# shizukutanaka/Otedama

Hardware: AMD Instinct MI355X
Metric: hashes/sec (whole node) SHA-256d + scrypt at 1/2/4/8 MI355X; p50 share latency (higher is better)
Workload: dtype u32

## Files before the change

csrc/bindings.cpp:

```cpp
#include <pybind11/pybind11.h>
#include <pybind11/stl.h>

#include <array>
#include <atomic>
#include <cstring>
#include <stdexcept>
#include <thread>
#include <tuple>

#include "otedama/aead.h"
#include "otedama/job.h"
#include "otedama/runtime.h"
#include "otedama/trace.h"
#include "otedama/sha256.h"
#include "otedama/sv2_frame.h"
#include "otedama/clock_bounds.h"
#include "otedama/launch_plan.h"
#include "otedama/search_launch.h"
#include "otedama/work_queue.h"
#include "otedama/x11.h"

namespace py = pybind11;
using namespace otedama;

namespace {

std::string need(const py::bytes& b, size_t n, const char* what) {
  std::string s = b;
  if (s.size() != n) throw std::invalid_argument(std::string(what) + ": expected " + std::to_string(n) + " bytes");
  return s;
}

py::bytes to_bytes(const uint8_t* p, size_t n) { return py::bytes(reinterpret_cast<const char*>(p), n); }

std::shared_ptr<JobTemplate> make_job(const py::dict& d) {
  auto j = std::make_shared<JobTemplate>();
  auto get = [&](const char* k) -> py::object {
    if (d.contains(k)) return py::object(d[k]);
    return py::none();
  };
  std::string hdr = need(d["header"].cast<py::bytes>(), 80, "header");
  std::memcpy(j->header, hdr.data(), 80);
  std::string tgt = need(d["target"].cast<py::bytes>(), 32, "target");
  std::memcpy(j->target, tgt.data(), 32);
  if (!get("epoch").is_none()) j->epoch = d["epoch"].cast<uint64_t>();
  if (!get("job_id").is_none()) j->job_id = d["job_id"].cast<std::string>();
  if (!get("channel_id").is_none()) j->channel_id = d["channel_id"].cast<uint32_t>();
  if (!get("algo").is_none()) {
    auto a = d["algo"].cast<std::string>();
    if (a == "sha256d") j->algo = Algo::kSha256d;
    else if (a == "scrypt") j->algo = Algo::kScrypt;
    else if (a == "x11") j->algo = Algo::kX11;
    else throw std::invalid_argument("unsupported algo for the native miner: " + a);
  }
  if (!get("version_mask").is_none()) j->version_mask = d["version_mask"].cast<uint32_t>();
  if (!get("ntime_roll").is_none()) j->ntime_roll = d["ntime_roll"].cast<uint32_t>();
  if (!get("coinb1").is_none()) {
    j->has_coinbase = true;
    std::string c1 = d["coinb1"].cast<py::bytes>(), c2 = d["coinb2"].cast<py::bytes>();
    std::string e1 = d["extranonce1"].cast<py::bytes>();
    j->coinb1.assign(c1.begin(), c1.end());
    j->coinb2.assign(c2.begin(), c2.end());
    j->extranonce1.assign(e1.begin(), e1.end());
    j->extranonce2_size = d["extranonce2_size"].cast<uint32_t>();
    for (auto& br : d["merkle_branches"].cast<py::list>()) {
      std::string b = br.cast<py::bytes>();
      j->merkle_branches.emplace_back(b.begin(), b.end());
    }
  }
  if (!get("variant_start").is_none()) j->variant_start = d["variant_start"].cast<uint64_t>();
  if (!get("variant_stride").is_none()) j->variant_stride = d["variant_stride"].cast<uint64_t>();
  if (j->variant_stride == 0) j->variant_stride = 1;
  return j;
}

py::list shares_to_list(std::vector<ShareRecord>&& v) {
  py::list out;
  for (auto& s : v) {
    py::dict d;
    d["epoch"] = s.epoch;
    d["job_id"] = s.job_id;
    d["channel_id"] = s.channel_id;
    d["nonce"] = s.nonce;
    d["ntime"] = s.ntime;
    d["version"] = s.version;
    d["extranonce2"] = s.extranonce2;
    d["extranonce2_size"] = s.extranonce2_size;
    d["hash"] = to_bytes(s.hash, 32);
    d["device_id"] = s.device_id;
    d["found_at"] = s.found_at;
    d["device_found_at"] = s.device_found_at;
    out.append(d);
  }
  return out;
}

py::dict stats_to_dict(const MinerStats& s) {
  py::dict d;
  d["hashes"] = s.hashes;
  d["candidates"] = s.candidates;
  d["shares"] = s.shares;
  d["dropped"] = s.dropped;
  d["launches"] = s.launches;
  d["rejected_candidates"] = s.rejected_candidates;
  d["variant_launches"] = s.variant_launches;
  d["busy_seconds"] = s.busy_seconds;
  d["faulted"] = s.faulted;
  d["error"] = s.error;
  d["variant_next"] = s.variant_next;
  d["variant_epoch"] = s.variant_epoch;
  d["job_switches"] = s.job_switches;
  d["last_job_switch_ms"] = s.last_job_switch_ms;
  d["job_switch_ms"] = s.job_switch_ms;
  d["work_started"] = s.work_started;
  d["reserved_cus"] = s.reserved_cus;
  d["ring_overflow"] = s.ring_overflow;
  d["verify_dropped"] = s.verify_dropped;
  d["verify_queue_peak"] = s.verify_queue_peak;
  d["launch_hashes"] = s.launch_hashes;
  d["aborted_launches"] = s.aborted_launches;
  d["ring_hits"] = s.ring_hits;
  d["clock_calib_rtt_us"] = s.clock_calib_rtt_us;
  d["clock_samples"] = s.clock_samples;
  d["host_abort"] = s.host_abort;
  d["hashes_done_at_s"] = s.hashes_done_at_s;
  {
    py::dict ph;
    for (const auto& kv : s.startup_ms) ph[py::str(kv.first)] = kv.second;
    d["startup_ms"] = ph;
    py::dict rs;
    for (const auto& kv : s.startup_rss_mb) rs[py::str(kv.first)] = kv.second;
    d["startup_rss_mb"] = rs;
  }
  return d;
}

}

PYBIND11_MODULE(_native, m) {
  m.doc() = "Otedama MI355X native runtime (gfx950 HIP kernels + C++ host runtime)";

  m.def("cpu_has_sha_ni", &cpu_has_sha_ni);
  m.def("sha256", [](const py::bytes& b) {
    std::string s = b; uint8_t o[32];
    sha256(reinterpret_cast<const uint8_t*>(s.data()), s.size(), o);
    return to_bytes(o, 32);
  });
  m.def("sha256d", [](const py::bytes& b) {
    std::string s = b; uint8_t o[32];
    { py::gil_scoped_release r; sha256d(reinterpret_cast<const uint8_t*>(s.data()), s.size(), o); }
    return to_bytes(o, 32);
  });
  m.def("hmac_sha256", [](const py::bytes& k, const py::bytes& msg) {
    std::string ks = k, ms = msg; uint8_t o[32];
    hmac_sha256(reinterpret_cast<const uint8_t*>(ks.data()), ks.size(),
                reinterpret_cast<const uint8_t*>(ms.data()), ms.size(), o);
    return to_bytes(o, 32);
  });
  m.def("aead_seal", [](int kind, const py::bytes& key, const py::bytes& nonce, const py::bytes& plain,
                        const py::bytes& aad) {
    std::string out = aead_seal(static_cast<AeadKind>(kind), key, nonce, plain, aad);
    return py::bytes(out);
  }, py::arg("kind"), py::arg("key"), py::arg("nonce"), py::arg("plain"), py::arg("aad") = py::bytes());
  m.def("aead_open", [](int kind, const py::bytes& key, const py::bytes& nonce, const py::bytes& sealed,
                        const py::bytes& aad) -> py::object {
    std::string out;
    if (!aead_open(static_cast<AeadKind>(kind), key, nonce, sealed, aad, &out)) return py::none();
    return py::bytes(out);
  }, py::arg("kind"), py::arg("key"), py::arg("nonce"), py::arg("sealed"), py::arg("aad") = py::bytes());
  m.attr("SCRYPT_COOP") = kScryptCoop;
  m.attr("SCRYPT_LANE_W8") = kScryptLaneW8;
  m.attr("SCRYPT_COOP2") = kScryptCoop2;
  m.attr("SCRYPT_COOP_SPLIT") = kScryptCoopSplit;
  m.attr("AEAD_AES256GCM") = 0;
  m.attr("AEAD_CHACHA20POLY1305") = 1;
  m.def("scrypt_1024_1_1_batch", [](const std::vector<py::bytes>& hs) {
    std::vector<std::string> in;
    for (const auto& h : hs) in.push_back(need(h, 80, "header"));
    std::vector<std::array<uint8_t, 32>> out(in.size());
    std::vector<const uint8_t*> ip;
    std::vector<uint8_t*> op;
    for (size_t i = 0; i < in.size(); ++i) {
      ip.push_back(reinterpret_cast<const uint8_t*>(in[i].data()));
      op.push_back(out[i].data());
    }
    {
      py::gil_scoped_release r;
      scrypt_1024_1_1_batch(int(in.size()), ip.data(), op.data());
    }
    py::list res;
    for (const auto& o : out) res.append(to_bytes(o.data(), 32));
    return res;
  });
  m.def("scrypt_1024_1_1", [](const py::bytes& h) {
    std::string s = need(h, 80, "header"); uint8_t o[32];
    { py::gil_scoped_release r; scrypt_1024_1_1(reinterpret_cast<const uint8_t*>(s.data()), o); }
    return to_bytes(o, 32);
  });
  m.def("_clock_bounds", [](double window, const std::vector<std::pair<double, double>>& samples) {
    ClockBounds cb(window);
    std::vector<double> out;
    for (const auto& s : samples) out.push_back(cb.add(s.first, s.second));
    return out;
  });
  m.def("_launch_plan_rules", [](uint64_t batch_nonces, uint32_t target_hi, bool capped, int sha_variants, int run,
                                 const std::string& reserve_cus, int ncu) {
    const ShaLayout lay = pick_layout(sha_variants, run);
    const CuMask cm = parse_reserved_cus(reserve_cus.c_str(), ncu);
    py::dict d;
    d["batch"] = normalize_batch(batch_nonces);
    d["cap"] = launch_cap_hashes(target_hi, capped);
    d["layout"] = py::make_tuple(lay.nvar, lay.use_v);
    d["cu_mask"] = cm.words;
    d["reserved"] = cm.reserved;
    return d;
  }, py::arg("batch_nonces") = 0, py::arg("target_hi") = 0, py::arg("capped") = true, py::arg("sha_variants") = 1,
     py::arg("run") = 1, py::arg("reserve_cus") = "", py::arg("ncu") = 256);
  m.def("_launch_plan_walk", [](const std::string& kind, uint64_t batch, uint64_t cap, int nvar, uint64_t lanes,
                                uint64_t start, size_t max_launches, uint64_t variant_start, uint64_t variant_stride) {
    const LaunchKind lk = kind == "scrypt" ? LaunchKind::kScrypt : kind == "x11" ? LaunchKind::kX11
                        : kind == "v" ? LaunchKind::kVersionParallel : kind == "k" ? LaunchKind::kVariantK
                        : kind == "single" ? LaunchKind::kSingle
                        : throw std::invalid_argument("kind: scrypt, x11, v, k or single");
    if (start >= kNonceSpace) throw std::invalid_argument("start must be below 2^32");
    SearchCursor c;
    c.nonce_off = start;
    std::vector<std::tuple<uint64_t, uint64_t, uint64_t>> launches;
    while (c.k == 0 && launches.size() < max_launches) {
      const uint64_t base = c.nonce_off, count = launch_count(lk, batch, cap, nvar, lanes, c.nonce_off);
      c.advance(count, nvar);
      launches.emplace_back(base, count, c.variant_next(variant_start, variant_stride, nvar));
    }
    return py::make_tuple(launches, c.k);
  }, py::arg("kind"), py::arg("batch"), py::arg("cap"), py::arg("nvar") = 1, py::arg("lanes") = 0,
     py::arg("start") = 0, py::arg("max_launches") = size_t(1) << 20, py::arg("variant_start") = 0,
     py::arg("variant_stride") = 1);
  m.def("_work_queue_flood", [](size_t cap, size_t n, bool hash_each, size_t batch) {
    BoundedWorkQueue<std::array<uint8_t, 80>> q(cap);
    std::atomic<uint64_t> processed{0};
    uint64_t accepted = 0;
    {
      py::gil_scoped_release r;
      std::thread consumer([&] {
        if (batch > 1) {
          std::vector<std::array<uint8_t, 80>> items;
          std::vector<const uint8_t*> ip;
          std::vector<std::array<uint8_t, 32>> outs(batch);
          std::vector<uint8_t*> op;
          for (auto& o : outs) op.push_back(o.data());
          while (items.clear(), q.pop_many(&items, batch) > 0) {
            ip.clear();
            for (const auto& it : items) ip.push_back(it.data());
            if (hash_each) scrypt_1024_1_1_batch(int(items.size()), ip.data(), op.data());
            processed.fetch_add(items.size());
          }
          return;
        }
        std::array<uint8_t, 80> h;
        uint8_t out[32];
        while (q.pop(&h)) {
          if (hash_each) scrypt_1024_1_1(h.data(), out);
          processed.fetch_add(1);
        }
      });
      for (size_t i = 0; i < n; ++i) {
        std::array<uint8_t, 80> h{};
        std::memcpy(h.data() + 76, &i, 4);
        if (q.push(std::move(h))) ++accepted;
      }
      q.stop(~size_t(0));
      consumer.join();
    }
    py::dict d;
    d["accepted"] = accepted;
    d["refused"] = q.refused();
    d["peak"] = q.peak();
    d["processed"] = processed.load();
    return d;
  }, py::arg("cap"), py::arg("n"), py::arg("hash_each") = true, py::arg("batch") = 1);
  m.attr("X11_STAGES") = kX11StageCount;
  m.def("x11", [](const py::bytes& msg) {
    std::string s = msg; uint8_t o[32];
    { py::gil_scoped_release r; x11::x11(reinterpret_cast<const uint8_t*>(s.data()), s.size(), o, nullptr); }
    return to_bytes(o, 32);
  }, py::arg("msg"));
  m.def("x11_trace", [](const py::bytes& msg) {
    std::string s = msg; uint8_t o[32], t[64 * kX11StageCount];
    x11::x11(reinterpret_cast<const uint8_t*>(s.data()), s.size(), o, t);
    return to_bytes(t, sizeof t);
  }, py::arg("msg"), "The 11 intermediate 64-byte digests of the X11 chain, concatenated.");
  m.def("x11_stage", [](int i, const py::bytes& msg) {
    if (i < 0 || i >= kX11StageCount) throw std::invalid_argument("stage must be in [0, 11)");
    std::string s = msg; uint8_t o[64];
    x11::stage(i, reinterpret_cast<const uint8_t*>(s.data()), s.size(), o);
    return to_bytes(o, 64);
  }, py::arg("stage"), py::arg("msg"));
  m.def("x11_luffa_sbox_selfcheck", &x11::luffa_sbox_selfcheck);
  m.def(
      "sv2_scan",
      [](py::buffer b, uint32_t max_frame) {
        py::buffer_info info = b.request();
        if (info.itemsize != 1 || info.ndim != 1) throw std::invalid_argument("sv2_scan: need a contiguous byte buffer");
        const size_t n = (size_t)info.size;
        if (n > 0xFFFFFFFFull) throw std::invalid_argument("sv2_scan: buffer larger than 4 GiB");
        std::vector<Sv2FrameRec> recs(n / kSv2HeaderSize + 1);
        size_t consumed = 0, k = 0;
        int status = kSv2Ok;
        {
          py::gil_scoped_release nogil;
          k = sv2_scan(static_cast<const uint8_t*>(info.ptr), n, max_frame, recs.data(), recs.size(), &consumed,
                       &status);
        }
        py::list frames(k);
        for (size_t i = 0; i < k; ++i) {
          const Sv2FrameRec& r = recs[i];
          frames[i] = py::make_tuple(r.extension_type, r.msg_type, r.offset, r.length);
        }
        return py::make_tuple(frames, consumed, status);
      },
      py::arg("buf"), py::arg("max_frame"),
      "Split complete SV2 frames: ([(extension_type, msg_type, payload_offset, payload_length)], consumed, status)");
  m.def("cpu_scan_sha256d", [](const py::bytes& h, const py::bytes& t, uint32_t start, uint64_t count) {
    std::string hs = need(h, 80, "header"), ts = need(t, 32, "target");
    std::vector<uint32_t> hits;
    {
      py::gil_scoped_release r;
      hits = cpu_scan_sha256d(reinterpret_cast<const uint8_t*>(hs.data()), reinterpret_cast<const uint8_t*>(ts.data()),
                              start, count);
    }
    return hits;
  }, py::arg("header"), py::arg("target"), py::arg("start"), py::arg("count"));
  m.def("cpu_scan_method", &cpu_scan_method);
  m.def("_cpu_scan_lanes", [](int lanes, const py::bytes& h, const py::bytes& t, uint32_t start, uint64_t count) {
    std::string hs = need(h, 80, "header"), ts = need(t, 32, "target");
    std::vector<uint32_t> hits;
    {
      py::gil_scoped_release r;
      hits = cpu_scan_sha256d_lanes(lanes, reinterpret_cast<const uint8_t*>(hs.data()),
                                    reinterpret_cast<const uint8_t*>(ts.data()), start, count);
    }
    return hits;
  });
  m.def("merkle_root", [](const py::dict& job, uint64_t en2) {
    auto j = make_job(job); uint8_t root[32];
    merkle_root_from_coinbase(*j, en2, root);
    return to_bytes(root, 32);
  });
  m.def("variant_header", [](const py::dict& job, uint64_t v) {
    auto j = make_job(job);
    uint8_t hdr[80]; uint32_t ver, nt; uint64_t en2;
    j->variant_header(v, hdr, &ver, &nt, &en2);
    return py::make_tuple(to_bytes(hdr, 80), ver, nt, en2);
  });
  m.def("variant_space", [](const py::dict& job) { return make_job(job)->variant_space(); });

  m.def("sha256d_prepare", [](const py::bytes& h, const py::bytes& t) {
    std::string hs = need(h, 80, "header"), ts = need(t, 32, "target");
    Sha256dParams p;
    sha256d_prepare(reinterpret_cast<const uint8_t*>(hs.data()), reinterpret_cast<const uint8_t*>(ts.data()), &p);
    return py::bytes(reinterpret_cast<const char*>(&p), sizeof p);
  });
  m.attr("SHA256D_MAX_K") = kSha256dMaxK;
  {
    py::list ks;
    for (int k = 2; k <= kSha256dMaxK; ++k)
      if (sha256d_k_floor(k) == k) ks.append(k);
    m.attr("SHA256D_K_VALUES") = py::tuple(ks);
  }
  m.def("sha256d_prepare_k", [](const py::list& headers, const py::bytes& t) {
    std::string ts = need(t, 32, "target");
    std::vector<std::string> hs;
    for (auto& h : headers) hs.push_back(need(h.cast<py::bytes>(), 80, "header"));
    std::vector<const uint8_t*> ptrs;
    for (auto& h : hs) ptrs.push_back(reinterpret_cast<const uint8_t*>(h.data()));
    Sha256dParamsK p;
    if (!sha256d_prepare_k(ptrs.data(), (int)ptrs.size(), reinterpret_cast<const uint8_t*>(ts.data()), &p))
      throw std::invalid_argument("need K headers (K in SHA256D_K_VALUES) with identical bytes 64..75");
    return py::bytes(reinterpret_cast<const char*>(&p), sizeof p);
  }, py::arg("headers"), py::arg("target"));
  m.attr("SHA256D_V_GROUP") = kSha256dVGroup;
  m.attr("SHA256D_V2_GROUP") = kSha256dV2Group;
  m.def("sha256d_prepare_v", [](const py::list& headers, const py::bytes& t) {
    std::string ts = need(t, 32, "target");
    std::vector<std::string> hs;
    for (auto& h : headers) hs.push_back(need(h.cast<py::bytes>(), 80, "header"));
    std::vector<const uint8_t*> ptrs;
    for (auto& h : hs) ptrs.push_back(reinterpret_cast<const uint8_t*>(h.data()));
    Sha256dParamsV p;
    std::vector<Sha256dVariant> vars(hs.size());
    if (!sha256d_prepare_v(ptrs.data(), (int)ptrs.size(), reinterpret_cast<const uint8_t*>(ts.data()), &p, vars.data()))
      throw std::invalid_argument("need a positive multiple of 64 headers with identical bytes 64..75");
    return py::make_tuple(py::bytes(reinterpret_cast<const char*>(&p), sizeof p),
                          py::bytes(reinterpret_cast<const char*>(vars.data()), vars.size() * sizeof(Sha256dVariant)));
  }, py::arg("headers"), py::arg("target"));
  m.def("scrypt_prepare", [](const py::bytes& h, const py::bytes& t) {
    std::string hs = need(h, 80, "header"), ts = need(t, 32, "target");
    ScryptParams p;
    scrypt_prepare(reinterpret_cast<const uint8_t*>(hs.data()), reinterpret_cast<const uint8_t*>(ts.data()), &p);
    return py::bytes(reinterpret_cast<const char*>(&p), sizeof p);
  });

  m.def("x11_prepare", [](const py::bytes& h, const py::bytes& t) {
    std::string hs = need(h, 80, "header"), ts = need(t, 32, "target");
    X11Params p;
    x11_prepare(reinterpret_cast<const uint8_t*>(hs.data()), reinterpret_cast<const uint8_t*>(ts.data()), &p);
    return py::bytes(reinterpret_cast<const char*>(&p), sizeof p);
  });

  m.def("trace_push", [](const std::string& name) { trace_push(name.c_str()); });
  m.def("trace_pop", [] { trace_pop(); });
  m.def("trace_mark", [](const std::string& name) { trace_mark(name.c_str()); });
  m.def("gpu_device_count", &gpu_device_count);
  m.def("gpu_arch_name", &gpu_arch_name);
  m.def("gpu_cu_count", &gpu_cu_count);
  m.def("scrypt_scratch_bytes", &scrypt_scratch_bytes);
  m.def("maps_range_writable", [](const std::string& maps, uint64_t lo, uint64_t hi) {
    return maps_range_writable(maps, uintptr_t(lo), uintptr_t(hi));
  });
  m.def("launch_sha256d", [](const py::bytes& params, uint32_t base, uint64_t count, uintptr_t out, uint32_t cap,
                             int grid, uintptr_t stream) {
    std::string ps = need(params, sizeof(Sha256dParams), "params");
    Sha256dParams p; std::memcpy(&p, ps.data(), sizeof p);
    if (count == 0 || count > (1ull << 32)) throw std::invalid_argument("count must be in [1, 2^32]");
    if (grid <= 0 || out == 0) throw std::invalid_argument("bad grid / out");
    py_launch_sha256d(p, base, count, out, cap, grid, stream);
  }, py::arg("params"), py::arg("base"), py::arg("count"), py::arg("out"), py::arg("cap"), py::arg("grid"),
     py::arg("stream"));
  m.def("launch_sha256d_k", [](const py::bytes& params, uint32_t base, uint64_t count, uintptr_t out, uint32_t cap,
                               int grid, uintptr_t stream) {
    std::string ps = need(params, sizeof(Sha256dParamsK), "params");
    Sha256dParamsK p; std::memcpy(&p, ps.data(), sizeof p);
    if (p.k < 2 || p.k > kSha256dMaxK) throw std::invalid_argument("bad K");
    if (count == 0 || count > (1ull << 32)) throw std::invalid_argument("count must be in [1, 2^32]");
    if (grid <= 0 || out == 0) throw std::invalid_argument("bad grid / out");
    py_launch_sha256d_k(p, base, count, out, cap, grid, stream);
  }, py::arg("params"), py::arg("base"), py::arg("count"), py::arg("out"), py::arg("cap"), py::arg("grid"),
     py::arg("stream"));
  m.def("launch_sha256d_v", [](const py::bytes& params, uintptr_t vars, uint32_t base, uint64_t count, uintptr_t out,
                               uint32_t cap, int grid, uintptr_t stream, bool occupancy8, int block, int chains) {
    std::string ps = need(params, sizeof(Sha256dParamsV), "params");
    Sha256dParamsV p; std::memcpy(&p, ps.data(), sizeof p);
    p.occupancy8 = occupancy8 ? 1u : 0u;
    if (p.groups == 0 || count == 0 || count > (1ull << 32)) throw std::invalid_argument("bad groups / count");
    if (block != 64 && block != 256) throw std::invalid_argument("block must be 64 or 256 threads");
    if (chains < 1 || chains > 4) throw std::invalid_argument("chains must be 1..4");
    if (p.groups % uint32_t(chains) != 0)
      throw std::invalid_argument("chains variants per lane need a multiple of 64 * chains variants");
    if (grid <= 0 || (uint64_t(grid) * uint32_t(block / 64)) % (p.groups / uint32_t(chains)) != 0 || vars == 0 || out == 0)
      throw std::invalid_argument("the wave count must be a multiple of the variant groups; vars/out must be set");
    py_launch_sha256d_v(p, vars, base, count, out, cap, grid, stream, block, chains);
  }, py::arg("params"), py::arg("vars"), py::arg("base"), py::arg("count"), py::arg("out"), py::arg("cap"),
     py::arg("grid"), py::arg("stream"), py::arg("occupancy8") = false, py::arg("block") = 256, py::arg("chains") = 1);
  m.def("launch_scrypt", [](const py::bytes& params, uint32_t base, uint32_t count, uintptr_t xbuf, uintptr_t scratch,
                            int gap, uintptr_t out, uint32_t cap, int grid, uintptr_t stream) {
    std::string ps = need(params, sizeof(ScryptParams), "params");
    ScryptParams p; std::memcpy(&p, ps.data(), sizeof p);
    if (gap != 1 && gap != 2 && gap != 4 && gap != kScryptCoop && gap != kScryptLaneW8 && gap != kScryptCoop2 &&
        gap != kScryptCoopSplit)
      throw std::invalid_argument("gap must be 1, 2, 4, SCRYPT_COOP or SCRYPT_LANE_W8");
    if (grid <= 0 || out == 0 || xbuf == 0 || scratch == 0 || count == 0) throw std::invalid_argument("bad launch args");
    py_launch_scrypt(p, base, count, xbuf, scratch, gap, out, cap, grid, stream);
  }, py::arg("params"), py::arg("base"), py::arg("count"), py::arg("xbuf"), py::arg("scratch"), py::arg("gap"),
     py::arg("out"), py::arg("cap"), py::arg("grid"), py::arg("stream"));

  m.def("launch_x11_stage", [](const py::bytes& params, int stage, uint32_t base, uintptr_t H, uint32_t stride,
                               uint32_t n, uintptr_t out, uint32_t cap, uintptr_t stream) {
    std::string ps = need(params, sizeof(X11Params), "params");
    X11Params p; std::memcpy(&p, ps.data(), sizeof p);
    if (stage < 0 || stage >= kX11StageCount) throw std::invalid_argument("stage must be in [0, 11)");
    if (H == 0 || n == 0 || stride < n) throw std::invalid_argument("need H != 0, n > 0, stride >= n");
    py_launch_x11_stage(p, stage, base, H, stride, n, out, cap, stream);
  }, py::arg("params"), py::arg("stage"), py::arg("base"), py::arg("H"), py::arg("stride"), py::arg("n"),
     py::arg("out") = 0, py::arg("cap") = 0, py::arg("stream") = 0);
  m.def("launch_x11", [](const py::bytes& params, uint32_t base, uintptr_t H, uint32_t stride, uint32_t n,
                         uintptr_t out, uint32_t cap, uintptr_t stream) {
    std::string ps = need(params, sizeof(X11Params), "params");
    X11Params p; std::memcpy(&p, ps.data(), sizeof p);
    if (H == 0 || n == 0 || stride < n) throw std::invalid_argument("need H != 0, n > 0, stride >= n");
    py_launch_x11(p, base, H, stride, n, out, cap, stream);
  }, py::arg("params"), py::arg("base"), py::arg("H"), py::arg("stride"), py::arg("n"), py::arg("out") = 0,
     py::arg("cap") = 0, py::arg("stream") = 0);

  py::class_<MinerBase, std::shared_ptr<MinerBase>>(m, "Miner")
      .def("start", &MinerBase::start, py::call_guard<py::gil_scoped_release>())
      .def("stop", &MinerBase::stop, py::call_guard<py::gil_scoped_release>())
      .def("set_job", [](MinerBase& self, py::object job) {
        if (job.is_none()) { py::gil_scoped_release r; self.set_job(nullptr); return; }
        auto j = make_job(job.cast<py::dict>());
        py::gil_scoped_release r;
        self.set_job(j);
      })
      .def("poll", [](MinerBase& self, size_t max) {
        std::vector<ShareRecord> v;
        { py::gil_scoped_release r; v = self.poll(max); }
        return shares_to_list(std::move(v));
      }, py::arg("max") = 256)
      .def("stats", [](MinerBase& self) { return stats_to_dict(self.stats()); })
      .def("share_fd", &MinerBase::share_fd,
           "eventfd that becomes readable when shares are queued (read 8 bytes to reset, then poll())")
      .def_property_readonly("device_id", &MinerBase::device_id);

  py::class_<GpuMiner, MinerBase, std::shared_ptr<GpuMiner>>(m, "GpuMiner")
      .def(py::init<int, std::string, uint64_t, int, size_t, int>(), py::arg("device"), py::arg("device_id"),
           py::arg("batch_nonces") = (1ull << 32), py::arg("grid") = 2048, py::arg("queue_cap") = 1024,
           py::arg("sha_variants") = 128);
  py::class_<CpuMiner, MinerBase, std::shared_ptr<CpuMiner>>(m, "CpuMiner")
      .def(py::init<int, std::string, size_t>(), py::arg("threads"), py::arg("device_id") = "cpu-0",
           py::arg("queue_cap") = 1024);

  m.attr("SHA256D_PARAMS_SIZE") = sizeof(Sha256dParams);
  m.attr("SHA256D_V_PARAMS_SIZE") = sizeof(Sha256dParamsV);
  m.attr("SCRYPT_PARAMS_SIZE") = sizeof(ScryptParams);
}
```

csrc/include/otedama/hitsink.h:

```cpp
#pragma once
#include <cstdint>

namespace otedama {

struct HitRecord {
  uint32_t nonce;
  uint32_t variant;
  uint32_t stamp;
  uint32_t tag;
};
static_assert(sizeof(HitRecord) == 16, "HitRecord is one 16-byte record");

struct HitSink {
  uint32_t* out = nullptr;
  HitRecord* ring = nullptr;
  const uint32_t* abort = nullptr;
  uint32_t cap = 0;
  uint32_t tag = 0;
  uint32_t epoch = 0;
  uint32_t words = 1;
};

}
```

csrc/include/otedama/launch_plan.h:

```cpp
#pragma once
#include <algorithm>
#include <cstdint>
#include <cstdlib>
#include <vector>

#include "otedama/job.h"

namespace otedama {

constexpr uint32_t kHitCap = 4096;
constexpr uint64_t kMinLaunchHashes = 1ull << 22;
constexpr uint64_t kNoLaunchCap = 1ull << 40;
constexpr uint64_t kNonceSpace = 1ull << 32;

inline uint64_t normalize_batch(uint64_t batch_nonces) {
  if (batch_nonces == 0 || batch_nonces > kNonceSpace) batch_nonces = 1ull << 30;
  while (kNonceSpace % batch_nonces) --batch_nonces;
  return batch_nonces;
}

inline uint64_t launch_cap_hashes(uint32_t target_hi, bool capped) {
  if (!capped) return kNoLaunchCap;
  const double p = (double(target_hi) + 1.0) / 4294967296.0;
  const double lim = double(kHitCap / 8) / p;
  uint64_t cap = kNoLaunchCap;
  while (cap > kMinLaunchHashes && double(cap) > lim) cap >>= 1;
  return cap;
}

struct ShaLayout {
  int nvar = 1;
  bool use_v = false;
};

inline ShaLayout pick_layout(int sha_variants, int run) {
  const int sha_k = sha_variants < 1 ? 1 : sha_variants > kSha256dMaxK ? kSha256dMaxK : sha_variants;
  if (sha_variants >= kSha256dV2Group && run >= kSha256dV2Group) return {kSha256dV2Group, true};
  if (sha_variants >= kSha256dVGroup && run >= kSha256dVGroup) return {kSha256dVGroup, true};
  if (sha_k > 1) return {sha256d_k_floor(std::min(run, sha_k)), false};
  return {1, false};
}

enum class LaunchKind { kScrypt, kX11, kVersionParallel, kVariantK, kSingle };

inline uint64_t launch_count(LaunchKind kind, uint64_t batch, uint64_t cap, int nvar, uint64_t lanes,
                             uint64_t nonce_off) {
  const uint64_t remaining = kNonceSpace - nonce_off;
  const uint64_t launch = std::min(batch, cap);
  switch (kind) {
    case LaunchKind::kScrypt:
    case LaunchKind::kX11:
      return std::min({remaining, lanes, cap});
    case LaunchKind::kVersionParallel:
      return std::min(launch >= uint64_t(nvar) ? launch / uint64_t(nvar) : 1, remaining);
    case LaunchKind::kVariantK: {
      uint64_t div = 1;
      while (div * 2 <= uint64_t(nvar) && div * 2 <= launch) div *= 2;
      return std::min(launch / div, remaining);
    }
    case LaunchKind::kSingle:
      break;
  }
  return std::min(launch, remaining);
}

struct SearchCursor {
  uint64_t k = 0;
  uint64_t nonce_off = 0;

  void reset() { k = 0; nonce_off = 0; }
  void advance(uint64_t count, int nvar) {
    nonce_off += count;
    if (nonce_off >= kNonceSpace) { nonce_off = 0; k += uint64_t(nvar); }
  }
  uint64_t variant_next(uint64_t variant_start, uint64_t variant_stride, int nvar) const {
    return variant_start + (nonce_off == 0 ? k : k + uint64_t(nvar)) * variant_stride;
  }
};

struct CuMask {
  std::vector<uint32_t> words;
  int reserved = 0;
};
inline CuMask parse_reserved_cus(const char* spec, int ncu) {
  CuMask m;
  m.words.assign(size_t(ncu + 31) / 32, 0xFFFFFFFFu);
  if (ncu % 32) m.words.back() = (1u << (ncu % 32)) - 1u;
  for (const char* q = spec; *q;) {
    char* end = nullptr;
    const long cu = std::strtol(q, &end, 10);
    if (end == q) break;
    if (cu >= 0 && cu < ncu && (m.words[size_t(cu) / 32] >> (cu % 32) & 1u)) {
      m.words[size_t(cu) / 32] &= ~(1u << (cu % 32));
      ++m.reserved;
    }
    q = (*end == ',') ? end + 1 : end;
  }
  return m;
}

inline uint64_t aborted_launch_hashes(uint64_t full, double rate_hpms, double ms) {
  return rate_hpms > 0 ? std::min<uint64_t>(full, uint64_t(rate_hpms * ms)) : full;
}
inline double update_rate_hpms(double rate_hpms, uint64_t full, double ms) {
  return rate_hpms > 0 ? 0.8 * rate_hpms + 0.2 * (double(full) / ms) : double(full) / ms;
}
inline double update_scrypt_hash_s(double scrypt_hash_s, double ms) { return 0.7 * scrypt_hash_s + 0.3e-3 * ms; }

}
```

csrc/include/otedama/runtime.h:

```cpp
#pragma once
#include <atomic>
#include <condition_variable>
#include <cstdint>
#include <deque>
#include <memory>
#include <mutex>
#include <string>
#include <thread>
#include <vector>

namespace otedama {

enum class Algo : int { kSha256d = 0, kScrypt = 1, kX11 = 2 };

struct JobTemplate {
  uint64_t epoch = 0;
  std::string job_id;
  uint32_t channel_id = 0;
  Algo algo = Algo::kSha256d;
  uint8_t header[80] = {0};
  uint8_t target[32] = {0};
  uint32_t version_mask = 0;
  uint32_t ntime_roll = 0;
  bool has_coinbase = false;
  std::vector<uint8_t> coinb1, coinb2, extranonce1;
  uint32_t extranonce2_size = 0;
  std::vector<std::vector<uint8_t>> merkle_branches;
  uint64_t variant_start = 0;
  uint64_t variant_stride = 1;

  uint64_t variant_space() const;
  void variant_header(uint64_t v, uint8_t out[80], uint32_t* version, uint32_t* ntime,
                      uint64_t* extranonce2) const;
};

struct ShareRecord {
  uint64_t epoch;
  std::string job_id;
  uint32_t channel_id;
  uint32_t nonce;
  uint32_t ntime;
  uint32_t version;
  uint64_t extranonce2;
  uint32_t extranonce2_size;
  uint8_t hash[32];
  std::string device_id;
  double found_at = 0;
  double device_found_at = 0;
};

struct MinerStats {
  uint64_t hashes = 0;
  uint64_t candidates = 0;
  uint64_t shares = 0;
  uint64_t dropped = 0;
  uint64_t launches = 0;
  uint64_t rejected_candidates = 0;
  uint64_t variant_launches = 0;
  double busy_seconds = 0;
  bool faulted = false;
  std::string error;
  uint64_t variant_next = 0;
  uint64_t variant_epoch = 0;
  uint64_t job_switches = 0;
  double last_job_switch_ms = 0;
  std::vector<double> job_switch_ms;
  std::vector<std::pair<uint64_t, double>> work_started;
  uint64_t aborted_launches = 0;
  uint64_t ring_hits = 0;
  uint64_t ring_overflow = 0;
  uint64_t verify_dropped = 0;
  uint64_t verify_queue_peak = 0;
  uint64_t launch_hashes = 0;
  double clock_calib_rtt_us = 0;
  uint64_t clock_samples = 0;
  bool host_abort = false;
  uint64_t reserved_cus = 0;
  double hashes_done_at_s = 0;
  std::vector<std::pair<std::string, double>> startup_ms;
  std::vector<std::pair<std::string, double>> startup_rss_mb;
};

bool verify_share(Algo algo, const uint8_t header80[80], const uint8_t target[32], uint8_t hash_out[32]);
void scrypt_1024_1_1(const uint8_t header80[80], uint8_t out[32]);
void scrypt_1024_1_1_batch(int n, const uint8_t* const header80[], uint8_t* const out[]);
void merkle_root_from_coinbase(const JobTemplate& job, uint64_t extranonce2, uint8_t root_out[32]);

class ShareQueue {
 public:
  explicit ShareQueue(size_t cap);
  ~ShareQueue();
  ShareQueue(const ShareQueue&) = delete;
  ShareQueue& operator=(const ShareQueue&) = delete;
  bool push(ShareRecord&& s);
  std::vector<ShareRecord> drain(size_t max);
  size_t size();
  uint64_t dropped() const { return dropped_.load(); }
  int event_fd() const { return efd_; }
 private:
  int efd_ = -1;
  std::mutex mu_;
  std::deque<ShareRecord> q_;
  size_t cap_;
  std::atomic<uint64_t> dropped_{0};
};

class MinerBase {
 public:
  MinerBase(std::string device_id, size_t queue_cap) : device_id_(std::move(device_id)), queue_(queue_cap) {}
  virtual ~MinerBase() = default;
  virtual void start() = 0;
  virtual void stop() = 0;
  void set_job(std::shared_ptr<const JobTemplate> job);
  std::vector<ShareRecord> poll(size_t max) { return queue_.drain(max); }
  MinerStats stats();
  const std::string& device_id() const { return device_id_; }
  int share_fd() const { return queue_.event_fd(); }

 protected:
  std::shared_ptr<const JobTemplate> current_job(uint64_t* gen);
  std::shared_ptr<const JobTemplate> peek_job(uint64_t* gen, double* set_at);
  std::string device_id_;
  ShareQueue queue_;
  std::mutex job_mu_;
  std::condition_variable job_cv_;
  std::shared_ptr<const JobTemplate> job_;
  std::shared_ptr<const JobTemplate> last_work_;
  uint64_t job_gen_ = 0;
  double job_set_at_ = 0;
  std::atomic<bool> running_{false};
  std::mutex stats_mu_;
  MinerStats stats_;
};

class GpuMiner : public MinerBase {
 public:
  GpuMiner(int device, std::string device_id, uint64_t batch_nonces, int grid, size_t queue_cap,
           int sha_variants = 128);
  ~GpuMiner() override;
  void start() override;
  void stop() override;
 private:
  struct Run;
  void loop();
  int device_;
  uint64_t batch_;
  int grid_;
  int sha_variants_;
  std::thread th_;
};

class CpuMiner : public MinerBase {
 public:
  CpuMiner(int threads, std::string device_id, size_t queue_cap);
  ~CpuMiner() override;
  void start() override;
  void stop() override;
 private:
  void loop(int tid);
  int threads_;
  std::vector<std::thread> ths_;
  std::atomic<uint64_t> cursor_{0};
  std::atomic<uint64_t> cursor_gen_{0};
  std::mutex cursor_mu_;
};

std::vector<uint32_t> cpu_scan_sha256d(const uint8_t header80[80], const uint8_t target[32], uint32_t start,
                                       uint64_t count);
std::string cpu_scan_method();
std::vector<uint32_t> cpu_scan_sha256d_lanes(int lanes, const uint8_t header80[80], const uint8_t target[32],
                                             uint32_t start, uint64_t count);

double monotonic_seconds();

bool maps_range_writable(const std::string& maps, uintptr_t lo, uintptr_t hi);

}
```

csrc/include/otedama/search_launch.h:

```cpp
#pragma once
#include <cstdint>
#include <string>

#include "otedama/hitsink.h"
#include "otedama/job.h"

namespace otedama {

uint64_t scrypt_scratch_bytes(int grid, int gap);

int gpu_device_count();
std::string gpu_arch_name(int device);
int gpu_cu_count(int device);

void py_launch_sha256d(const Sha256dParams& p, uint32_t base, uint64_t count, uintptr_t out, uint32_t cap, int grid,
                       uintptr_t stream);
void py_launch_sha256d_k(const Sha256dParamsK& p, uint32_t base, uint64_t count, uintptr_t out, uint32_t cap, int grid,
                         uintptr_t stream);
void py_launch_sha256d_v(const Sha256dParamsV& p, uintptr_t vars, uint32_t base, uint64_t count, uintptr_t out,
                         uint32_t cap, int grid, uintptr_t stream, int block, int chains);
void py_launch_scrypt(const ScryptParams& p, uint32_t base, uint32_t count, uintptr_t xbuf, uintptr_t scratch, int gap,
                      uintptr_t out, uint32_t cap, int grid, uintptr_t stream);
void py_launch_x11_stage(const X11Params& p, int stage, uint32_t base, uintptr_t H, uint32_t stride, uint32_t n,
                         uintptr_t out, uint32_t cap, uintptr_t stream);
void py_launch_x11(const X11Params& p, uint32_t base, uintptr_t H, uint32_t stride, uint32_t n, uintptr_t out,
                   uint32_t cap, uintptr_t stream);

}

#ifdef __HIPCC__
#include <hip/hip_runtime.h>

namespace otedama {

hipError_t launch_sha256d_search(const Sha256dParams& p, uint32_t base, uint64_t count, const HitSink& sink, int grid,
                                 hipStream_t stream);
hipError_t launch_sha256d_search_k(const Sha256dParamsK& p, uint32_t base, uint64_t count, const HitSink& sink,
                                   int grid, hipStream_t stream);
hipError_t launch_sha256d_search_v(const Sha256dParamsV& p, const Sha256dVariant* vars, uint32_t base, uint64_t count,
                                   const HitSink& sink, int grid, hipStream_t stream, int block = 256, int chains = 1);

hipError_t launch_scrypt_search(const ScryptParams& p, uint32_t base, uint32_t count, void* xbuf, void* scratch,
                                int gap, const HitSink& sink, int grid, hipStream_t stream);

}
#endif
```

csrc/kernels/hitsink_dev.h:

```cpp
#pragma once
#include <hip/hip_runtime.h>

#include <cstdint>

#include "otedama/hitsink.h"

namespace otedama_dev {

__device__ __forceinline__ uint32_t abort_peek(const uint32_t* word, uint32_t epoch) {
  if (word == nullptr) return epoch;
  const uint32_t v = __hip_atomic_load(const_cast<uint32_t*>(word), __ATOMIC_RELAXED, __HIP_MEMORY_SCOPE_SYSTEM);
  return __builtin_amdgcn_readfirstlane(v);
}
__device__ __forceinline__ uint32_t abort_peek(const otedama::HitSink& s) { return abort_peek(s.abort, s.epoch); }

__device__ __forceinline__ uint32_t abort_issue(const otedama::HitSink& s) {
  if (s.abort == nullptr) return s.epoch;
  return __hip_atomic_load(const_cast<uint32_t*>(s.abort), __ATOMIC_RELAXED, __HIP_MEMORY_SCOPE_SYSTEM);
}

__device__ __forceinline__ uint32_t abort_peek_scalar(const otedama::HitSink& s) {
  if (s.abort == nullptr) return s.epoch;
  uint32_t v;
  asm volatile("s_load_dword %0, %1, 0x0 glc\n\ts_waitcnt lgkmcnt(0)" : "=s"(v) : "s"(s.abort));
  return v;
}

__device__ __forceinline__ bool abort_newer(uint32_t word, uint32_t epoch) {
  return static_cast<int32_t>(word - epoch) > 0;
}
__device__ __forceinline__ bool abort_seen(uint32_t raw, uint32_t epoch) {
  return abort_newer(__builtin_amdgcn_readfirstlane(raw), epoch);
}

__device__ __forceinline__ void hit_publish(const otedama::HitSink& s, uint32_t nonce, uint32_t variant) {
  const uint32_t slot = atomicAdd(s.out, 1u);
  if (slot >= s.cap) return;
  if (s.ring != nullptr) {
    otedama::HitRecord* r = s.ring + slot;
    r->nonce = nonce;
    r->variant = variant;
    r->stamp = static_cast<uint32_t>(__builtin_amdgcn_s_memrealtime());
    __threadfence_system();
    __hip_atomic_store(&r->tag, s.tag, __ATOMIC_RELAXED, __HIP_MEMORY_SCOPE_SYSTEM);
  } else if (s.words == 2) {
    s.out[1 + 2 * slot] = nonce;
    s.out[2 + 2 * slot] = variant;
  } else {
    s.out[1 + slot] = nonce;
  }
}

}
```

csrc/kernels/scrypt_search.hip:

```cpp
#include <hip/hip_runtime.h>

#include <cstdint>

#include "cdna_bitops.h"
#include "hitsink_dev.h"
#include <cstdlib>
#include <cstring>

#include "otedama/job.h"
#include "otedama/search_launch.h"

namespace {

using namespace otedama_dev;

__device__ __forceinline__ uint32_t bswap(uint32_t x) { return __builtin_bswap32(x); }

__device__ __forceinline__ void salsa20_8(uint32_t B[16]) {
  uint32_t x0 = B[0], x1 = B[1], x2 = B[2], x3 = B[3], x4 = B[4], x5 = B[5], x6 = B[6], x7 = B[7];
  uint32_t x8 = B[8], x9 = B[9], x10 = B[10], x11 = B[11], x12 = B[12], x13 = B[13], x14 = B[14], x15 = B[15];
#pragma unroll
  for (int i = 0; i < 8; i += 2) {
    x4 ^= rol(x0 + x12, 7);   x8 ^= rol(x4 + x0, 9);    x12 ^= rol(x8 + x4, 13);   x0 ^= rol(x12 + x8, 18);
    x9 ^= rol(x5 + x1, 7);    x13 ^= rol(x9 + x5, 9);   x1 ^= rol(x13 + x9, 13);   x5 ^= rol(x1 + x13, 18);
    x14 ^= rol(x10 + x6, 7);  x2 ^= rol(x14 + x10, 9);  x6 ^= rol(x2 + x14, 13);   x10 ^= rol(x6 + x2, 18);
    x3 ^= rol(x15 + x11, 7);  x7 ^= rol(x3 + x15, 9);   x11 ^= rol(x7 + x3, 13);   x15 ^= rol(x11 + x7, 18);
    x1 ^= rol(x0 + x3, 7);    x2 ^= rol(x1 + x0, 9);    x3 ^= rol(x2 + x1, 13);    x0 ^= rol(x3 + x2, 18);
    x6 ^= rol(x5 + x4, 7);    x7 ^= rol(x6 + x5, 9);    x4 ^= rol(x7 + x6, 13);    x5 ^= rol(x4 + x7, 18);
    x11 ^= rol(x10 + x9, 7);  x8 ^= rol(x11 + x10, 9);  x9 ^= rol(x8 + x11, 13);   x10 ^= rol(x9 + x8, 18);
    x12 ^= rol(x15 + x14, 7); x13 ^= rol(x12 + x15, 9); x14 ^= rol(x13 + x12, 13); x15 ^= rol(x14 + x13, 18);
  }
  B[0] += x0; B[1] += x1; B[2] += x2; B[3] += x3; B[4] += x4; B[5] += x5; B[6] += x6; B[7] += x7;
  B[8] += x8; B[9] += x9; B[10] += x10; B[11] += x11; B[12] += x12; B[13] += x13; B[14] += x14; B[15] += x15;
}

__device__ __forceinline__ void blockmix(uint32_t X[32]) {
#pragma unroll
  for (int k = 0; k < 16; ++k) X[k] ^= X[16 + k];
  salsa20_8(X);
#pragma unroll
  for (int k = 0; k < 16; ++k) X[16 + k] ^= X[k];
  salsa20_8(X + 16);
}

__device__ __forceinline__ void store_entry(uint4* __restrict__ dst, const uint32_t X[32]) {
#pragma unroll
  for (int q = 0; q < 8; ++q) dst[q] = make_uint4(X[4 * q], X[4 * q + 1], X[4 * q + 2], X[4 * q + 3]);
}
__device__ __forceinline__ void load_entry(const uint4* __restrict__ src, uint32_t T[32]) {
#pragma unroll
  for (int q = 0; q < 8; ++q) {
    const uint4 v = src[q];
    T[4 * q] = v.x; T[4 * q + 1] = v.y; T[4 * q + 2] = v.z; T[4 * q + 3] = v.w;
  }
}

__device__ __forceinline__ void hmac_states(const uint32_t key[8], uint32_t istate[8], uint32_t ostate[8]) {
  uint32_t blk[16];
#pragma unroll
  for (int i = 0; i < 8; ++i) blk[i] = key[i] ^ 0x36363636u;
#pragma unroll
  for (int i = 8; i < 16; ++i) blk[i] = 0x36363636u;
#pragma unroll
  for (int i = 0; i < 8; ++i) istate[i] = kSha256IVd[i];
  sha256_compress(istate, blk);
#pragma unroll
  for (int i = 0; i < 8; ++i) blk[i] = key[i] ^ 0x5c5c5c5cu;
#pragma unroll
  for (int i = 8; i < 16; ++i) blk[i] = 0x5c5c5c5cu;
#pragma unroll
  for (int i = 0; i < 8; ++i) ostate[i] = kSha256IVd[i];
  sha256_compress(ostate, blk);
}

__device__ __forceinline__ void hmac_outer(const uint32_t ostate[8], const uint32_t digest[8], uint32_t out[8]) {
  uint32_t blk[16];
#pragma unroll
  for (int i = 0; i < 8; ++i) blk[i] = digest[i];
  blk[8] = 0x80000000u;
#pragma unroll
  for (int i = 9; i < 15; ++i) blk[i] = 0u;
  blk[15] = 768u;
#pragma unroll
  for (int i = 0; i < 8; ++i) out[i] = ostate[i];
  sha256_compress(out, blk);
}

__device__ __forceinline__ void scrypt_pbkdf_in(const otedama::ScryptParams& p, uint32_t nonce, uint32_t X[32]) {
  uint32_t hdrbe[20];
#pragma unroll
  for (int i = 0; i < 19; ++i) hdrbe[i] = bswap(p.hdr[i]);
  hdrbe[19] = bswap(nonce);
  uint32_t key[8];
#pragma unroll
  for (int i = 0; i < 8; ++i) key[i] = p.hmid[i];
  {
    uint32_t blk[16] = {hdrbe[16], hdrbe[17], hdrbe[18], hdrbe[19], 0x80000000u, 0, 0, 0, 0, 0, 0, 0, 0, 0, 0, 640u};
    sha256_compress(key, blk);
  }
  uint32_t istate[8], ostate[8];
  hmac_states(key, istate, ostate);
  uint32_t ist2[8];
#pragma unroll
  for (int i = 0; i < 8; ++i) ist2[i] = istate[i];
  sha256_compress(ist2, hdrbe);
#pragma unroll
  for (int blkno = 1; blkno <= 4; ++blkno) {
    uint32_t st[8];
#pragma unroll
    for (int i = 0; i < 8; ++i) st[i] = ist2[i];
    uint32_t blk[16] = {hdrbe[16], hdrbe[17], hdrbe[18], hdrbe[19], uint32_t(blkno), 0x80000000u,
                        0, 0, 0, 0, 0, 0, 0, 0, 0, (64u + 84u) * 8u};
    sha256_compress(st, blk);
    uint32_t t[8];
    hmac_outer(ostate, st, t);
#pragma unroll
    for (int i = 0; i < 8; ++i) X[8 * (blkno - 1) + i] = bswap(t[i]);
  }
}

__device__ __forceinline__ uint32_t scrypt_pbkdf_out(const otedama::ScryptParams& p, uint32_t nonce,
                                                     const uint32_t X[32]) {
  uint32_t key[8];
#pragma unroll
  for (int i = 0; i < 8; ++i) key[i] = p.hmid[i];
  {
    uint32_t blk[16] = {bswap(p.hdr[16]), bswap(p.hdr[17]), bswap(p.hdr[18]), bswap(nonce), 0x80000000u,
                        0, 0, 0, 0, 0, 0, 0, 0, 0, 0, 640u};
    sha256_compress(key, blk);
  }
  uint32_t istate[8], ostate[8];
  hmac_states(key, istate, ostate);
  uint32_t st[8];
#pragma unroll
  for (int i = 0; i < 8; ++i) st[i] = istate[i];
  uint32_t blk[16];
#pragma unroll
  for (int i = 0; i < 16; ++i) blk[i] = bswap(X[i]);
  sha256_compress(st, blk);
#pragma unroll
  for (int i = 0; i < 16; ++i) blk[i] = bswap(X[16 + i]);
  sha256_compress(st, blk);
  uint32_t tail[16] = {1u, 0x80000000u, 0, 0, 0, 0, 0, 0, 0, 0, 0, 0, 0, 0, 0, (64u + 132u) * 8u};
  sha256_compress(st, tail);
  uint32_t out[8];
  hmac_outer(ostate, st, out);
  return out[7];
}

template <int GAP>
__device__ __forceinline__ void scrypt_romix(uint32_t X[32], uint4* __restrict__ Vw, uint32_t lane) {
  for (int i = 0; i < 1024; ++i) {
    if (i % GAP == 0) store_entry(Vw + ((uint64_t(i / GAP) * 64u + lane) << 3), X);
    blockmix(X);
  }
  for (int i = 0; i < 1024; ++i) {
    const uint32_t j = X[16] & 1023u;
    uint32_t T[32];
    load_entry(Vw + ((uint64_t(j / GAP) * 64u + lane) << 3), T);
    if constexpr (GAP > 1) {
      for (uint32_t r = 0; r < (j % GAP); ++r) blockmix(T);
    }
#pragma unroll
    for (int k = 0; k < 32; ++k) X[k] ^= T[k];
    blockmix(X);
  }
}

typedef __attribute__((address_space(3))) void glds_lptr_t;
typedef unsigned coop_v4u __attribute__((ext_vector_type(4)));

#ifndef OTD_SCRYPT_STORE_CPOL
#define OTD_SCRYPT_STORE_CPOL 2
#endif
constexpr int kStoreNT = OTD_SCRYPT_STORE_CPOL;

__device__ __forceinline__ uint32_t coop_swz(uint32_t s_local) {
  return ((s_local >> 1) & 3u) | (((s_local >> 3) & 1u) << 2);
}

__device__ __forceinline__ void coop_store_entry(const uint32_t X[32], __amdgpu_buffer_rsrc_t rs, uint4* __restrict__ tile,
                                                 uint32_t lane, uint32_t i) {
  char* tb = reinterpret_cast<char*>(tile);
  uint32_t ln = lane;
  asm volatile("" : "+v"(ln));
  const uint32_t slot = ln & 7u, octet = ln >> 3, own = ln & 31u;
  const uint32_t rd = (own << 7) ^ (coop_swz(own) << 4);
#pragma unroll
  for (int h = 0; h < 2; ++h) {
    asm volatile("s_waitcnt lgkmcnt(0)" ::: "memory");
    if ((ln >> 5) == uint32_t(h)) {
#pragma unroll
      for (int c = 0; c < 8; ++c)
        *reinterpret_cast<uint4*>(tb + (rd ^ (uint32_t(c) << 4))) =
            make_uint4(X[4 * c], X[4 * c + 1], X[4 * c + 2], X[4 * c + 3]);
    }
    __builtin_amdgcn_wave_barrier();
#pragma unroll
    for (int r = 0; r < 4; ++r) {
      const uint4 v = tile[64 * r + ln];
      const uint32_t owner = uint32_t(32 * h + 8 * r) + octet;
      const uint32_t chunk = slot ^ (((octet >> 1) & 3u) | (uint32_t(r & 1) << 2));
      const coop_v4u vv = {v.x, v.y, v.z, v.w};
      __builtin_amdgcn_raw_buffer_store_b128(vv, rs, (i << 13) | (owner << 7) | (chunk << 4), 0, kStoreNT);
    }
  }
}

template <int LCPOL>
__device__ __forceinline__ void coop_issue(const uint32_t X[32], __amdgpu_buffer_rsrc_t rs, uint4* __restrict__ tile,
                                           uint32_t lane, coop_v4u R[4]) {
  uint32_t ln = lane;
  asm volatile("" : "+v"(ln));
  const uint32_t slot = ln & 7u, octet = ln >> 3;
  const uint32_t j = X[16] & 1023u;
  asm volatile("s_waitcnt lgkmcnt(0)" ::: "memory");
#pragma unroll
  for (int r = 0; r < 4; ++r) {
    const uint32_t chunk = slot ^ (((octet >> 1) & 3u) | (uint32_t(r & 1) << 2));
    const uint32_t o0 = uint32_t(8 * r) + octet, o1 = o0 + 32u;
    const uint32_t j0 = uint32_t(__shfl(int(j), int(o0), 64));
    const uint32_t j1 = uint32_t(__shfl(int(j), int(o1), 64));
    __builtin_amdgcn_raw_ptr_buffer_load_lds(rs, (glds_lptr_t*)(tile + 64 * r), 16, (j0 << 13) | (o0 << 7) | (chunk << 4),
                                             0, 0, LCPOL);
    R[r] = __builtin_amdgcn_raw_buffer_load_b128(rs, (j1 << 13) | (o1 << 7) | (chunk << 4), 0, LCPOL);
  }
}

__device__ __forceinline__ void coop_consume(uint32_t X[32], uint4* __restrict__ tile, uint32_t lane,
                                             const coop_v4u R[4]) {
  const char* tb = reinterpret_cast<const char*>(tile);
  uint32_t ln = lane;
  asm volatile("" : "+v"(ln));
  const uint32_t own = ln & 31u;
  const uint32_t rd = (own << 7) ^ (coop_swz(own) << 4);
  asm volatile("s_waitcnt vmcnt(0)" ::: "memory");
  if (ln < 32u) {
#pragma unroll
    for (int c = 0; c < 8; ++c) {
      const uint4 t = *reinterpret_cast<const uint4*>(tb + (rd ^ (uint32_t(c) << 4)));
      X[4 * c] ^= t.x; X[4 * c + 1] ^= t.y; X[4 * c + 2] ^= t.z; X[4 * c + 3] ^= t.w;
    }
  }
  asm volatile("s_waitcnt lgkmcnt(0)" ::: "memory");
#pragma unroll
  for (int r = 0; r < 4; ++r) tile[64 * r + ln] = make_uint4(R[r].x, R[r].y, R[r].z, R[r].w);
  __builtin_amdgcn_wave_barrier();
  if (ln >= 32u) {
#pragma unroll
    for (int c = 0; c < 8; ++c) {
      const uint4 t = *reinterpret_cast<const uint4*>(tb + (rd ^ (uint32_t(c) << 4)));
      X[4 * c] ^= t.x; X[4 * c + 1] ^= t.y; X[4 * c + 2] ^= t.z; X[4 * c + 3] ^= t.w;
    }
  }
}

template <int LCPOL, int POLL>
__device__ __forceinline__ bool scrypt_romix_coop(uint32_t X[32], __amdgpu_buffer_rsrc_t rs, uint4* __restrict__ tile,
                                                  uint32_t lane, const otedama::HitSink& sink) {
  static_assert(POLL > 0 && 1024 % POLL == 0, "poll interval must divide the ROMix loop");
  if (abort_newer(abort_peek(sink), sink.epoch)) return false;
  for (uint32_t c = 0; c < 1024; c += POLL) {
    if (c && abort_newer(abort_peek_scalar(sink), sink.epoch)) return false;
    for (uint32_t i = c; i < c + POLL; ++i) {
      coop_store_entry(X, rs, tile, lane, i);
      blockmix(X);
    }
  }
  if (abort_newer(abort_peek(sink), sink.epoch)) return false;
  for (int i = 0; i < 1024; ++i) {
    coop_v4u R[4];
    coop_issue<LCPOL>(X, rs, tile, lane, R);
    coop_consume(X, tile, lane, R);
    blockmix(X);
  }
  return true;
}

template <int LCPOL, int PHASE>
__device__ __forceinline__ void scrypt_romix_coop_phase(uint32_t X[32], __amdgpu_buffer_rsrc_t rs,
                                                        uint4* __restrict__ tile, uint32_t lane) {
  if constexpr (PHASE == 1) {
    for (uint32_t i = 0; i < 1024; ++i) {
      coop_store_entry(X, rs, tile, lane, i);
      blockmix(X);
    }
  } else {
    for (int i = 0; i < 1024; ++i) {
      coop_v4u R[4];
      coop_issue<LCPOL>(X, rs, tile, lane, R);
      coop_consume(X, tile, lane, R);
      blockmix(X);
    }
  }
}

template <int LCPOL>
__device__ __forceinline__ void scrypt_romix_coop2(uint32_t XA[32], uint32_t XB[32], __amdgpu_buffer_rsrc_t rsA,
                                                   __amdgpu_buffer_rsrc_t rsB, uint4* __restrict__ tile, uint32_t lane) {
  for (uint32_t i = 0; i < 1024; ++i) {
    coop_store_entry(XA, rsA, tile, lane, i);
    blockmix(XA);
    coop_store_entry(XB, rsB, tile, lane, i);
    blockmix(XB);
  }
  coop_v4u R[4];
  coop_issue<LCPOL>(XA, rsA, tile, lane, R);
  for (int i = 0; i < 1024; ++i) {
    coop_consume(XA, tile, lane, R);
    coop_issue<LCPOL>(XB, rsB, tile, lane, R);
    blockmix(XA);
    coop_consume(XB, tile, lane, R);
    if (i < 1023) coop_issue<LCPOL>(XA, rsA, tile, lane, R);
    blockmix(XB);
  }
}

}

extern "C" __global__ __launch_bounds__(256) void otd_scrypt_pbkdf_in(const otedama::ScryptParams p, uint32_t base,
                                                                      uint32_t count, uint4* __restrict__ xbuf) {
  const uint32_t i = blockIdx.x * blockDim.x + threadIdx.x;
  if (i >= count) return;
  uint32_t X[32];
  scrypt_pbkdf_in(p, base + i, X);
  store_entry(xbuf + (uint64_t(i) << 3), X);
}

template <int GAP>
__global__ __launch_bounds__(256) void otd_scrypt_romix(uint32_t count, uint4* __restrict__ xbuf,
                                                        uint4* __restrict__ V) {
  const uint64_t slot = uint64_t(blockIdx.x) * blockDim.x + threadIdx.x;
  const uint64_t nslots = uint64_t(gridDim.x) * blockDim.x;
  uint4* Vw = V + (slot >> 6) * (uint64_t(1024 / GAP) * 64u * 8u);
  const uint32_t lane = uint32_t(slot & 63u);
  for (uint64_t i = slot; i < count; i += nslots) {
    uint32_t X[32];
    load_entry(xbuf + (i << 3), X);
    scrypt_romix<GAP>(X, Vw, lane);
    store_entry(xbuf + (i << 3), X);
  }
}

template <int LCPOL, int POLL>
__global__ __launch_bounds__(256) __attribute__((amdgpu_waves_per_eu(8, 8))) void otd_scrypt_romix_coop(uint32_t count, uint4* __restrict__ xbuf,
                                                             uint4* __restrict__ V, const otedama::HitSink sink) {
  __shared__ uint4 tiles[4 * 256];
  const uint64_t slot = uint64_t(blockIdx.x) * blockDim.x + threadIdx.x;
  const uint64_t nslots = uint64_t(gridDim.x) * blockDim.x;
  const uint32_t lane = uint32_t(slot & 63u);
  const uint64_t wave = (uint64_t(__builtin_amdgcn_readfirstlane(uint32_t(slot >> 32))) << 26) |
                        uint64_t(__builtin_amdgcn_readfirstlane(uint32_t(slot) >> 6));
  uint4* Vw = V + wave * (1024ull * 64u * 8u);
  const __amdgpu_buffer_rsrc_t rs = __builtin_amdgcn_make_buffer_rsrc(Vw, (short)0, 1024 * 64 * 128, 0x00020000);
  (void)Vw;
  uint4* tile = tiles + __builtin_amdgcn_readfirstlane(threadIdx.x >> 6) * 256;
  for (uint64_t i = slot; i < count; i += nslots) {
    uint32_t X[32];
    load_entry(xbuf + (i << 3), X);
    if (!scrypt_romix_coop<LCPOL, POLL>(X, rs, tile, lane, sink)) return;
    store_entry(xbuf + (i << 3), X);
  }
}

template <int LCPOL, int PHASE>
__global__ __launch_bounds__(256) __attribute__((amdgpu_waves_per_eu(8, 8))) void otd_scrypt_romix_coop_phase(
    uint32_t count, uint4* __restrict__ xbuf, uint4* __restrict__ V) {
  __shared__ uint4 tiles[4 * 256];
  const uint64_t slot = uint64_t(blockIdx.x) * blockDim.x + threadIdx.x;
  const uint32_t lane = uint32_t(slot & 63u);
  const uint64_t wave = (uint64_t(__builtin_amdgcn_readfirstlane(uint32_t(slot >> 32))) << 26) |
                        uint64_t(__builtin_amdgcn_readfirstlane(uint32_t(slot) >> 6));
  uint4* Vw = V + wave * (1024ull * 64u * 8u);
  const __amdgpu_buffer_rsrc_t rs = __builtin_amdgcn_make_buffer_rsrc(Vw, (short)0, 1024 * 64 * 128, 0x00020000);
  uint4* tile = tiles + __builtin_amdgcn_readfirstlane(threadIdx.x >> 6) * 256;
  if (slot < count) {
    uint32_t X[32];
    load_entry(xbuf + (slot << 3), X);
    scrypt_romix_coop_phase<LCPOL, PHASE>(X, rs, tile, lane);
    store_entry(xbuf + (slot << 3), X);
  }
}

template <int LCPOL>
__global__ __launch_bounds__(256) __attribute__((amdgpu_waves_per_eu(8, 8))) void otd_scrypt_romix_coop_seg(
    uint32_t count, uint4* __restrict__ xbuf, uint4* __restrict__ V, uint32_t it0, uint32_t it1,
    const otedama::HitSink sink) {
  __shared__ uint4 tiles[4 * 256];
  const uint64_t slot = uint64_t(blockIdx.x) * blockDim.x + threadIdx.x;
  const uint32_t lane = uint32_t(slot & 63u);
  uint4* tile = tiles + __builtin_amdgcn_readfirstlane(threadIdx.x >> 6) * 256;
  if (abort_newer(abort_peek(sink), sink.epoch)) return;
  const uint64_t nslots = uint64_t(gridDim.x) * blockDim.x;
  for (uint64_t h = slot; h < count; h += nslots) {
    const uint64_t hw = (uint64_t(__builtin_amdgcn_readfirstlane(uint32_t(h >> 32))) << 26) |
                        uint64_t(__builtin_amdgcn_readfirstlane(uint32_t(h) >> 6));
    const __amdgpu_buffer_rsrc_t rh =
        __builtin_amdgcn_make_buffer_rsrc(V + hw * (1024ull * 64u * 8u), (short)0, 1024 * 64 * 128, 0x00020000);
    uint32_t X[32];
    load_entry(xbuf + (h << 3), X);
    const uint32_t w1 = it1 < 1024u ? it1 : 1024u;
    for (uint32_t i = it0; i < w1; ++i) {
      coop_store_entry(X, rh, tile, lane, i);
      blockmix(X);
    }
    for (uint32_t i = it0 > 1024u ? it0 : 1024u; i < it1; ++i) {
      coop_v4u R[4];
      coop_issue<LCPOL>(X, rh, tile, lane, R);
      coop_consume(X, tile, lane, R);
      blockmix(X);
    }
    store_entry(xbuf + (h << 3), X);
  }
}

template <int LCPOL>
__global__ __launch_bounds__(256) __attribute__((amdgpu_waves_per_eu(4, 4))) void otd_scrypt_romix_coop2(
    uint32_t count, uint4* __restrict__ xbuf, uint4* __restrict__ V) {
  __shared__ uint4 tiles[4 * 256];
  const uint32_t lane = threadIdx.x & 63u;
  const uint64_t wave0 = (uint64_t(blockIdx.x) * blockDim.x + threadIdx.x) >> 6;
  const uint64_t nwaves = (uint64_t(gridDim.x) * blockDim.x) >> 6;
  const uint64_t wslot = (uint64_t(__builtin_amdgcn_readfirstlane(uint32_t(wave0 >> 32))) << 32) |
                         uint64_t(__builtin_amdgcn_readfirstlane(uint32_t(wave0)));
  uint4* VA = V + wslot * (2ull * 1024 * 64 * 8);
  uint4* VB = VA + 1024ull * 64 * 8;
  const __amdgpu_buffer_rsrc_t rsA = __builtin_amdgcn_make_buffer_rsrc(VA, (short)0, 1024 * 64 * 128, 0x00020000);
  const __amdgpu_buffer_rsrc_t rsB = __builtin_amdgcn_make_buffer_rsrc(VB, (short)0, 1024 * 64 * 128, 0x00020000);
  uint4* tile = tiles + __builtin_amdgcn_readfirstlane(threadIdx.x >> 6) * 256;
  for (uint64_t w = wslot; w * 128 < count; w += nwaves) {
    const uint64_t ia = w * 128 + lane, ib = ia + 64;
    uint32_t XA[32], XB[32];
    load_entry(xbuf + (ia << 3), XA);
    load_entry(xbuf + (ib << 3), XB);
    scrypt_romix_coop2<LCPOL>(XA, XB, rsA, rsB, tile, lane);
    store_entry(xbuf + (ia << 3), XA);
    store_entry(xbuf + (ib << 3), XB);
  }
}

__global__ __launch_bounds__(256) __attribute__((amdgpu_waves_per_eu(8, 8))) void otd_scrypt_romix_w8(
    uint32_t count, uint4* __restrict__ xbuf, uint4* __restrict__ V) {
  const uint64_t slot = uint64_t(blockIdx.x) * blockDim.x + threadIdx.x;
  const uint64_t nslots = uint64_t(gridDim.x) * blockDim.x;
  uint4* Vw = V + (slot >> 6) * (1024ull * 64u * 8u);
  const uint32_t lane = uint32_t(slot & 63u);
  for (uint64_t i = slot; i < count; i += nslots) {
    uint32_t X[32];
    load_entry(xbuf + (i << 3), X);
    scrypt_romix<1>(X, Vw, lane);
    store_entry(xbuf + (i << 3), X);
  }
}

extern "C" __global__ __launch_bounds__(256) void otd_scrypt_pbkdf_out(const otedama::ScryptParams p, uint32_t base,
                                                                       uint32_t count, const uint4* __restrict__ xbuf,
                                                                       const otedama::HitSink sink) {
  const uint32_t i = blockIdx.x * blockDim.x + threadIdx.x;
  if (i >= count) return;
  if (abort_newer(abort_peek(sink), sink.epoch)) return;
  uint32_t X[32];
  load_entry(xbuf + (uint64_t(i) << 3), X);
  const uint32_t h7 = scrypt_pbkdf_out(p, base + i, X);
  if (bswap(h7) <= p.target_hi) hit_publish(sink, base + i, 0u);
}

template __global__ void otd_scrypt_romix<1>(uint32_t, uint4*, uint4*);
template __global__ void otd_scrypt_romix<2>(uint32_t, uint4*, uint4*);
template __global__ void otd_scrypt_romix<4>(uint32_t, uint4*, uint4*);

namespace otedama {

uint64_t scrypt_scratch_bytes(int grid, int gap) {
  if (gap == kScryptCoop2) return uint64_t(grid) * 512ull * 1024ull * 128ull;
  if (gap == kScryptCoop || gap == kScryptLaneW8 || gap == kScryptCoopSplit) gap = 1;
  return uint64_t(grid) * 256ull * (1024ull / uint64_t(gap)) * 128ull;
}

static bool scrypt_write_polls() {
  static const bool on = [] {
    const char* v = std::getenv("OTEDAMA_SCRYPT_POLL");
    return !(v && v[0] == '0');
  }();
  return on;
}

static uint32_t scrypt_segments() {
  const char* v = std::getenv("OTEDAMA_SCRYPT_SEGMENTS");
  if (!v || !v[0]) return 0;
  const long x = std::strtol(v, nullptr, 10);
  return uint32_t(x < 1 ? 1 : (x > 64 ? 64 : x));
}

static int scrypt_seg_grid(int grid) {
  const char* v = std::getenv("OTEDAMA_SCRYPT_SEG_GRID");
  if (!v || !v[0]) return grid;
  int cap = 0;
  if (std::strcmp(v, "resident") == 0) {
    int dev = 0, cus = 0;
    if (hipGetDevice(&dev) != hipSuccess ||
        hipDeviceGetAttribute(&cus, hipDeviceAttributeMultiprocessorCount, dev) != hipSuccess || cus <= 0)
      return grid;
    cap = cus * 8;
  } else {
    cap = int(std::strtol(v, nullptr, 10));
  }
  return cap > 0 && cap < grid ? cap : grid;
}

hipError_t launch_scrypt_search(const ScryptParams& p, uint32_t base, uint32_t count, void* xbuf, void* scratch,
                                int gap, const HitSink& sink, int grid, hipStream_t stream) {
  uint4* X = static_cast<uint4*>(xbuf);
  uint4* V = static_cast<uint4*>(scratch);
  const int eg = int((count + 255) / 256);
  const uint32_t count64 = (count + 63u) & ~63u;
  if (gap == kScryptCoopSplit && uint64_t(count64) > uint64_t(grid) * 256u) return hipErrorInvalidValue;
  hipLaunchKernelGGL(otd_scrypt_pbkdf_in, dim3(eg), dim3(256), 0, stream, p, base, count, X);
  switch (gap) {
    case kScryptCoop:
      if (scrypt_segments() > 0 && uint64_t(count64) <= uint64_t(grid) * 256u) {
        const uint32_t S = scrypt_segments();
        const int sg = scrypt_seg_grid(grid);
        for (uint32_t k = 0; k < S; ++k)
          hipLaunchKernelGGL(otd_scrypt_romix_coop_seg<2>, dim3(sg), dim3(256), 0, stream, count64, X, V,
                             2048u * k / S, 2048u * (k + 1) / S, sink);
      } else if (scrypt_write_polls())
        hipLaunchKernelGGL((otd_scrypt_romix_coop<2, 64>), dim3(grid), dim3(256), 0, stream, count64, X, V, sink);
      else
        hipLaunchKernelGGL((otd_scrypt_romix_coop<2, 1024>), dim3(grid), dim3(256), 0, stream, count64, X, V, sink);
      break;
    case kScryptLaneW8:
      hipLaunchKernelGGL(otd_scrypt_romix_w8, dim3(grid), dim3(256), 0, stream, count, X, V);
      break;
    case kScryptCoopSplit:
      hipLaunchKernelGGL((otd_scrypt_romix_coop_phase<2, 1>), dim3(grid), dim3(256), 0, stream, count64, X, V);
      hipLaunchKernelGGL((otd_scrypt_romix_coop_phase<2, 2>), dim3(grid), dim3(256), 0, stream, count64, X, V);
      break;
    case kScryptCoop2:
      hipLaunchKernelGGL(otd_scrypt_romix_coop2<2>, dim3(grid), dim3(256), 0, stream, (count + 127u) & ~127u, X, V);
      break;
    case 1: hipLaunchKernelGGL(otd_scrypt_romix<1>, dim3(grid), dim3(256), 0, stream, count, X, V); break;
    case 2: hipLaunchKernelGGL(otd_scrypt_romix<2>, dim3(grid), dim3(256), 0, stream, count, X, V); break;
    case 4: hipLaunchKernelGGL(otd_scrypt_romix<4>, dim3(grid), dim3(256), 0, stream, count, X, V); break;
    default: return hipErrorInvalidValue;
  }
  hipLaunchKernelGGL(otd_scrypt_pbkdf_out, dim3(eg), dim3(256), 0, stream, p, base, count, X, sink);
  return hipGetLastError();
}

}
```

csrc/runtime/gpu_miner.hip:

```cpp
#include <hip/hip_runtime.h>
#include <hsa/hsa.h>
#include <hsa/hsa_ext_amd.h>
#include <immintrin.h>

#include <algorithm>
#include <atomic>
#include <chrono>
#include <cstdio>
#include <cstdlib>
#include <cstring>
#include <deque>
#include <memory>
#include <stdexcept>
#include <string>
#include <unistd.h>

#include "otedama/clock_bounds.h"
#include "otedama/hitsink.h"
#include "otedama/job.h"
#include "otedama/launch_plan.h"
#include "otedama/runtime.h"
#include "otedama/search_launch.h"
#include "otedama/sha256.h"
#include "otedama/trace.h"
#include "otedama/work_queue.h"
#include "otedama/x11_launch.h"

namespace otedama {

static double resident_mb() {
  FILE* f = std::fopen("/proc/self/statm", "r");
  if (!f) return 0;
  unsigned long size = 0, res = 0;
  const int n = std::fscanf(f, "%lu %lu", &size, &res);
  std::fclose(f);
  return n == 2 ? double(res) * double(sysconf(_SC_PAGESIZE)) / (1024.0 * 1024.0) : 0;
}

#define OTD_HIP(call)                                                                              \
  do {                                                                                             \
    hipError_t e_ = (call);                                                                        \
    if (e_ != hipSuccess)                                                                          \
      throw std::runtime_error(std::string("HIP error ") + hipGetErrorString(e_) + " at " #call); \
  } while (0)

}

__global__ void otd_rt_probe(uint64_t* out) {
  if (threadIdx.x == 0) *out = __builtin_amdgcn_s_memrealtime();
}

namespace otedama {

namespace {
constexpr size_t kVerifyCap = 8192;
constexpr int kInflight = 2;
constexpr double kRtHz = 100e6;
constexpr auto kIdlePoll = std::chrono::microseconds(100);
constexpr double kClockWindowS = 2.0;
constexpr int kScryptGap = kScryptCoop;
constexpr uint32_t kX11Batch = 1u << 23;

bool cpu_store_map(void* p, size_t n) {
  hsa_agent_t cpu{};
  auto pick = [](hsa_agent_t a, void* data) -> hsa_status_t {
    hsa_device_type_t t;
    if (hsa_agent_get_info(a, HSA_AGENT_INFO_DEVICE, &t) == HSA_STATUS_SUCCESS && t == HSA_DEVICE_TYPE_CPU) {
      *static_cast<hsa_agent_t*>(data) = a;
      return HSA_STATUS_INFO_BREAK;
    }
    return HSA_STATUS_SUCCESS;
  };
  if (hsa_iterate_agents(pick, &cpu) != HSA_STATUS_INFO_BREAK) return false;
  if (hsa_amd_agents_allow_access(1, &cpu, nullptr, p) != HSA_STATUS_SUCCESS) return false;
  FILE* f = std::fopen("/proc/self/maps", "r");
  if (!f) return false;
  std::string maps;
  char buf[4096];
  size_t got;
  while ((got = std::fread(buf, 1, sizeof buf, f)) > 0) maps.append(buf, got);
  std::fclose(f);
  const uintptr_t lo = reinterpret_cast<uintptr_t>(p);
  return maps_range_writable(maps, lo, lo + n);
}

template <class T, class Drop>
struct Owned {
  T h{};
  Owned() = default;
  Owned(const Owned&) = delete;
  Owned& operator=(const Owned&) = delete;
  ~Owned() { if (h) Drop()(h); }
  operator T() const { return h; }
};
struct FreeDevice { void operator()(void* p) const { (void)hipFree(p); } };
struct FreePinned { void operator()(void* p) const { (void)hipHostFree(p); } };
struct DestroyStream { void operator()(hipStream_t s) const { (void)hipStreamDestroy(s); } };
struct DestroyEvent { void operator()(hipEvent_t e) const { (void)hipEventDestroy(e); } };
template <class T> using DeviceMem = Owned<T*, FreeDevice>;
template <class T> using PinnedMem = Owned<T*, FreePinned>;
using Stream = Owned<hipStream_t, DestroyStream>;
using Event = Owned<hipEvent_t, DestroyEvent>;

struct Group {
  uint64_t gen = ~0ull, k = ~0ull;
  int nvar = 1;
  bool use_v = false;
  uint8_t header[kSha256dV2Group][80];
  uint32_t version[kSha256dV2Group] = {0}, ntime[kSha256dV2Group] = {0};
  uint64_t en2[kSha256dV2Group] = {0};
  Sha256dParamsV v_params{};
  Sha256dVariant v_table[kSha256dV2Group];
};

struct Candidate {
  std::shared_ptr<const JobTemplate> job;
  std::shared_ptr<const Group> group;
  uint64_t gen;
  uint32_t nonce, vi, stamp;
  double enq_host;
  uint32_t rt_enq;
  int nvar;
};

struct Batch {
  bool busy = false;
  std::shared_ptr<const JobTemplate> job;
  std::shared_ptr<const Group> group;
  uint64_t gen = 0;
  uint32_t epoch = 0, tag = 0;
  uint64_t count = 0;
  int nvar = 1;
  uint32_t consumed = 0;
  double enq_host = 0;
  uint32_t rt_enq = 0;
  bool started = false;
  hipStream_t stream = nullptr;
  Event start, done;
  DeviceMem<uint32_t> d_count;
  PinnedMem<uint32_t> h_count;
  PinnedMem<HitRecord> ring;
  HitRecord* ring_dev = nullptr;
  DeviceMem<Sha256dVariant> d_vars;
  PinnedMem<Sha256dVariant> h_vars;
  uint64_t* h_clk = nullptr;
  uint64_t* d_clk = nullptr;
  bool clk_pending = false;
  TraceId range = 0;
};

using JobPtr = std::shared_ptr<const JobTemplate>;
}

GpuMiner::GpuMiner(int device, std::string device_id, uint64_t batch_nonces, int grid, size_t queue_cap, int sha_variants)
    : MinerBase(std::move(device_id), queue_cap), device_(device), batch_(normalize_batch(batch_nonces)), grid_(grid),
      sha_variants_(sha_variants) {}

GpuMiner::~GpuMiner() { stop(); }

void GpuMiner::start() {
  if (running_.exchange(true)) return;
  th_ = std::thread([this] {
    try {
      loop();
    } catch (const std::exception& ex) {
      std::lock_guard<std::mutex> g(stats_mu_);
      stats_.faulted = true;
      stats_.error = ex.what();
    }
  });
}

void GpuMiner::stop() {
  if (!running_.exchange(false)) return;
  job_cv_.notify_all();
  if (th_.joinable()) th_.join();
}

struct GpuMiner::Run {
  explicit Run(GpuMiner& miner) : m(miner) {}

  GpuMiner& m;
  double t_phase = 0, t_loop = 0;

  Stream ctl;
  Stream search[kInflight];

  bool host_abort = false;
  DeviceMem<uint32_t> d_abort;
  Event ref_ev;
  PinnedMem<uint64_t> h_rt;
  uint64_t* d_rt = nullptr;
  DeviceMem<void> scratch;
  DeviceMem<void> xbuf;
  DeviceMem<uint64_t> x11_h;
  Batch slots[kInflight];

  int cus = 256;
  ShaLayout max_layout;
  int scrypt_grid = 0;
  uint32_t scrypt_batch = 0;
  bool scrypt_halves = true, x11_overlap = true;
  bool cap_launches = true;
  int grid_k = 0, grid_v = 0, grid_v2 = 0;

  double rt_offset = 0.0;
  double calib_rtt = 1e9;
  ClockBounds clk_bounds{kClockWindowS};

  std::shared_ptr<Group> group;
  uint64_t cur_gen = ~0ull;
  SearchCursor cursor;
  uint32_t epoch = 1, tag = 0;
  uint64_t epoch_gen = ~0ull;
  bool switch_pending = false, first_switch = true;
  double switch_t0 = 0;
  double rate_hpms = 0;
  double scrypt_hash_s = 0.064;
  std::deque<int> fifo;
  BoundedWorkQueue<Candidate> vq{kVerifyCap};
  std::thread verifier;

  ~Run() {
    vq.stop(m.running_.load() ? ~size_t(0) : 64);
    if (verifier.joinable()) verifier.join();
    for (auto& s : search)
      if (s) (void)hipStreamSynchronize(s);
    if (ctl) (void)hipStreamSynchronize(ctl);
  }

  void phase(const char* name) {
    const double now = monotonic_seconds();
    std::lock_guard<std::mutex> g(m.stats_mu_);
    m.stats_.startup_ms.emplace_back(name, (now - t_phase) * 1e3);
    m.stats_.startup_rss_mb.emplace_back(name, resident_mb());
    t_phase = now;
  }

  void setup_streams() {
    const int ncu = gpu_cu_count(m.device_);
    cus = ncu > 0 ? ncu : 256;
    const char* ss_env = std::getenv("OTEDAMA_SEARCH_STREAMS");
    const bool one_stream = ss_env && std::atoi(ss_env) == 1;
    CuMask mask;
    if (const char* rc_env = std::getenv("OTEDAMA_RESERVE_CUS")) mask = parse_reserved_cus(rc_env, cus);
    for (int i = 0; i < kInflight; ++i) {
      if (one_stream && i > 0) {
        slots[i].stream = search[0];
        continue;
      }
      if (mask.reserved > 0)
        OTD_HIP(hipExtStreamCreateWithCUMask(&search[i].h, uint32_t(mask.words.size()), mask.words.data()));
      else OTD_HIP(hipStreamCreateWithFlags(&search[i].h, hipStreamNonBlocking));
      slots[i].stream = search[i];
    }
    std::lock_guard<std::mutex> g(m.stats_mu_);
    m.stats_.reserved_cus = uint64_t(mask.reserved);
  }

  void setup_abort_word() {
    hipStream_t s0 = slots[0].stream;
    OTD_HIP(hipExtMallocWithFlags(reinterpret_cast<void**>(&d_abort.h), 256, hipDeviceMallocUncached));
    OTD_HIP(hipMemsetAsync(d_abort, 0, 256, s0));
    OTD_HIP(hipStreamSynchronize(s0));
    const char* ha_env = std::getenv("OTEDAMA_HOST_ABORT");
    host_abort = !(ha_env && ha_env[0] == '0') && cpu_store_map(d_abort, 256);
    if (host_abort) {
      for (uint32_t probe : {0xA5C3E10Fu, 0u}) {
        __atomic_store_n(d_abort.h, probe, __ATOMIC_RELEASE);
        _mm_sfence();
        uint32_t back = ~probe;
        OTD_HIP(hipMemcpyAsync(&back, d_abort, sizeof back, hipMemcpyDeviceToHost, s0));
        OTD_HIP(hipStreamSynchronize(s0));
        if (back != probe) { host_abort = false; break; }
      }
      if (!host_abort) {
        OTD_HIP(hipMemsetAsync(d_abort, 0, 256, s0));
        OTD_HIP(hipStreamSynchronize(s0));
      }
    }
    if (!host_abort) {
      int prio_lo = 0, prio_hi = 0;
      OTD_HIP(hipDeviceGetStreamPriorityRange(&prio_lo, &prio_hi));
      OTD_HIP(hipStreamCreateWithPriority(&ctl.h, hipStreamNonBlocking, prio_hi));
    }
    std::lock_guard<std::mutex> g(m.stats_mu_);
    m.stats_.host_abort = host_abort;
  }

  void setup_buffers() {
    OTD_HIP(hipHostMalloc(reinterpret_cast<void**>(&h_rt.h), 64 * (1 + kInflight),
                          hipHostMallocCoherent | hipHostMallocMapped));
    std::memset(h_rt, 0, 64 * (1 + kInflight));
    OTD_HIP(hipHostGetDevicePointer(reinterpret_cast<void**>(&d_rt), h_rt, 0));
    for (int i = 0; i < kInflight; ++i) {
      slots[i].h_clk = h_rt.h + 8 * (1 + i);
      slots[i].d_clk = d_rt + 8 * (1 + i);
    }
    phase("control_words");
    max_layout = pick_layout(m.sha_variants_, kSha256dV2Group);
    for (auto& s : slots) {
      OTD_HIP(hipMalloc(&s.d_count.h, 64));
      OTD_HIP(hipHostMalloc(reinterpret_cast<void**>(&s.h_count.h), 64, hipHostMallocDefault));
      OTD_HIP(hipHostMalloc(reinterpret_cast<void**>(&s.ring.h), kHitCap * sizeof(HitRecord),
                            hipHostMallocCoherent | hipHostMallocMapped));
      std::memset(s.ring, 0, kHitCap * sizeof(HitRecord));
      OTD_HIP(hipHostGetDevicePointer(reinterpret_cast<void**>(&s.ring_dev), s.ring, 0));
      OTD_HIP(hipEventCreate(&s.start.h));
      OTD_HIP(hipEventCreate(&s.done.h));
      if (max_layout.use_v) {
        OTD_HIP(hipMalloc(&s.d_vars.h, kSha256dV2Group * sizeof(Sha256dVariant)));
        OTD_HIP(hipHostMalloc(&s.h_vars.h, kSha256dV2Group * sizeof(Sha256dVariant), hipHostMallocDefault));
      }
    }
    phase("buffers");
    scrypt_grid = cus * 16;
    scrypt_batch = uint32_t(scrypt_grid) * 256u;
    const char* halves_env = std::getenv("OTEDAMA_SCRYPT_HALVES");
    scrypt_halves = !(halves_env && halves_env[0] == '0');
    const char* x11ov_env = std::getenv("OTEDAMA_X11_OVERLAP");
    x11_overlap = !(x11ov_env && x11ov_env[0] == '0');
    const char* cap_env = std::getenv("OTEDAMA_LAUNCH_CAP");
    cap_launches = !(cap_env && cap_env[0] == '0');
    grid_k = cus * 16;
    grid_v = cus * 64;
    grid_v2 = cus * 128;
  }

  void probe_clock(hipStream_t on) {
    __atomic_store_n(h_rt.h, 0ull, __ATOMIC_RELEASE);
    const double t0 = monotonic_seconds();
    hipLaunchKernelGGL(otd_rt_probe, dim3(1), dim3(64), 0, on, d_rt);
    OTD_HIP(hipGetLastError());
    OTD_HIP(hipStreamSynchronize(on));
    const double t1 = monotonic_seconds();
    const uint64_t rt = __atomic_load_n(h_rt.h, __ATOMIC_ACQUIRE);
    if (rt && (t1 - t0) < calib_rtt) {
      rt_offset = 0.5 * (t0 + t1) - double(rt) / kRtHz;
      calib_rtt = t1 - t0;
      std::lock_guard<std::mutex> g(m.stats_mu_);
      m.stats_.clock_calib_rtt_us = (t1 - t0) * 1e6;
    }
  }

  void clock_seen(Batch& b) {
    const uint64_t rt = __atomic_load_n(b.h_clk, __ATOMIC_ACQUIRE);
    if (!rt) return;
    const double now = monotonic_seconds();
    b.clk_pending = false;
    rt_offset = clk_bounds.add(now, now - double(rt) / kRtHz);
    std::lock_guard<std::mutex> g(m.stats_mu_);
    m.stats_.clock_samples += 1;
  }

  void write_abort(uint32_t e) {
    if (host_abort) {
      __atomic_store_n(d_abort.h, e, __ATOMIC_RELEASE);
      _mm_sfence();
    } else {
      OTD_HIP(hipStreamWriteValue32(ctl, d_abort, e, 0));
    }
  }

  JobPtr check_epoch(uint64_t* gen_out) {
    uint64_t gen = 0;
    double set_at = 0;
    auto job = m.peek_job(&gen, &set_at);
    const uint64_t want_gen = job ? gen : epoch_gen;
    if (want_gen != epoch_gen) {
      epoch_gen = want_gen;
      ++epoch;
      if (!fifo.empty()) write_abort(epoch);
      if (job) { switch_pending = true; switch_t0 = set_at; }
    }
    if (gen_out) *gen_out = gen;
    return job;
  }

  void verify_push(const Candidate& b, uint32_t nonce, uint32_t vi, uint32_t stamp, bool stamped, const JobPtr& cur,
                   uint64_t cur_g, uint64_t* good, uint64_t* bad, const uint8_t* pre_hash = nullptr) {
    if (vi >= (uint32_t)b.nvar) { ++*bad; return; }
    uint8_t hdr[80];
    std::memcpy(hdr, b.group->header[vi], 80);
    store_le32(hdr + 76, nonce);
    ShareRecord r{};
    const JobTemplate* tj = (cur && cur_g == b.gen) ? cur.get() : b.job.get();
    if (pre_hash) {
      std::memcpy(r.hash, pre_hash, 32);
      if (!le256_leq(r.hash, tj->target)) { ++*bad; return; }
    } else if (!verify_share(b.job->algo, hdr, tj->target, r.hash)) {
      ++*bad;
      return;
    }
    r.epoch = tj->epoch; r.job_id = tj->job_id; r.channel_id = tj->channel_id;
    r.nonce = nonce; r.ntime = b.group->ntime[vi]; r.version = b.group->version[vi]; r.extranonce2 = b.group->en2[vi];
    r.extranonce2_size = b.job->extranonce2_size; r.device_id = m.device_id_;
    r.found_at = monotonic_seconds();
    if (stamped) r.device_found_at = b.enq_host + double(int32_t(stamp - b.rt_enq)) / kRtHz;
    m.queue_.push(std::move(r));
    ++*good;
  }

  void verify_loop() {
    std::vector<Candidate> cs;
    cs.reserve(16);
    uint8_t hb[16][80], ho[16][32];
    const uint8_t* ip[16];
    uint8_t* op[16];
    for (int l = 0; l < 16; ++l) { ip[l] = hb[l]; op[l] = ho[l]; }
    while (cs.clear(), vq.pop_many(&cs, 16) > 0) {
      uint64_t good = 0, bad = 0, g = 0;
      auto cur = m.peek_job(&g, nullptr);
      int n = 0;
      for (const Candidate& c : cs) {
        if (c.job->algo != Algo::kScrypt || c.vi >= (uint32_t)c.nvar) continue;
        std::memcpy(hb[n], c.group->header[c.vi], 80);
        store_le32(hb[n] + 76, c.nonce);
        ++n;
      }
      if (n > 0) scrypt_1024_1_1_batch(n, ip, op);
      int l = 0;
      for (const Candidate& c : cs) {
        const bool batched = c.job->algo == Algo::kScrypt && c.vi < (uint32_t)c.nvar;
        verify_push(c, c.nonce, c.vi, c.stamp, true, cur, g, &good, &bad, batched ? ho[l] : nullptr);
        l += batched;
      }
      std::lock_guard<std::mutex> sg(m.stats_mu_);
      m.stats_.shares += good;
      m.stats_.rejected_candidates += bad;
    }
  }

  uint32_t drain_ring(Batch& b, uint32_t final_n, const JobPtr& cur, uint64_t cur_g) {
    const uint32_t limit = final_n == ~0u ? kHitCap : std::min(final_n, kHitCap);
    uint64_t good = 0, bad = 0, lost = 0, handled = 0;
    while (b.consumed < limit) {
      HitRecord* r = b.ring.h + b.consumed;
      const uint32_t tg = __atomic_load_n(&r->tag, __ATOMIC_ACQUIRE);
      if (tg != b.tag) {
        if (final_n == ~0u) break;
        ++lost;
        ++b.consumed;
        continue;
      }
      const uint32_t nonce = __atomic_load_n(&r->nonce, __ATOMIC_RELAXED);
      const uint32_t vi = __atomic_load_n(&r->variant, __ATOMIC_RELAXED);
      const uint32_t stamp = __atomic_load_n(&r->stamp, __ATOMIC_RELAXED);
      if (b.job->algo == Algo::kScrypt) {
        vq.push(Candidate{b.job, b.group, b.gen, nonce, vi, stamp, b.enq_host, b.rt_enq, b.nvar});
      } else {
        verify_push(Candidate{b.job, b.group, b.gen, 0, 0, 0, b.enq_host, b.rt_enq, b.nvar}, nonce, vi, stamp, true,
                    cur, cur_g, &good, &bad);
      }
      ++b.consumed;
      ++handled;
    }
    if (handled || lost) {
      const uint64_t refused = vq.refused(), peak = vq.peak();
      std::lock_guard<std::mutex> g(m.stats_mu_);
      m.stats_.shares += good;
      m.stats_.rejected_candidates += bad + lost;
      if (final_n == ~0u) m.stats_.ring_hits += handled;
      m.stats_.verify_dropped = refused;
      m.stats_.verify_queue_peak = peak;
    }
    return uint32_t(handled);
  }

  void finish(Batch& b, const JobPtr& cur, uint64_t cur_g) {
    trace_stop(b.range);
    const uint32_t n = *b.h_count.h;
    drain_ring(b, n, cur, cur_g);
    float ms = 0;
    (void)hipEventElapsedTime(&ms, b.start, b.done);
    float done_ms = 0;
    const bool have_done = hipEventElapsedTime(&done_ms, ref_ev, b.done) == hipSuccess;
    const uint64_t full = b.count * uint64_t(b.nvar);
    const bool aborted = int32_t(epoch - b.epoch) > 0;
    const uint64_t done_hashes = aborted ? aborted_launch_hashes(full, rate_hpms, ms) : full;
    if (!aborted && ms > 0) rate_hpms = update_rate_hpms(rate_hpms, full, ms);
    if (!aborted && ms > 0 && b.job && b.job->algo == Algo::kScrypt)
      scrypt_hash_s = update_scrypt_hash_s(scrypt_hash_s, ms);
    std::lock_guard<std::mutex> g(m.stats_mu_);
    if (n > kHitCap) {
      if (m.stats_.ring_overflow == 0)
        std::fprintf(stderr, "otedama: %s: launch found %u candidates, hit ring holds %u: %u lost (counted in "
                     "ring_overflow)\n", m.device_id_.c_str(), n, kHitCap, n - kHitCap);
      m.stats_.ring_overflow += n - kHitCap;
    }
    m.stats_.hashes += done_hashes;
    if (have_done) m.stats_.hashes_done_at_s = std::max(m.stats_.hashes_done_at_s, double(done_ms) * 1e-3);
    m.stats_.candidates += n;
    m.stats_.busy_seconds += ms * 1e-3;
    m.stats_.launches += 1;
    if (aborted) m.stats_.aborted_launches += 1;
    if (b.nvar > 1) m.stats_.variant_launches += 1;
    b.busy = false;
    b.job.reset();
    b.group.reset();
  }

  std::shared_ptr<Group> build_group(const JobPtr& job, uint64_t gen) {
    auto gp = std::make_shared<Group>();
    const uint64_t k = cursor.k;
    gp->gen = gen;
    gp->k = k;
    gp->nvar = 1;
    const uint64_t v = job->variant_start + k * job->variant_stride;
    job->variant_header(v, gp->header[0], &gp->version[0], &gp->ntime[0], &gp->en2[0]);
    if (job->algo != Algo::kSha256d || max_layout.nvar <= 1) return gp;
    int kv = 1;
    while (kv < max_layout.nvar) {
      const uint64_t vk = job->variant_start + (k + kv) * job->variant_stride;
      if (vk >= job->variant_space()) break;
      job->variant_header(vk, gp->header[kv], &gp->version[kv], &gp->ntime[kv], &gp->en2[kv]);
      if (std::memcmp(gp->header[kv] + 64, gp->header[0] + 64, 12) != 0) break;
      ++kv;
    }
    const ShaLayout lay = pick_layout(m.sha_variants_, kv);
    gp->nvar = lay.nvar;
    gp->use_v = lay.use_v;
    if (gp->use_v) {
      const uint8_t* hs[kSha256dV2Group];
      for (int j = 0; j < gp->nvar; ++j) hs[j] = gp->header[j];
      if (!sha256d_prepare_v(hs, gp->nvar, job->target, &gp->v_params, gp->v_table))
        throw std::runtime_error("sha256d_prepare_v");
      gp->v_params.occupancy8 = gp->nvar == kSha256dV2Group ? 0 : 1;
    }
    return gp;
  }

  uint64_t launch_cap(const JobTemplate& job) const {
    return launch_cap_hashes(load_le32(job.target + 28), cap_launches);
  }

  uint64_t launch_scrypt(Batch& s, const JobTemplate& job, const HitSink& sink) {
    if (!scratch) {
      OTD_HIP(hipMalloc(&scratch.h, scrypt_scratch_bytes(scrypt_grid, kScryptGap)));
      OTD_HIP(hipMalloc(&xbuf.h, uint64_t(scrypt_batch) * 128));
    }
    ScryptParams p;
    scrypt_prepare(group->header[0], job.target, &p);
    const int slot_i = int(&s - slots);
    const int grid = scrypt_halves ? scrypt_grid / 2 : scrypt_grid;
    const uint32_t lanes = scrypt_halves ? scrypt_batch / 2 : scrypt_batch;
    char* pad = static_cast<char*>(scratch.h) +
                (scrypt_halves ? uint64_t(slot_i) * scrypt_scratch_bytes(grid, kScryptGap) : 0);
    char* xb = static_cast<char*>(xbuf.h) + (scrypt_halves ? uint64_t(slot_i) * lanes * 128ull : 0);
    const uint64_t count = launch_count(LaunchKind::kScrypt, m.batch_, launch_cap(job), 1, lanes, cursor.nonce_off);
    OTD_HIP(launch_scrypt_search(p, uint32_t(cursor.nonce_off), uint32_t(count), xb, pad, kScryptGap, sink, grid,
                                 s.stream));
    return count;
  }

  uint64_t launch_x11(Batch& s, const JobTemplate& job, const HitSink& sink) {
    if (!x11_h) OTD_HIP(hipMalloc(&x11_h.h, uint64_t(kX11Batch) * 64 * (x11_overlap ? kInflight : 1)));
    X11Params p;
    x11_prepare(group->header[0], job.target, &p);
    const int slot_i = int(&s - slots);
    const uint64_t count = launch_count(LaunchKind::kX11, m.batch_, launch_cap(job), 1, kX11Batch, cursor.nonce_off);
    uint64_t* H = x11_h.h + (x11_overlap ? uint64_t(slot_i) * kX11Batch * 8 : 0);
    OTD_HIP(x11_launch_chain(p, uint32_t(cursor.nonce_off), H, kX11Batch, uint32_t(count), &sink, s.stream));
    return count;
  }

  uint64_t launch_sha_v(Batch& s, const JobTemplate& job, const HitSink& sink) {
    const bool two = group->nvar == kSha256dV2Group;
    Sha256dParamsV vp = group->v_params;
    vp.target_hi = load_le32(job.target + 28);
    const size_t table_bytes = size_t(group->nvar) * sizeof(Sha256dVariant);
    std::memcpy(s.h_vars, group->v_table, table_bytes);
    OTD_HIP(hipMemcpyAsync(s.d_vars, s.h_vars, table_bytes, hipMemcpyHostToDevice, s.stream));
    const uint64_t count =
        launch_count(LaunchKind::kVersionParallel, m.batch_, launch_cap(job), group->nvar, 0, cursor.nonce_off);
    OTD_HIP(launch_sha256d_search_v(vp, s.d_vars, uint32_t(cursor.nonce_off), count, sink, two ? grid_v2 : grid_v,
                                    s.stream, 256, two ? 2 : 1));
    return count;
  }

  uint64_t launch_sha_k(Batch& s, const JobTemplate& job, const HitSink& sink) {
    Sha256dParamsK p;
    const uint8_t* hs[kSha256dMaxK];
    for (int j = 0; j < group->nvar; ++j) hs[j] = group->header[j];
    if (!sha256d_prepare_k(hs, group->nvar, job.target, &p)) throw std::runtime_error("sha256d_prepare_k");
    const uint64_t count =
        launch_count(LaunchKind::kVariantK, m.batch_, launch_cap(job), group->nvar, 0, cursor.nonce_off);
    OTD_HIP(launch_sha256d_search_k(p, uint32_t(cursor.nonce_off), count, sink, grid_k, s.stream));
    return count;
  }

  uint64_t launch_sha_single(Batch& s, const JobTemplate& job, const HitSink& sink) {
    Sha256dParams p;
    sha256d_prepare(group->header[0], job.target, &p);
    const uint64_t count = launch_count(LaunchKind::kSingle, m.batch_, launch_cap(job), 1, 0, cursor.nonce_off);
    OTD_HIP(launch_sha256d_search(p, uint32_t(cursor.nonce_off), count, sink, m.grid_, s.stream));
    return count;
  }

  void enqueue(Batch& s, const JobPtr& job, uint64_t gen, const Batch* prev) {
    hipStream_t stream = s.stream;
    if (!group || group->gen != gen || group->k != cursor.k) group = build_group(job, gen);
    s.job = job;
    s.group = group;
    s.gen = gen;
    s.nvar = group->nvar;
    s.epoch = epoch;
    s.tag = ++tag == 0 ? ++tag : tag;
    s.consumed = 0;
    s.started = false;
    s.range = trace_start(job->algo == Algo::kScrypt ? "otd.scrypt.batch"
                          : job->algo == Algo::kX11  ? "otd.x11.batch"
                                                     : "otd.sha256d.batch");
    HitSink sink;
    sink.out = s.d_count;
    sink.ring = s.ring_dev;
    sink.abort = d_abort;
    sink.cap = kHitCap;
    sink.tag = s.tag;
    sink.epoch = s.epoch;
    sink.words = 2;
    const bool shared_buf = (job->algo == Algo::kScrypt && !scrypt_halves) || (job->algo == Algo::kX11 && !x11_overlap);
    if (prev && prev->busy && shared_buf) OTD_HIP(hipStreamWaitEvent(stream, prev->done, 0));
    OTD_HIP(hipMemsetAsync(s.d_count, 0, 64, stream));
    OTD_HIP(hipEventRecord(s.start, stream));
    __atomic_store_n(s.h_clk, 0ull, __ATOMIC_RELEASE);
    hipLaunchKernelGGL(otd_rt_probe, dim3(1), dim3(64), 0, stream, s.d_clk);
    OTD_HIP(hipGetLastError());
    s.clk_pending = true;
    s.enq_host = monotonic_seconds();
    s.rt_enq = uint32_t(uint64_t((s.enq_host - rt_offset) * kRtHz));
    s.count = job->algo == Algo::kScrypt ? launch_scrypt(s, *job, sink)
              : job->algo == Algo::kX11  ? launch_x11(s, *job, sink)
              : group->use_v             ? launch_sha_v(s, *job, sink)
              : group->nvar > 1          ? launch_sha_k(s, *job, sink)
                                         : launch_sha_single(s, *job, sink);
    OTD_HIP(hipMemcpyAsync(s.h_count, s.d_count, sizeof(uint32_t), hipMemcpyDeviceToHost, stream));
    OTD_HIP(hipEventRecord(s.done, stream));
    s.busy = true;
    cursor.advance(s.count, group->nvar);
    std::lock_guard<std::mutex> g(m.stats_mu_);
    m.stats_.variant_epoch = job->epoch;
    m.stats_.launch_hashes = s.count * uint64_t(s.nvar);
    m.stats_.variant_next = cursor.variant_next(job->variant_start, job->variant_stride, group->nvar);
  }

  bool retire_completed(const JobPtr& job, uint64_t gen) {
    bool progressed = false;
    for (auto it = fifo.begin(); it != fifo.end();) {
      Batch& b = slots[*it];
      const hipError_t q = hipEventQuery(b.done);
      if (q == hipErrorNotReady) { ++it; continue; }
      OTD_HIP(q);
      if (!b.started) b.started = true;
      finish(b, job, gen);
      it = fifo.erase(it);
      progressed = true;
    }
    return progressed;
  }

  void record_switch(const JobPtr& job) {
    for (int i : fifo) {
      Batch& b = slots[i];
      if (b.epoch != epoch) continue;
      const hipError_t q = hipEventQuery(b.start);
      if (q == hipErrorNotReady) break;
      OTD_HIP(q);
      b.started = true;
      const double ms = (monotonic_seconds() - switch_t0) * 1e3;
      switch_pending = false;
      std::lock_guard<std::mutex> g(m.stats_mu_);
      MinerStats& st = m.stats_;
      if (first_switch) {
        first_switch = false;
        double before = 0;
        for (const auto& kv : st.startup_ms) before += kv.second;
        st.startup_ms.emplace_back("wait_first_job", std::max(0.0, (switch_t0 - t_loop) * 1e3 - before));
        st.startup_ms.emplace_back("first_batch", ms);
      }
      st.job_switches += 1;
      st.last_job_switch_ms = ms;
      st.job_switch_ms.push_back(ms);
      if (st.job_switch_ms.size() > 64) st.job_switch_ms.erase(st.job_switch_ms.begin());
      st.work_started.emplace_back(job ? job->epoch : 0, switch_t0 + ms * 1e-3);
      if (st.work_started.size() > 64) st.work_started.erase(st.work_started.begin());
      break;
    }
  }

  bool fill(const JobPtr& job, uint64_t gen) {
    bool progressed = false;
    while (job && (int)fifo.size() < kInflight) {
      const uint64_t v = job->variant_start + cursor.k * job->variant_stride;
      if (v >= job->variant_space()) break;
      if (job->algo == Algo::kScrypt && scrypt_halves && fifo.size() == 1) {
        const Batch& only = slots[fifo.front()];
        if (only.epoch == epoch && monotonic_seconds() - only.enq_host < 0.5 * scrypt_hash_s) break;
      }
      int free_slot = -1;
      for (int i = 0; i < kInflight; ++i)
        if (!slots[i].busy) { free_slot = i; break; }
      if (free_slot < 0) break;
      enqueue(slots[free_slot], job, gen, fifo.empty() ? nullptr : &slots[fifo.back()]);
      fifo.push_back(free_slot);
      progressed = true;
    }
    return progressed;
  }

  void drain_inflight() {
    if (!fifo.empty()) {
      ++epoch;
      try {
        write_abort(epoch);
      } catch (const std::exception&) {
      }
    }
    uint64_t gen = 0;
    auto job = m.peek_job(&gen, nullptr);
    while (!fifo.empty()) {
      Batch& b = slots[fifo.front()];
      OTD_HIP(hipEventSynchronize(b.done));
      finish(b, job, gen);
      fifo.pop_front();
    }
  }

  void run() {
    trace_name_thread(("otedama-" + m.device_id_).c_str());
    t_phase = t_loop = monotonic_seconds();
    OTD_HIP(hipSetDevice(m.device_));
    OTD_HIP(hipFree(nullptr));
    phase("hip_set_device");
    setup_streams();
    setup_abort_word();
    phase("streams");
    setup_buffers();
    for (int t = 0; t < 8; ++t) probe_clock(slots[0].stream);
    phase("clock_calibration");
    OTD_HIP(hipEventCreate(&ref_ev.h));
    OTD_HIP(hipEventRecord(ref_ev, slots[0].stream));
    verifier = std::thread([this] { verify_loop(); });

    while (m.running_.load()) {
      uint64_t gen = 0;
      auto job = check_epoch(&gen);
      if (job && gen != cur_gen) { cur_gen = gen; cursor.reset(); }
      bool progressed = false;
      for (int i : fifo)
        if (slots[i].clk_pending) clock_seen(slots[i]);
      for (int i : fifo) progressed |= drain_ring(slots[i], ~0u, job, gen) > 0;
      progressed |= retire_completed(job, gen);
      if (switch_pending) record_switch(job);
      progressed |= fill(job, gen);
      if (!progressed) {
        if (!job && fifo.empty()) {
          uint64_t g2 = 0;
          (void)m.current_job(&g2);
        } else {
          std::this_thread::sleep_for(kIdlePoll);
        }
      }
    }
    drain_inflight();
  }
};

void GpuMiner::loop() { Run(*this).run(); }


static HitSink ops_sink(uintptr_t out, uint32_t cap, uint32_t words) {
  HitSink s;
  s.out = reinterpret_cast<uint32_t*>(out);
  s.cap = cap;
  s.words = words;
  return s;
}

void py_launch_sha256d(const Sha256dParams& p, uint32_t base, uint64_t count, uintptr_t out, uint32_t cap, int grid,
                       uintptr_t stream) {
  OTD_HIP(launch_sha256d_search(p, base, count, ops_sink(out, cap, 1), grid, reinterpret_cast<hipStream_t>(stream)));
}

void py_launch_sha256d_k(const Sha256dParamsK& p, uint32_t base, uint64_t count, uintptr_t out, uint32_t cap, int grid,
                         uintptr_t stream) {
  OTD_HIP(launch_sha256d_search_k(p, base, count, ops_sink(out, cap, 2), grid, reinterpret_cast<hipStream_t>(stream)));
}

void py_launch_sha256d_v(const Sha256dParamsV& p, uintptr_t vars, uint32_t base, uint64_t count, uintptr_t out,
                         uint32_t cap, int grid, uintptr_t stream, int block, int chains) {
  OTD_HIP(launch_sha256d_search_v(p, reinterpret_cast<const Sha256dVariant*>(vars), base, count,
                                  ops_sink(out, cap, 2), grid, reinterpret_cast<hipStream_t>(stream), block, chains));
}

void py_launch_scrypt(const ScryptParams& p, uint32_t base, uint32_t count, uintptr_t xbuf, uintptr_t scratch, int gap,
                      uintptr_t out, uint32_t cap, int grid, uintptr_t stream) {
  OTD_HIP(launch_scrypt_search(p, base, count, reinterpret_cast<void*>(xbuf), reinterpret_cast<void*>(scratch), gap,
                               ops_sink(out, cap, 1), grid, reinterpret_cast<hipStream_t>(stream)));
}

void py_launch_x11_stage(const X11Params& p, int stage, uint32_t base, uintptr_t H, uint32_t stride, uint32_t n,
                         uintptr_t out, uint32_t cap, uintptr_t stream) {
  const HitSink s = ops_sink(out, cap, 1);
  OTD_HIP(x11_launch_stage(stage, p, base, reinterpret_cast<uint64_t*>(H), stride, n, out ? &s : nullptr,
                           reinterpret_cast<hipStream_t>(stream)));
}

void py_launch_x11(const X11Params& p, uint32_t base, uintptr_t H, uint32_t stride, uint32_t n, uintptr_t out,
                   uint32_t cap, uintptr_t stream) {
  const HitSink s = ops_sink(out, cap, 1);
  OTD_HIP(x11_launch_chain(p, base, reinterpret_cast<uint64_t*>(H), stride, n, out ? &s : nullptr,
                           reinterpret_cast<hipStream_t>(stream)));
}

int gpu_device_count() {
  int n = 0;
  if (hipGetDeviceCount(&n) != hipSuccess) return 0;
  return n;
}

std::string gpu_arch_name(int device) {
  hipDeviceProp_t prop;
  if (hipGetDeviceProperties(&prop, device) != hipSuccess) return "";
  return prop.gcnArchName;
}

int gpu_cu_count(int device) {
  hipDeviceProp_t prop;
  if (hipGetDeviceProperties(&prop, device) != hipSuccess) return 0;
  return prop.multiProcessorCount;
}

}
```

otedama_amd/engine/devproc.py:

```python
from __future__ import annotations

import collections
import os
import select
import signal
import socket
import struct
import subprocess
import sys
import threading
import time

import msgpack

ROOT = os.path.dirname(os.path.dirname(os.path.dirname(os.path.abspath(__file__))))
STATS_PERIOD = 0.5
_HDR = struct.Struct("<I")
MAX_FRAME = 64 << 20

_CUMULATIVE = ("hashes", "candidates", "shares", "dropped", "launches", "rejected_candidates", "variant_launches",
               "busy_seconds", "job_switches", "aborted_launches", "ring_hits", "ring_overflow", "verify_dropped")


def _send(sock: socket.socket, obj, lock: threading.Lock | None = None) -> None:
    data = msgpack.packb(obj, use_bin_type=True)
    frame = _HDR.pack(len(data)) + data
    if lock is None:
        sock.sendall(frame)
    else:
        with lock:
            sock.sendall(frame)


class _Framer:
    def __init__(self):
        self.buf = bytearray()

    def feed(self, data: bytes) -> list:
        self.buf += data
        out = []
        while len(self.buf) >= 4:
            (n,) = _HDR.unpack_from(self.buf)
            if n > MAX_FRAME:
                raise ValueError(f"frame of {n} bytes exceeds {MAX_FRAME}")
            if len(self.buf) < 4 + n:
                break
            out.append(msgpack.unpackb(bytes(self.buf[4 : 4 + n]), raw=False))
            del self.buf[: 4 + n]
        return out


DEVICE_HW_QUEUES = ""


class DeviceProcess:

    def __init__(self, device_index: int, device_id: str, batch_nonces: int = 1 << 32, grid: int = 1536,
                 queue_cap: int = 4096, sha_variants: int = 128, cpu_threads: int = 0, log=None,
                 on_exit=None, on_ready=None, env: dict | None = None):
        self.device_index = device_index
        self.device_id = device_id
        self.args = {"batch": batch_nonces, "grid": grid, "queue_cap": queue_cap, "sha_variants": sha_variants,
                     "cpu_threads": cpu_threads}
        self.log = log or (lambda level, msg: None)
        self.on_exit = on_exit
        self.on_ready = on_ready
        self.env = env
        self._lock = threading.Lock()
        self._send_lock = threading.Lock()
        self._shares: collections.deque = collections.deque()
        self._efd = os.eventfd(0, os.EFD_NONBLOCK | os.EFD_CLOEXEC)
        self._job: dict | None = None
        self._proc: subprocess.Popen | None = None
        self._sock: socket.socket | None = None
        self._reader: threading.Thread | None = None
        self._child: dict = {}
        self._base = {k: 0 for k in _CUMULATIVE}
        self._stopping = False
        self.exit_code: int | None = None
        self.error = ""
        self.restarts = 0
        self.ready_at = 0.0
        self.spawned_at = 0.0
        self.startup_seconds = 0.0
        self.first_hash_wall = 0.0
        self.child_timing: dict = {}
        self.native_startup_ms: dict = {}

    def start(self) -> None:
        self._spawn()

    def _spawn(self) -> None:
        parent, child = socket.socketpair(socket.AF_UNIX, socket.SOCK_STREAM)
        env = dict(os.environ if self.env is None else self.env)
        env["OTEDAMA_NO_TORCH"] = "1"
        env["PYTHONPATH"] = ROOT + (os.pathsep + env["PYTHONPATH"] if env.get("PYTHONPATH") else "")
        hwq = env.get("OTEDAMA_DEVICE_HW_QUEUES", DEVICE_HW_QUEUES)
        if hwq and "GPU_MAX_HW_QUEUES" not in env:
            env["GPU_MAX_HW_QUEUES"] = str(hwq)
        a = self.args
        cmd = [sys.executable, "-m", "otedama_amd.engine.devproc", "--fd", str(child.fileno()),
               "--device", str(self.device_index), "--id", self.device_id, "--batch", str(a["batch"]),
               "--grid", str(a["grid"]), "--queue-cap", str(a["queue_cap"]), "--sha-variants", str(a["sha_variants"]),
               "--cpu-threads", str(a["cpu_threads"])]
        self.spawned_at = time.monotonic()
        self._proc = subprocess.Popen(cmd, pass_fds=(child.fileno(),), env=env, cwd=ROOT)
        child.close()
        self._sock = parent
        self.exit_code = None
        self.error = ""
        self._stopping = False
        self._child = {}
        self._reader = threading.Thread(target=self._read_loop, args=(parent, self._proc),
                                        name=f"otedama-devproc-{self.device_id}", daemon=True)
        self._reader.start()
        if self._job is not None:
            self._post({"op": "job", "t": self._job})

    def stop(self) -> None:
        self._stopping = True
        self._post({"op": "stop"})
        p = self._proc
        if p is not None:
            try:
                p.wait(timeout=10)
            except subprocess.TimeoutExpired:
                p.kill()
                p.wait()
        if self._reader is not None:
            self._reader.join(timeout=5)
        if self._sock is not None:
            try:
                self._sock.close()
            except OSError:
                pass

    def restart(self, replay_job: bool = True) -> bool:
        if self.alive:
            return False
        if not replay_job:
            self._job = None
        with self._lock:
            for k in _CUMULATIVE:
                self._base[k] += self._child.get(k, 0)
            self._child = {}
        self.restarts += 1
        self._spawn()
        return True

    def kill(self, sig: int = signal.SIGKILL) -> None:
        if self._proc is not None and self._proc.poll() is None:
            self._proc.send_signal(sig)

    @property
    def alive(self) -> bool:
        return self._proc is not None and self._proc.poll() is None and self.exit_code is None

    @property
    def pid(self) -> int:
        return self._proc.pid if self._proc is not None else 0

    def set_job(self, template: dict | None) -> None:
        self._job = dict(template) if template is not None else None
        self._post({"op": "job", "t": self._job, "sent": time.monotonic()})

    def poll(self, max_items: int = 256) -> list[dict]:
        out = []
        with self._lock:
            while self._shares and len(out) < max_items:
                out.append(self._shares.popleft())
        return out

    def share_fd(self) -> int:
        return self._efd

    def stats(self) -> dict:
        with self._lock:
            st = dict(self._child)
            for k in _CUMULATIVE:
                st[k] = self._base[k] + st.get(k, 0)
        st.setdefault("error", "")
        st.setdefault("faulted", False)
        if self.exit_code is not None:
            st["faulted"] = True
            st["error"] = self.error
        st["process_restarts"] = self.restarts
        st["pid"] = self.pid
        st["startup_seconds"] = self.startup_seconds
        st["first_hash_wall"] = self.first_hash_wall
        st["child_timing"] = dict(self.child_timing)
        st["native_startup_ms"] = dict(self.native_startup_ms)
        return st

    def _post(self, obj) -> None:
        s = self._sock
        if s is None:
            return
        try:
            _send(s, obj, self._send_lock)
        except OSError:
            pass

    def _read_loop(self, sock: socket.socket, proc: subprocess.Popen) -> None:
        fr = _Framer()
        while True:
            try:
                data = sock.recv(1 << 20)
            except OSError:
                data = b""
            if not data:
                break
            try:
                msgs = fr.feed(data)
            except ValueError as exc:
                self.log("error", f"devproc {self.device_id}: bad frame: {exc}")
                break
            for m in msgs:
                op = m.get("op")
                if op == "shares":
                    with self._lock:
                        self._shares.extend(m["s"])
                    os.eventfd_write(self._efd, 1)
                elif op == "stats":
                    with self._lock:
                        self._child = m["st"]
                elif op == "first_hash":
                    self.first_hash_wall = float(m.get("wall", 0.0))
                    self.child_timing = {"main": m.get("t_main", 0.0), "native_loaded": m.get("t_native", 0.0),
                                         "miner_started": m.get("t_started", 0.0), "first_job": m.get("t_job", 0.0),
                                         "first_hash": self.first_hash_wall}
                    self.native_startup_ms = dict(m.get("native_ms") or {})
                elif op == "ready":
                    self.ready_at = time.monotonic()
                    self.startup_seconds = self.ready_at - self.spawned_at
                    if self.on_ready is not None:
                        self.on_ready(self)
        try:
            sock.close()
        except OSError:
            pass
        try:
            rc = proc.wait(timeout=10)
        except subprocess.TimeoutExpired:
            proc.kill()
            rc = proc.wait()
        if proc is not self._proc:
            return
        last_err = self._child.get("error", "")
        self.exit_code = rc
        self.error = (f"device process exited with code {rc}" if rc >= 0 else
                      f"device process killed by signal {-rc}") + (f": {last_err}" if last_err else "")
        if not self._stopping:
            self.log("error", f"devproc {self.device_id}: {self.error}")
            if self.on_exit is not None:
                self.on_exit(self)


def _child(argv: list[str]) -> int:
    import argparse

    ap = argparse.ArgumentParser(prog="otedama_amd.engine.devproc")
    ap.add_argument("--fd", type=int, required=True)
    ap.add_argument("--device", type=int, required=True)
    ap.add_argument("--id", required=True)
    ap.add_argument("--batch", type=int, default=1 << 32)
    ap.add_argument("--grid", type=int, default=1536)
    ap.add_argument("--queue-cap", type=int, default=4096)
    ap.add_argument("--sha-variants", type=int, default=128)
    ap.add_argument("--cpu-threads", type=int, default=0, help="> 0: a native CpuMiner instead of a GPU (tests)")
    a = ap.parse_args(argv)
    t_main = time.time()
    os.environ["OTEDAMA_NO_TORCH"] = "1"
    sock = socket.socket(fileno=a.fd)
    from otedama_amd.ops.native import require_native

    N = require_native()
    t_native = time.time()
    if a.cpu_threads > 0:
        m = N.CpuMiner(a.cpu_threads, a.id, a.queue_cap)
    else:
        m = N.GpuMiner(a.device, a.id, batch_nonces=a.batch, grid=a.grid, queue_cap=a.queue_cap,
                       sha_variants=a.sha_variants)
    m.start()
    t_started = time.time()
    t_job = 0.0
    _send(sock, {"op": "ready", "pid": os.getpid()})
    efd = m.share_fd()
    poller = select.poll()
    poller.register(sock.fileno(), select.POLLIN)
    poller.register(efd, select.POLLIN)
    fr = _Framer()
    hops: collections.deque = collections.deque(maxlen=64)
    next_stats = 0.0
    first_hash = False
    rc = 0
    try:
        while True:
            timeout = max(0.0, next_stats - time.monotonic())
            if not first_hash:
                timeout = min(timeout, 0.005)
            for fd, _ev in poller.poll(timeout * 1e3):
                if fd == efd:
                    try:
                        os.read(efd, 8)
                    except BlockingIOError:
                        pass
                    shares = m.poll(4096)
                    if shares:
                        _send(sock, {"op": "shares", "s": shares})
                    continue
                data = sock.recv(1 << 20)
                if not data:
                    return 0
                for msg in fr.feed(data):
                    if msg.get("op") == "job":
                        m.set_job(msg.get("t"))
                        if msg.get("sent"):
                            hops.append((time.monotonic() - float(msg["sent"])) * 1e3)
                        t_job = t_job or time.time()
                    elif msg.get("op") == "stop":
                        return 0
            if not first_hash and (m.stats()["job_switches"] > 0 or m.stats()["hashes"] > 0):
                first_hash = True
                _send(sock, {"op": "first_hash", "wall": time.time(), "t_main": t_main, "t_native": t_native,
                             "t_started": t_started, "t_job": t_job,
                             "native_ms": dict(m.stats().get("startup_ms", {}))})
                next_stats = 0.0
            if time.monotonic() >= next_stats:
                st = m.stats()
                st["job_hop_ms"] = list(hops)
                _send(sock, {"op": "stats", "st": st})
                next_stats = time.monotonic() + STATS_PERIOD
                if st.get("faulted"):
                    rc = 3
                    return rc
    except (BrokenPipeError, ConnectionResetError):
        return 0
    finally:
        m.stop()
        shares = m.poll(1 << 16)
        if shares:
            try:
                _send(sock, {"op": "shares", "s": shares})
            except OSError:
                pass
        try:
            st = m.stats()
            st["job_hop_ms"] = list(hops)
            _send(sock, {"op": "stats", "st": st})
        except OSError:
            pass


if __name__ == "__main__":
    sys.exit(_child(sys.argv[1:]))
```

otedama_amd/parallel/comm_probe.py:

```python
from __future__ import annotations

import contextlib
import statistics
import sys
import time


def _say(msg: str) -> None:
    print(f"[comm_probe] {msg}", file=sys.stderr, flush=True)


def _q(xs: list[float]) -> dict:
    xs = sorted(xs)
    n = len(xs)

    def at(p):
        return xs[min(max(int(p * n + 0.5) - 1, 0), n - 1)] if n else None

    return {"p50_ms": at(0.5), "p99_ms": at(0.99), "max_ms": xs[-1] if n else None, "samples": n}


def _miner_rate(dp, t0: tuple[int, float], t1: tuple[int, float]) -> float | None:
    (h0, d0), (h1, d1) = t0, t1
    return (h1 - h0) / (d1 - d0) if d1 > d0 > 0 and h1 > h0 else None


def _counter(dp) -> tuple[int, float]:
    st = dp.stats()
    return int(st.get("hashes", 0)), float(st.get("hashes_done_at_s", 0.0) or 0.0)


def run_ops(comm, seconds: float, cadence_hz: float = 50.0, probe_kernel: bool = True) -> dict:
    import torch

    lat: dict[str, list[float]] = {"R1_job": [], "R2_gather": [], "R3_counters": [], "kernel": []}
    job = {"job_id": "probe", "header": bytes(80), "coinb1": bytes(2000), "coinb2": bytes(2000),
           "merkle_branches": [bytes(32)] * 12, "epoch": 1}
    shares = [{"epoch": 1, "nonce": i, "ntime": 1, "version": 2, "extranonce2": 3, "found_at": time.monotonic()}
              for i in range(4)]
    x = torch.zeros(1 << 12, dtype=torch.float32, device=comm.dev) if comm.stream is not None else None
    period = 1.0 / cadence_hz
    end = time.monotonic() + seconds
    k = 0
    nxt = time.monotonic()
    while time.monotonic() < end:
        k += 1
        t = time.perf_counter()
        if k % 10 == 0:
            comm.broadcast_job(job)
            lat["R1_job"].append((time.perf_counter() - t) * 1e3)
        elif k % 25 == 0:
            comm.gather_counters([1, 2, 3, 4])
            lat["R3_counters"].append((time.perf_counter() - t) * 1e3)
        else:
            comm.gather_shares(shares)
            lat["R2_gather"].append((time.perf_counter() - t) * 1e3)
        if probe_kernel and x is not None and k % 5 == 0:
            t = time.perf_counter()
            with torch.cuda.stream(comm.stream):
                x.add_(1.0)
            comm.stream.synchronize()
            lat["kernel"].append((time.perf_counter() - t) * 1e3)
        nxt += period
        time.sleep(max(0.0, nxt - time.monotonic()))
    return {k: _q(v) for k, v in lat.items() if v}


CONFIGS = {"legacy": {"pg_high": False, "staging": "legacy", "stream_priority": None},
           "node": {"pg_high": True, "staging": "stream", "stream_priority": "high"},
           "native": {"native": True}}


def _one_rank_group(device, high: bool) -> None:
    import torch.distributed as dist

    opts = None
    if high:
        opts = dist.ProcessGroupNCCL.Options()
        opts.is_high_priority_stream = True
    dist.init_process_group("nccl", store=dist.HashStore(), rank=0, world_size=1, device_id=device,
                            pg_options=opts)


def _with_config(dev, device_index: int, name: str, fn):
    import torch.distributed as dist

    from otedama_amd.parallel.comm import DistInfo, NodeComm

    cfg = CONFIGS[name]
    if cfg.get("native"):
        return _with_native(device_index, fn)
    _one_rank_group(dev, cfg["pg_high"])
    try:
        comm = NodeComm(DistInfo(0, 1, device_index, "nccl", dev), bounded=True, deadline=10.0, force=True,
                        stream_priority=cfg["stream_priority"], staging=cfg["staging"])
        run_ops(comm, 0.3)
        return fn(comm)
    finally:
        dist.destroy_process_group()


_NATIVE_GEN = [0]


def _with_native(device_index: int, fn):
    from otedama_amd.parallel.commbase import Device, DistInfo
    from otedama_amd.parallel.kvclient import StoreClient
    from otedama_amd.parallel.kvstore import StoreServer
    from otedama_amd.parallel.rcclcomm import NativeNodeComm

    with StoreServer() as srv:
        info = DistInfo(0, 1, device_index, "rccl", Device("cuda", device_index),
                        store=StoreClient("127.0.0.1", srv.port, timeout=30))
        comm = NativeNodeComm(info, bounded=True, deadline=10.0, force=True)
        _NATIVE_GEN[0] += 1
        comm.reform([0], _NATIVE_GEN[0])
        try:
            run_ops(comm, 0.3)
            return fn(comm)
        finally:
            comm.close()


def measure_comm_under_load(device_index: int = 0, algorithms=("sha256d", "scrypt"), seconds: float = 4.0,
                            cadence_hz: float = 50.0, windows: int = 2, reserves=("",), variants=()) -> dict:
    import torch
    import torch.distributed as dist

    from otedama_amd import hal
    from otedama_amd.engine.latency_probe import _switch_job
    from otedama_amd.engine.miners import MinerSet

    if dist.is_initialized():
        raise RuntimeError("the comm probe needs the default process group to itself")
    dev = torch.device(f"cuda:{device_index}")
    torch.cuda.set_device(dev)
    _say("idle phase")
    out: dict = {"idle": {c: _with_config(dev, device_index, c, lambda comm: run_ops(comm, seconds, cadence_hz))
                          for c in CONFIGS},
                 "configs": CONFIGS, "rccl_world": 1, "cadence_hz": cadence_hz,
                 "definition": ("rank-process call -> result on the host for R1 (64 KiB job blob), R2 (share slots "
                                "all_gather) and R3 (counters all_gather) of a forced one-rank RCCL group; 'kernel' = "
                                "a 16 KiB elementwise kernel on the comm stream, enqueue -> done")}
    devs = [d for d in hal.KFDDriver().enumerate() if d.index == device_index]
    if not devs:
        raise RuntimeError(f"no KFD GPU node for device {device_index}")
    import os

    runs = [(algo, f"reserve:{spec}" if spec else "", {"OTEDAMA_RESERVE_CUS": spec} if spec else {})
            for spec in reserves for algo in algorithms]
    runs += [(algo, v, dict(kv.split("=", 1) for kv in v.split("&"))) for v in variants for algo in algorithms]
    for algo, tag, env in runs:
        key = algo if not tag else f"{algo}@{tag}"
        configs = list(CONFIGS) if not tag else ["native"]
        _say(f"{key}: miner up, alternating windows")
        saved = {k: os.environ.get(k) for k in env}
        os.environ.update(env)
        ms = MinerSet(devs, algo, 1 << 32, 0, isolation="process")
        dp = ms.miners[0].native
        ms.start()
        try:
            end = time.monotonic() + 60
            while not dp.ready_at and dp.alive and time.monotonic() < end:
                time.sleep(0.01)
            ms.set_job(_switch_job(0, algo))
            time.sleep(3.0 if algo == "scrypt" else 1.5)
            res: dict = {"loaded": {}, "rate_alone": [], "rate_with_ops": {c: [] for c in configs}}
            for w in range(windows):
                a = _counter(dp)
                time.sleep(seconds)
                res["rate_alone"].append(_miner_rate(dp, a, _counter(dp)))
                for c in configs:
                    def window(comm, c=c, w=w):
                        a = _counter(dp)
                        r = run_ops(comm, seconds, cadence_hz)
                        res["rate_with_ops"][c].append(_miner_rate(dp, a, _counter(dp)))
                        if w == 0:
                            res["loaded"][c] = r

                    _with_config(dev, device_index, c, window)
            st = dp.stats()
            if st.get("faulted"):
                raise RuntimeError(st.get("error"))
            res["reserved_cus"] = st.get("reserved_cus", 0)
        finally:
            ms.stop()
            for k, v in saved.items():
                if v is None:
                    os.environ.pop(k, None)
                else:
                    os.environ[k] = v
        alone = [r for r in res["rate_alone"] if r]
        base = statistics.fmean(alone) if alone else None
        res["rate_alone_hps"] = base
        res["rate_loss_pct"] = {c: (100.0 * (1.0 - statistics.fmean([r for r in v if r]) / base)
                                    if base and any(v) else None) for c, v in res["rate_with_ops"].items()}
        out[key] = res
    return out


NODE_COMM_DEFINITION = (
    "every rank in lockstep on the run's data plane (bench.py preflight.data_plane): R1 = the node's 64 KiB job-blob "
    "broadcast, R2 = its share-slot all_gather (64 x 10 int64 per rank), R3 = its counter all_reduce, each host call -> "
    "result on the host; R2_dev = bench.py's device-resident hit-slot gather, enqueue -> stream done. Ops interleaved "
    "R1,R2,R3,R2_dev at `cadence_hz` from a common barrier. Phases: idle, then with every rank's device process mining "
    "the named algorithm (the production miner, one per GPU). miner_rate_change_pct = node-wide miner rate with the ops "
    "against an equal window without them. busbw: one all_gather of `busbw_bytes` in total (device buffers), "
    "busbw = bytes/time x (N-1)/N as nccl-tests defines it")


def _lockstep_ops(comm, ops: int, cadence_hz: float, dev) -> dict:
    import torch

    from otedama_amd.parallel.commbase import SHARE_SLOTS

    job = {"job_id": "comm", "header": bytes(80), "coinb1": bytes(2000), "coinb2": bytes(2000),
           "merkle_branches": [bytes(32)] * 12, "epoch": 1}
    shares = [{"epoch": 1, "nonce": i, "ntime": 1, "version": 2, "extranonce2": 3, "found_at": time.monotonic()}
              for i in range(4)]
    world = comm.info.world_size
    slot = torch.zeros(1 + 2 * SHARE_SLOTS, dtype=torch.int32, device=dev)
    gathered = torch.zeros(world, slot.numel(), dtype=torch.int32, device=dev)
    cuda = dev.type == "cuda"
    lat: dict[str, list[float]] = {"R1": [], "R2": [], "R3": [], "R2_dev": []}
    names = list(lat)
    comm.barrier()
    t0 = time.monotonic()
    period = 1.0 / cadence_hz
    for k in range(4 * ops):
        time.sleep(max(0.0, t0 + k * period - time.monotonic()))
        op = names[k % 4]
        t = time.perf_counter()
        if op == "R1":
            comm.broadcast_job(job)
        elif op == "R2":
            comm.gather_shares(shares)
        elif op == "R3":
            comm.allreduce_counters(1, 2, 3, 4)
        else:
            stream = comm.stream if cuda else None
            with torch.cuda.stream(stream) if stream is not None else contextlib.nullcontext():
                comm.gather_tensor(gathered, slot)
            if stream is not None:
                stream.synchronize()
            elif cuda:
                torch.cuda.synchronize(dev)
        lat[op].append((time.perf_counter() - t) * 1e3)
    return {k: _q(v) for k, v in lat.items()}


def _busbw(comm, dev, total_bytes: int, iters: int = 5) -> dict:
    import torch

    world, rank = comm.info.world_size, comm.info.rank
    per = max(4096, (total_bytes // world) // 4096 * 4096)
    send = torch.full((per,), (rank + 1) & 0xFF, dtype=torch.uint8, device=dev)
    recv = torch.zeros(world, per, dtype=torch.uint8, device=dev)

    def sync():
        if dev.type == "cuda":
            torch.cuda.synchronize(dev)

    comm.gather_tensor(recv, send)
    sync()
    ok = all(int(recv[r, 0]) == (r + 1) & 0xFF and int(recv[r, -1]) == (r + 1) & 0xFF for r in range(world))
    comm.barrier()
    sync()
    t0 = time.perf_counter()
    for _ in range(iters):
        comm.gather_tensor(recv, send)
    sync()
    t = comm.allreduce_max((time.perf_counter() - t0) / iters)
    ok = comm.allreduce_counters(int(ok))[0] == world
    algbw = per * world / t / 1e9
    return {"bytes": per * world, "iters": iters, "ms": t * 1e3, "algbw_gbps": algbw,
            "busbw_gbps": algbw * (world - 1) / world, "blocks_ok": ok, "device": dev.type}


def _start_miner(device_index: int, algo: str):
    from otedama_amd import hal
    from otedama_amd.engine.latency_probe import _switch_job
    from otedama_amd.engine.miners import MinerSet

    devs = [d for d in hal.KFDDriver().enumerate() if d.index == device_index]
    if not devs:
        raise RuntimeError(f"no KFD GPU node for device {device_index}")
    ms = MinerSet(devs, algo, 1 << 32, 0, isolation="process")
    dp = ms.miners[0].native
    ms.start()
    end = time.monotonic() + 60
    while not dp.ready_at and dp.alive and time.monotonic() < end:
        time.sleep(0.01)
    if not dp.ready_at:
        ms.stop()
        raise RuntimeError(f"{algo} device process not ready")
    ms.set_job(_switch_job(0, algo))
    return ms, dp


def measure_node_comm(comm, dev, phases=("idle", "sha256d", "scrypt"), ops: int = 200, cadence_hz: float = 100.0,
                      busbw_bytes: int = 256 << 20, rate_window_s: float = 3.0, warm_s: dict | None = None,
                      say=None) -> dict:
    say = say or (lambda m: None)
    world = comm.info.world_size
    warm_s = warm_s or {"sha256d": 1.5, "scrypt": 3.0}
    out: dict = {"world": world, "ops_per_type": ops, "cadence_hz": cadence_hz, "definition": NODE_COMM_DEFINITION}
    rates: dict = {}
    for ph in phases:
        if ph == "idle":
            say("comm: idle ops")
            out["idle"] = _lockstep_ops(comm, ops, cadence_hz, dev)
            continue
        say(f"comm: {ph} miner up")
        ms = dp = None
        err = ""
        try:
            ms, dp = _start_miner(dev.index or 0, ph)
            time.sleep(warm_s.get(ph, 2.0))
        except Exception as exc:
            err = f"{type(exc).__name__}: {exc}"[:200]
        try:
            if comm.allreduce_counters(int(ms is not None))[0] != world:
                out[ph] = {"skipped": err or "a peer's miner did not start"}
                continue
            comm.barrier()
            a = _counter(dp)
            time.sleep(rate_window_s)
            alone = _miner_rate(dp, a, _counter(dp)) or 0.0
            a = _counter(dp)
            res = _lockstep_ops(comm, ops, cadence_hz, dev)
            with_ops = _miner_rate(dp, a, _counter(dp)) or 0.0
            st = dp.stats()
            res["miner_rate_alone_hps"], res["miner_rate_with_ops_hps"] = alone, with_ops
            res["miner_faulted"] = bool(st.get("faulted"))
            out[ph] = res
            rates[ph] = (alone, with_ops)
        finally:
            if ms is not None:
                ms.stop()
    if rates:
        change = {}
        for ph, (alone, with_ops) in rates.items():
            tot_alone, tot_with, _, _ = comm.allreduce_counters(int(alone), int(with_ops))
            change[ph] = round(100.0 * (tot_with / tot_alone - 1.0), 2) if tot_alone > 0 else None
        out["miner_rate_change_pct"] = change
    if busbw_bytes > 0:
        say("comm: bus bandwidth")
        out["busbw"] = _busbw(comm, dev, busbw_bytes)
    return out


def main(argv=None) -> int:
    import argparse
    import json

    ap = argparse.ArgumentParser(prog="otedama_amd.parallel.comm_probe")
    ap.add_argument("--device", type=int, default=0)
    ap.add_argument("--algorithms", default="sha256d,scrypt")
    ap.add_argument("--seconds", type=float, default=4.0)
    ap.add_argument("--cadence", type=float, default=50.0)
    ap.add_argument("--windows", type=int, default=2)
    ap.add_argument("--reserves", default="", help="';'-separated OTEDAMA_RESERVE_CUS specs besides none, e.g. '0;0,32'")
    ap.add_argument("--variants", default="",
                    help="';'-separated miner environments, e.g. 'OTEDAMA_SCRYPT_SEGMENTS=8;OTEDAMA_SCRYPT_SEGMENTS=16'")
    a = ap.parse_args(argv)
    reserves = [""] + [x for x in a.reserves.split(";") if x]
    r = measure_comm_under_load(a.device, [x for x in a.algorithms.split(",") if x], a.seconds, a.cadence, a.windows,
                                reserves, [x for x in a.variants.split(";") if x])
    print(json.dumps(r))
    return 0


if __name__ == "__main__":
    raise SystemExit(main())
```

otedama_amd/parallel/node.py:

```python
from __future__ import annotations

import collections
import json
import os
import random
import select
import socket
import threading
import time

from otedama_amd.engine.miners import GROUP, RESPLIT_GROUPS, MinerSet
from otedama_amd.parallel.commbase import SHARE_SLOTS, SHARE_WORDS, pack_shares, unpack_shares
from otedama_amd.utils.trace import span

DEFAULT_TICK = 0.005
HB_INTERVAL = 0.5
HB_TIMEOUT = 2.0
LIVENESS_EVERY = 0.25
STATS_INTERVAL = 10.0
BELL_FALLBACK = 0.05
PREVIEW_GRACE = 0.02
PENDING_CAP = 8192
OP_RETAIN = 4096
EPOCH_SHIFT = 40
PREFIX = "otd/"
PREVIEW_MAX = 60000
SEEN_MAX = 65536
SEEN_TTL = 120.0


def share_preview_msgs(shares: list[dict], orig_rank: int) -> list[bytes]:
    out = []
    for i in range(0, len(shares), SHARE_SLOTS):
        part = shares[i:i + SHARE_SLOTS]
        rows = pack_shares(part, orig_rank)[: len(part)]
        out.append(b"p" + orig_rank.to_bytes(2, "little") + rows.tobytes())
    return out


def parse_share_preview(msg: bytes) -> list[dict]:
    body = msg[3:]
    if msg[:1] != b"p" or not body or len(body) % (8 * SHARE_WORDS):
        return []
    import numpy as np

    orig = int.from_bytes(msg[1:3], "little")
    rows = np.frombuffer(body, dtype=np.int64).reshape(1, -1, SHARE_WORDS)
    return unpack_shares(rows, [orig])


def share_key(s: dict) -> int:
    return hash((s["orig_rank"], s["epoch"], s["nonce"], s.get("ntime", 0), s.get("version", 0),
                 s.get("extranonce2", 0)))


def op_retain() -> int:
    try:
        return max(16, int(os.environ.get("OTEDAMA_NODE_OP_RETAIN", OP_RETAIN)))
    except ValueError:
        return OP_RETAIN


def _k(*parts) -> str:
    return PREFIX + "/".join(str(p) for p in parts)


def _store_get(store, key: str, timeout: float | None = None):
    try:
        if not store.check([key]):
            return None
        if timeout is None or not hasattr(store, "set_timeout"):
            return store.get(key)
        import datetime

        prev = getattr(store, "timeout", None)
        store.set_timeout(datetime.timedelta(seconds=timeout))
        try:
            return store.get(key)
        finally:
            if prev is not None:
                store.set_timeout(prev)
    except Exception:
        return None


def _clone(store):
    return store.clone() if hasattr(store, "clone") else store


class _Bell:

    PORT_TTL = 2.0
    DROP = float(os.environ.get("OTEDAMA_FAULT_BELL_DROP", "0") or 0)

    def __init__(self, store, orig_rank: int):
        self.sock = socket.socket(socket.AF_INET, socket.SOCK_DGRAM)
        self.sock.bind(("127.0.0.1", 0))
        self.sock.setblocking(False)
        self.port = self.sock.getsockname()[1]
        self.orig = orig_rank
        self.store = _clone(store) if store is not None else None
        self._lock = threading.Lock()
        self._ports: dict = {}
        self.rings = 0
        self.dropped = 0
        if self.store is not None:
            self.store.set(_k("bell", orig_rank), str(self.port))

    def _port_of(self, orig: int) -> int | None:
        if orig == self.orig:
            return self.port
        now = time.monotonic()
        with self._lock:
            hit = self._ports.get(orig)
            if hit is not None and now - hit[1] < self.PORT_TTL:
                return hit[0]
            raw = _store_get(self.store, _k("bell", orig)) if self.store is not None else None
            if raw is None:
                return hit[0] if hit else None
            port = int(raw)
            self._ports[orig] = (port, now)
            return port

    def port_at(self, key: str) -> int | None:
        now = time.monotonic()
        with self._lock:
            hit = self._ports.get(key)
            if hit is not None and now - hit[1] < self.PORT_TTL:
                return hit[0]
            raw = _store_get(self.store, key) if self.store is not None else None
            if raw is None:
                return hit[0] if hit else None
            port = int(raw)
            self._ports[key] = (port, now)
            return port

    def ring(self, orig: int, kind: bytes = b"o") -> None:
        port = self._port_of(orig)
        if port is None:
            return
        if self.DROP and random.random() < self.DROP:
            self.dropped += 1
            return
        try:
            self.sock.sendto(kind, ("127.0.0.1", port))
            self.rings += 1
        except OSError:
            pass

    def send_port(self, port: int, msg: bytes) -> bool:
        if self.DROP and random.random() < self.DROP:
            self.dropped += 1
            return False
        try:
            self.sock.sendto(msg, ("127.0.0.1", port))
            return True
        except OSError:
            return False

    def wait(self, timeout: float) -> list[bytes]:
        got: list[bytes] = []
        try:
            ready, _, _ = select.select([self.sock], [], [], max(timeout, 0.0))
        except (OSError, ValueError):
            return got
        if ready:
            while True:
                try:
                    got.append(self.sock.recv(65536))
                except (BlockingIOError, OSError):
                    break
        return got

    def close(self) -> None:
        try:
            self.sock.close()
        except OSError:
            pass


def op_msg(k: int, raw: str) -> bytes:
    return b"o" + k.to_bytes(8, "little") + raw.encode()


def parse_op_msg(msg: bytes) -> tuple[int, dict] | None:
    if len(msg) <= 9 or msg[:1] != b"o":
        return None
    try:
        return int.from_bytes(msg[1:9], "little"), json.loads(msg[9:])
    except ValueError:
        return None


class _Heartbeat:

    def __init__(self, store, orig_rank: int, local: MinerSet, comm: NodeComm | None = None):
        self._origin = store
        self.store = _clone(store)
        self.failures = 0
        self.orig = orig_rank
        self.local = local
        self.comm = comm
        self.extra: dict = {}
        self.stop = threading.Event()
        self.th = threading.Thread(target=self._loop, name=f"otedama-hb-{orig_rank}", daemon=True)

    def start(self):
        self.th.start()

    def payload(self) -> dict:
        st = list(self.local.device_stats().values())
        return {"t": time.time(), "hw": self.local.high_water(), "ep": self.local.epoch,
                "hashes": sum(s["hashes"] for s in st), "shares": sum(s["shares"] for s in st),
                "dropped": sum(s["dropped"] for s in st), "faulted": sum(1 for s in st if s["faulted"]),
                "done": st[0].get("hashes_done_at_s", 0.0) if len(st) == 1 else 0.0,
                "coll": self.comm.collectives if self.comm is not None else 0,
                "ws": sorted(tuple(x) for s in st for x in (s.get("work_started") or []))[-8:],
                "gen": self.comm.info.generation if self.comm is not None else 0,
                "pid": os.getpid(), **self.extra}

    def _loop(self):
        while not self.stop.is_set():
            try:
                self.store.set(_k("hb", self.orig), json.dumps(self.payload()))
            except Exception:
                self.failures += 1
                try:
                    self.store = _clone(self._origin)
                except Exception:
                    pass
            self.stop.wait(HB_INTERVAL)


class _Link:

    def __init__(self, local: MinerSet, comm: NodeComm, log):
        self.local = local
        self.comm = comm
        self.log = log
        self.store = comm.info.store
        self.rows: list[list[int]] = [[0, 0, 0, 0] for _ in range(comm.info.world_size)]
        self.error: BaseException | None = None
        self.tick_seconds: collections.deque = collections.deque(maxlen=1024)
        self.ops_run = 0
        self.reforms = 0

    @property
    def rank(self) -> int:
        return self.comm.info.rank

    @property
    def world(self) -> int:
        return self.comm.info.world_size

    @property
    def tick(self) -> float:
        return DEFAULT_TICK

    def local_counters(self) -> list[int]:
        st = self.local.device_stats().values()
        return [sum(s["hashes"] for s in st), sum(s["shares"] for s in st), sum(s["dropped"] for s in st),
                sum(1 for s in st if s["faulted"])]

    def run_op(self, op: dict, blob, outgoing: list[dict]):
        t0 = time.perf_counter()
        kind = op["op"]
        job, shares = None, None
        try:
            with span(f"otd.node.{kind}"):
                if kind == "job":
                    job = self.comm.broadcast_job(blob)
                elif kind == "gather":
                    shares = self.comm.gather_shares(outgoing)
                elif kind == "stats":
                    self.rows = self.comm.gather_counters(self.local_counters())
                elif kind == "reform":
                    self.comm.reform(list(op["members"]), int(op["gen"]))
                    self.local.set_rank(self.comm.info.rank, self.comm.info.world_size)
                    self.rows = [[0, 0, 0, 0] for _ in range(self.comm.info.world_size)]
                    self.reforms += 1
        finally:
            self.tick_seconds.append(time.perf_counter() - t0)
            self.ops_run += 1
        return job, shares

    def tick_quantile(self, q: float) -> float:
        xs = sorted(self.tick_seconds)
        if not xs:
            return 0.0
        return xs[min(len(xs) - 1, int(q * len(xs)))]


class NodeMinerSet:

    def __init__(self, local: MinerSet, comm: NodeComm, tick: float = DEFAULT_TICK, log=None,
                 stats_interval: float = STATS_INTERVAL, hb_timeout: float = HB_TIMEOUT):
        comm.bounded = True
        self.local = local
        self.comm = comm
        self.log = log or (lambda level, msg: None)
        self.link = _Link(local, comm, self.log)
        self.tick = tick
        self.stats_interval = stats_interval
        self.hb_timeout = hb_timeout
        self.algorithm = local.algorithm
        self.store = comm.info.store
        self._lock = threading.Lock()
        self._bell = _Bell(self.store, comm.info.orig_rank) if self.store is not None else None
        self._wake = threading.Event()
        self._gather_wanted = False
        self._seq = 0
        self._sent_seq = 0
        self._stop = False
        self._blob: dict | None = None
        self._template: dict | None = None
        self._epoch = 0
        self._variant_base = 0
        self._paused: set[str] = set()
        self._jobs: dict[int, dict] = {}
        self._remote = collections.deque(maxlen=65536)
        self._remote_efd = os.eventfd(0, os.EFD_NONBLOCK | os.EFD_CLOEXEC)
        self._seen: collections.OrderedDict = collections.OrderedDict()
        self._take_lock = threading.Lock()
        self.share_previews = 0
        self.share_gathered_first = 0
        self.previews_refused = 0
        self._spv: socket.socket | None = None
        self._spv_thread: threading.Thread | None = None
        self._thread: threading.Thread | None = None
        self._op_k = 0
        self._retain = op_retain()
        self._gen = comm.info.generation
        self._gen_started = time.monotonic()
        self.capacity = max(comm.info.capacity, comm.info.world_size, 1)
        self.takeover = comm.info.generation < 0
        self.incarnation = int(self.store.add(_k("leader_inc"), 1)) if self.store is not None else 1
        self._epoch = (self.incarnation - 1) << EPOCH_SHIFT
        self._seq = (self.incarnation - 1) << EPOCH_SHIFT
        local._epoch = max(local._epoch, self._epoch)
        self.remote_stale = 0
        self._rows_by_orig: dict[int, list[int]] = {}
        self.row_times: dict[int, float] = {}
        self.row_done_at: dict[int, float] = {}
        self._prev_rows: dict[int, list[int]] = {}
        self._hb_pairs: dict[int, tuple[int, float]] = {}
        self._prev_pairs: dict[int, tuple[int, float]] = {}
        self._exact: dict[int, bool] = {}
        self._rates: dict[str, float] = {}
        self._t_last = time.monotonic()
        self._remote_faults: dict[int, int] = {}
        self._remote_idle: dict[int, int] = {}
        self.lost_ranks: list[int] = []
        self._fail_at = 0.0
        self._hb = _Heartbeat(self.store, comm.info.orig_rank, local, comm) if self.store is not None else None
        self.job_set_at: collections.deque = collections.deque(maxlen=64)
        self.job_bcast_at: collections.deque = collections.deque(maxlen=64)

    @property
    def remote_ids(self) -> list[str]:
        return [f"rank{r}" for r in range(1, self.capacity)]

    def __len__(self) -> int:
        return len(self.local) * max(self.comm.info.world_size, 1)

    @property
    def miners(self):
        return self.local.miners

    @property
    def epoch(self) -> int:
        return self._epoch

    def start(self) -> None:
        self.local.start()
        if self._hb is not None:
            self._hb.start()
        if self.store is not None and not self.takeover:
            self.store.set(_k("next"), "0")
            self.store.set(_k("gen"), str(self._gen))
        if self.store is not None and self.capacity > 1:
            self._spv = socket.socket(socket.AF_INET, socket.SOCK_DGRAM)
            self._spv.bind(("127.0.0.1", 0))
            self._spv.setsockopt(socket.SOL_SOCKET, socket.SO_RCVBUF, 4 << 20)
            self._spv.setblocking(False)
            self.store.set(_k("spv"), str(self._spv.getsockname()[1]))
            self._spv_thread = threading.Thread(target=self._spv_loop, name="otedama-node-spv", daemon=True)
            self._spv_thread.start()
        self._thread = threading.Thread(target=self._loop, name="otedama-node-r0", daemon=True)
        self._thread.start()

    def stop(self) -> None:
        with self._lock:
            self._stop = True
        self._poke()
        if self._thread is not None:
            self._thread.join(timeout=30)
            self._thread = None
        if self._hb is not None:
            self._hb.stop.set()
        if self._spv_thread is not None:
            self._spv_thread.join(timeout=2)
            self._spv_thread = None
        if self._spv is not None:
            self._spv.close()
            self._spv = None
        self.local.stop()
        if self._bell is not None:
            self._bell.close()

    def _poke(self) -> None:
        self._wake.set()
        if self._bell is not None:
            self._bell.ring(self._bell.orig, b"w")

    def set_job(self, template: dict | None) -> int:
        with self._lock:
            self._template = dict(template) if template is not None else None
            if template is not None and self._variant_base:
                from otedama_amd.engine.miners import _work_key

                if _work_key(template) != getattr(self, "_work_key", None):
                    self._variant_base = 0
            if template is not None:
                from otedama_amd.engine.miners import _work_key

                self._work_key = _work_key(template)
            ep = self.local.set_job(self._with_base(self._template))
            self._epoch = ep
            self.job_set_at.append((ep, time.monotonic()))
            if template is not None:
                self._jobs[ep] = {"job_id": template.get("job_id", ""), "channel_id": template.get("channel_id", 0),
                                  "extranonce2_size": int(template.get("extranonce2_size", 0) or 0)}
                for old in [e for e in self._jobs if e < ep - 64]:
                    del self._jobs[old]
            self._publish()
            preview = self._blob if template is not None else None
        self._poke()
        if preview is not None:
            self._preview(preview)
        return ep

    def _preview(self, blob: dict) -> None:
        if self._bell is None or self.comm.info.world_size <= 1:
            return
        from otedama_amd.parallel.commbase import _encode

        msg = b"j" + json.dumps({"gen": self._gen, "blob": _encode(blob)}).encode()
        if len(msg) > PREVIEW_MAX:
            return
        for r in list(self.comm.info.members):
            if r != self.comm.info.orig_rank:
                self._bell.ring(r, msg)

    def _with_base(self, template: dict | None) -> dict | None:
        if template is None or not self._variant_base:
            return template
        return dict(template, variant_base=self._variant_base)

    def _publish(self) -> None:
        blob = None
        if self._template is not None:
            blob = {k: v for k, v in self._template.items() if k not in ("variant_start", "variant_stride")}
            blob["epoch"] = self._epoch
            if self._variant_base:
                blob["variant_base"] = self._variant_base
        self._seq += 1
        self._blob = {"job": blob, "paused": sorted(self._paused), "seq": self._seq}

    def pause_device(self, device_id: str, paused: bool = True) -> bool:
        if self.local.pause_device(device_id, paused):
            return True
        if device_id in self.remote_ids:
            with self._lock:
                if paused:
                    self._paused.add(device_id)
                else:
                    self._paused.discard(device_id)
                self._publish()
            self._poke()
            return True
        return False

    def pause_all(self) -> None:
        self.set_job(None)

    def poll(self, max_per_device: int = 256) -> list[dict]:
        out = self.local.poll(max_per_device)
        n = max_per_device * max(self.capacity - 1, 1)
        while self._remote and n > 0:
            out.append(self._remote.popleft())
            n -= 1
        return out

    def share_fds(self) -> list[int]:
        return list(self.local.share_fds()) + [self._remote_efd]

    def device_stats(self) -> dict[str, dict]:
        d = dict(self.local.device_stats())
        for r in range(1, self.capacity):
            row = self._rows_by_orig.get(r, [0, 0, 0, 0])
            lost = r in self.lost_ranks
            d[f"rank{r}"] = {"hashes": row[0], "shares": row[1], "dropped": row[2], "faulted": bool(row[3]) or lost,
                             "error": "rank lost" if lost else ("remote device fault" if row[3] else ""),
                             "candidates": 0, "launches": 0, "counted_at": self.row_times.get(r, 0.0),
                             "hashes_done_at_s": self.row_done_at.get(r, 0.0)}
        return d

    def total_hashes(self) -> int:
        return self.local.total_hashes() + sum(r[0] for o, r in self._rows_by_orig.items() if o != 0)

    def total_dropped(self) -> int:
        return self.local.total_dropped() + sum(r[2] for o, r in self._rows_by_orig.items() if o != 0)

    def faulted(self) -> list[tuple[str, str]]:
        out = self.local.faulted()
        for r in range(1, self.capacity):
            if r in self.lost_ranks:
                out.append((f"rank{r}", "rank lost"))
            elif self._rows_by_orig.get(r, [0, 0, 0, 0])[3]:
                out.append((f"rank{r}", "remote device fault"))
        return out

    def retire_faulted(self) -> list[tuple[str, str]]:
        out = self.local.retire_faulted()
        for r in range(1, self.capacity):
            n = self._rows_by_orig.get(r, [0, 0, 0, 0])[3]
            if n > self._remote_faults.get(r, 0):
                out.append((f"rank{r}", f"{n - self._remote_faults.get(r, 0)} device(s) faulted on rank{r}"))
                self._remote_faults[r] = n
        return out

    def stalled(self) -> list[str]:
        stall = self.local.stall_samples
        return self.local.stalled() + [f"rank{r}" for r, n in self._remote_idle.items() if n >= stall]

    def live(self):
        return self.local.live()

    def update_hashrates(self) -> dict[str, float]:
        rates = self.local.update_hashrates()
        now = time.monotonic()
        dt = max(now - self._t_last, 1e-6)
# ... 550 lines not shown
```

otedama_amd/parallel/rcclcomm.py:

```python
from __future__ import annotations

import importlib
import os
import time

import numpy as np

from otedama_amd.parallel.commbase import (COUNTER_WORDS, JOB_BLOB_BYTES, PG_TIMEOUT_S, SHARE_SLOTS, SHARE_WORDS,
                                           CollectiveTimeout, Device, DistInfo, job_from_payload, job_payload,
                                           pack_shares, unpack_shares)

COMM_KEY = "otd/comm"
FAILED_ID = b"!"
_HOSTED_SERVER = None


class NativeNodeComm:

    def __init__(self, info: DistInfo, bounded: bool = True, deadline: float = 3.0, force: bool = False,
                 device_stream: bool = False):
        self._rccl = rccl_module()
        self.info = info
        self.bounded = bounded
        self.deadline = deadline
        self.force = force
        self.collectives = 0
        self.stream = None
        self.dev = info.device
        if device_stream and getattr(info.device, "type", "cpu") == "cuda":
            import torch

            if not isinstance(info.device, torch.device):
                info.device = torch.device(info.device.type, info.device.index)
            self.dev = info.device
            lo, hi = torch.cuda.Stream.priority_range()
            self.stream = torch.cuda.Stream(self.dev, priority=min(lo, hi))
        self._rc = None
        self._job_h = np.zeros(JOB_BLOB_BYTES, dtype=np.uint8)

    @property
    def multi(self) -> bool:
        return self.info.world_size > 1 or self.force

    def bind_thread(self) -> None:
        """Nothing to do: every native op selects the comm's device itself."""

    def close(self) -> None:
        self.abort()

    def abort(self) -> None:
        rc, self._rc = self._rc, None
        if rc is not None:
            try:
                rc.abort()
            except Exception:
                pass

    def reform(self, members: list[int], generation: int, timeout: float | None = None) -> None:
        info = self.info
        if info.orig_rank not in members:
            raise ValueError(f"rank {info.orig_rank} is not a member of generation {generation}")
        self.abort()
        timeout = PG_TIMEOUT_S if timeout is None else timeout
        rank, world = members.index(info.orig_rank), len(members)
        if world > 1 or self.force:
            key = f"otd-g{generation}/rcclid"
            if rank == 0:
                try:
                    uid = self._rccl.unique_id()
                except Exception:
                    if info.store is not None:
                        info.store.set(key, FAILED_ID)
                    raise
                if info.store is not None:
                    info.store.set(key, uid)
            else:
                uid = _wait_get(info.store, key, timeout)
                if uid == FAILED_ID:
                    raise RuntimeError(f"generation {generation}: the group's rank 0 could not create an RCCL id")
            self._rc = self._rccl.RcclComm(int(info.device.index or 0), world, rank, uid, timeout)
        info.rank, info.world_size, info.generation, info.members = rank, world, generation, list(members)

    def _timeout(self) -> float:
        return self.deadline if self.bounded else PG_TIMEOUT_S

    def _call(self, fn, *args):
        if self._rc is None:
            raise RuntimeError("rccl: no communicator for this generation")
        self.collectives += 1
        try:
            return fn(*args, self._timeout())
        except TimeoutError as exc:
            raise CollectiveTimeout(str(exc)) from None

    def broadcast_job(self, job: dict | None) -> dict | None:
        if self.info.is_primary:
            buf = job_payload(job)
        else:
            buf = b""
        if self.multi:
            buf = self._call(self._rc.broadcast, buf, JOB_BLOB_BYTES, 0)
        return job_from_payload(buf)

    def gather_shares(self, shares: list[dict], device_index: int = 0) -> list[dict]:
        rows = pack_shares(shares, self.info.rank, device_index)
        if self.multi:
            raw = self._call(self._rc.all_gather, rows.tobytes())
            g = np.frombuffer(raw, dtype=np.int64).reshape(-1, SHARE_SLOTS, SHARE_WORDS)
        else:
            g = rows[None]
        return unpack_shares(g, self.info.members)

    def allreduce_counters(self, hashes: int, shares: int = 0, dropped: int = 0, faults: int = 0) -> tuple:
        v = np.array([hashes, shares, dropped, faults], dtype=np.int64)
        if self.multi:
            v = np.frombuffer(self._call(self._rc.all_reduce, v.tobytes(), "i64", "sum"), dtype=np.int64)
        return tuple(int(x) for x in v)

    def gather_counters(self, values: list[int]) -> list[list[int]]:
        v = np.array(list(values)[:COUNTER_WORDS] + [0] * (COUNTER_WORDS - len(values)), dtype=np.int64)
        if self.multi:
            raw = self._call(self._rc.all_gather, v.tobytes())
            return np.frombuffer(raw, dtype=np.int64).reshape(-1, COUNTER_WORDS).tolist()
        return [v.tolist()]

    def broadcast_control(self, words: list[int]) -> list[int]:
        v = np.array(list(words)[:4] + [0] * (4 - len(words)), dtype=np.int64)
        if self.multi:
            raw = self._call(self._rc.broadcast, v.tobytes() if self.info.is_primary else b"", 32, 0)
            v = np.frombuffer(raw, dtype=np.int64)
        return v.tolist()

    def allreduce_max(self, value: float) -> float:
        v = np.array([value], dtype=np.float64)
        if self.multi:
            v = np.frombuffer(self._call(self._rc.all_reduce, v.tobytes(), "f64", "max"), dtype=np.float64)
        return float(v[0])

    def barrier(self) -> None:
        if self.multi:
            self.allreduce_counters(0)

    def _cur_stream(self) -> int:
        if getattr(self.dev, "type", "cpu") != "cuda":
            return 0
        import torch

        return torch.cuda.current_stream(self.dev).cuda_stream

    def gather_tensor(self, out, inp) -> None:
        if not self.multi or (self.info.world_size == 1 and os.environ.get("OTEDAMA_RCCL_LOCAL_R2") == "1"):
            out[0].copy_(inp)
            return
        if self._rc is None:
            raise RuntimeError("rccl: no communicator for this generation")
        self.collectives += 1
        self._rc.all_gather_dev(inp.data_ptr(), out.data_ptr(), inp.numel() * inp.element_size(), self._cur_stream(),
                                self._timeout())

    def broadcast_tensor(self, t, src: int = 0) -> None:
        if not self.multi:
            return
        if self._rc is None:
            raise RuntimeError("rccl: no communicator for this generation")
        self.collectives += 1
        self._rc.broadcast_dev(t.data_ptr(), t.numel() * t.element_size(), src, self._cur_stream(), self._timeout())

    def run_async(self, fn):
        if self.stream is None:
            fn()
            return None
        import torch

        cur = torch.cuda.current_stream(self.dev)
        self.stream.wait_stream(cur)
        with torch.cuda.stream(self.stream):
            fn()
        ev = torch.cuda.Event()
        ev.record(self.stream)
        return ev


def rccl_module():
    name = os.environ.get("OTEDAMA_RCCL_MODULE")
    if name:
        return importlib.import_module(name)
    from otedama_amd import _rccl

    return _rccl


def cpu_standin() -> bool:
    return bool(os.environ.get("OTEDAMA_RCCL_MODULE")) and getattr(rccl_module(), "DEVICE_TYPE", "cuda") == "cpu"


def _rank_device(local: int) -> Device:
    return Device("cpu", None) if cpu_standin() else Device("cuda", local)


def _wait_get(store, key: str, timeout: float) -> bytes:
    end = time.monotonic() + timeout
    while not store.check([key]):
        if time.monotonic() > end:
            raise TimeoutError(f"{key} not published within {timeout:.0f} s")
        time.sleep(0.01)
    return store.get(key)


def native_wanted() -> bool:
    mode = os.environ.get("OTEDAMA_NODE_COMM", "").lower()
    if mode == "torch":
        return False
    if mode == "native":
        return True
    if os.environ.get("OTEDAMA_DIST_BACKEND", "") == "gloo":
        return False
    for var in ("HIP_VISIBLE_DEVICES", "CUDA_VISIBLE_DEVICES", "ROCR_VISIBLE_DEVICES"):
        if os.environ.get(var) == "":
            return False
    from otedama_amd.parallel.launch import visible_gpus_kfd

    return visible_gpus_kfd() > 0


def _store_client(rank: int, world: int):
    global _HOSTED_SERVER
    from otedama_amd.parallel.kvclient import StoreClient

    addr = os.environ.setdefault("MASTER_ADDR", "127.0.0.1")
    port = int(os.environ.get("MASTER_PORT", "29500"))
    hosted = os.environ.get("OTEDAMA_STORE_HOSTED") == "1" or os.environ.get("TORCHELASTIC_USE_AGENT_STORE") == "True"
    if rank == 0 and not hosted and _HOSTED_SERVER is None:
        from otedama_amd.parallel.kvstore import StoreServer

        _HOSTED_SERVER = StoreServer(addr, port)
        os.environ["OTEDAMA_STORE_HOSTED"] = "1"
    return StoreClient(addr, port, timeout=max(PG_TIMEOUT_S, 60.0))


def open_node_comm(joining: bool, host_buffers: bool = False, log=None):
    log = log or (lambda msg: None)
    if not native_wanted():
        return _torch_comm(joining, host_buffers)
    world = int(os.environ.get("WORLD_SIZE", "1"))
    rank = int(os.environ.get("RANK", "0"))
    local = int(os.environ.get("LOCAL_RANK", str(rank)))
    store = _store_client(rank, world)
    if joining:
        mode = _wait_get(store, COMM_KEY, PG_TIMEOUT_S).decode()
        if mode != "rccl":
            store.close()
            return _torch_comm(joining, host_buffers)
        info = DistInfo(-1, 0, local, "rccl", _rank_device(local), orig_rank=rank, generation=-1, members=[],
                        store=store, capacity=world)
        return info, NativeNodeComm(info)
    info = DistInfo(rank, world, local, "rccl", _rank_device(local), store=store, capacity=world)
    comm = None
    err = ""
    try:
        comm = NativeNodeComm(info)
        comm.reform(list(range(world)), 0)
        ok = True
    except Exception as exc:
        ok, err = False, f"{type(exc).__name__}: {exc}"
    store.set(f"otd/g0native/{rank}", "1" if ok else "0")
    flags = [_wait_get(store, f"otd/g0native/{r}", PG_TIMEOUT_S + 10.0) for r in range(world)]
    if all(f == b"1" for f in flags):
        if rank == 0:
            store.set(COMM_KEY, "rccl")
        return info, comm
    log(f"node: native RCCL unavailable on rank(s) {[r for r, f in enumerate(flags) if f != b'1']}"
        + (f" ({err})" if err else "") + "; using torch.distributed")
    if comm is not None:
        comm.abort()
    if rank == 0:
        store.set(COMM_KEY, "torch")
    store.close()
    return _torch_comm(joining, host_buffers)


def _torch_comm(joining: bool, host_buffers: bool):
    from otedama_amd.parallel.comm import NodeComm, init_from_env, join_from_env

    info = join_from_env() if joining else init_from_env()
    if not joining and info.store is not None and info.rank == 0:
        try:
            info.store.set(COMM_KEY, "torch")
        except Exception:
            pass
    return info, NodeComm(info, host_buffers=host_buffers)
```

Measured before the change: 19.29 billion.

## Add preemptible scrypt ROMix kernel that yields wave slots during RCCL collectives

Adds a resumable scrypt ROMix kernel that records per-wave progress and polls a yield word every few iterations, so in-flight batches can give their wave slots back and resume later. The RCCL comm wrapper raises a yield flag on all local miners around each collective and releases it after a stream event completes, so collectives are not starved by long scrypt kernels. It also adds a ds_bpermute variant of the coop shuffle. The aim is to reduce collective and share latency under mining load, at the cost of extra polling, relaunches and progress bookkeeping that can lower raw hash throughput.

```diff
diff --git a/csrc/bindings.cpp b/csrc/bindings.cpp
--- a/csrc/bindings.cpp
+++ b/csrc/bindings.cpp
@@ -119,6 +119,9 @@
   d["verify_queue_peak"] = s.verify_queue_peak;
   d["launch_hashes"] = s.launch_hashes;
   d["aborted_launches"] = s.aborted_launches;
+  d["yields"] = s.yields;
+  d["yield_expired"] = s.yield_expired;
+  d["resumed_launches"] = s.resumed_launches;
   d["ring_hits"] = s.ring_hits;
   d["clock_calib_rtt_us"] = s.clock_calib_rtt_us;
   d["clock_samples"] = s.clock_samples;
@@ -235,6 +238,25 @@
   }, py::arg("kind"), py::arg("batch"), py::arg("cap"), py::arg("nvar") = 1, py::arg("lanes") = 0,
      py::arg("start") = 0, py::arg("max_launches") = size_t(1) << 20, py::arg("variant_start") = 0,
      py::arg("variant_stride") = 1);
+  m.def("_romix_trips", &romix_trips, py::arg("count64"), py::arg("launch_grid"), py::arg("slot_base"));
+  m.def("_romix_progress_words", &romix_progress_words, py::arg("launch_grid"));
+  m.def("_romix_active_waves", &romix_active_waves, py::arg("count64"), py::arg("launch_grid"));
+  m.def("_romix_resume", [](uint32_t progress, uint32_t trips) {
+    const RomixResume r = romix_resume(progress, trips);
+    return py::make_tuple(r.trip, r.it, r.done);
+  }, py::arg("progress"), py::arg("trips"));
+  m.def("_romix_launch_stop", &romix_launch_stop, py::arg("progress"), py::arg("trips"),
+        py::arg("limit") = kRomixIters, py::arg("raised_at") = ~0u);
+  m.def("_romix_batch_complete", &romix_batch_complete, py::arg("finished_waves"), py::arg("count64"),
+        py::arg("launch_grid"));
+  m.def("_yield_step", [](bool aborted, bool complete, bool raised, uint64_t full, double rate_hpms, double ms) {
+    const YieldStep st = yield_step(aborted, complete, raised);
+    const char* name = st == YieldStep::kRetireAborted ? "retire_aborted" : st == YieldStep::kRetireComplete
+                       ? "retire_complete" : st == YieldStep::kResume ? "resume" : "wait";
+    return py::make_tuple(std::string(name), yielded_batch_hashes(st, full, rate_hpms, ms));
+  }, py::arg("aborted"), py::arg("complete"), py::arg("raised"), py::arg("full") = 0, py::arg("rate_hpms") = 0.0,
+     py::arg("ms") = 0.0);
+  m.def("_yield_wanted", &yield_wanted, py::arg("until"), py::arg("now"));
   m.def("_work_queue_flood", [](size_t cap, size_t n, bool hash_each, size_t batch) {
     BoundedWorkQueue<std::array<uint8_t, 80>> q(cap);
     std::atomic<uint64_t> processed{0};
@@ -463,6 +485,22 @@
   }, py::arg("params"), py::arg("base"), py::arg("count"), py::arg("xbuf"), py::arg("scratch"), py::arg("gap"),
      py::arg("out"), py::arg("cap"), py::arg("grid"), py::arg("stream"));
 
+  m.def("launch_scrypt_yield", [](const py::bytes& params, uint32_t base, uint32_t count, uintptr_t xbuf,
+                                  uintptr_t scratch, uintptr_t progress, uint32_t it_end, int stages, uintptr_t abort,
+                                  uintptr_t yield, uint32_t epoch, uintptr_t out, uint32_t cap, int grid,
+                                  int launch_grid, uintptr_t stream) {
+    std::string ps = need(params, sizeof(ScryptParams), "params");
+    ScryptParams p; std::memcpy(&p, ps.data(), sizeof p);
+    if (grid <= 0 || launch_grid <= 0 || launch_grid > grid || out == 0 || xbuf == 0 || scratch == 0 ||
+        progress == 0 || count == 0 || uint64_t(count) > uint64_t(grid) * 256u || (stages & ~7) || stages == 0)
+      throw std::invalid_argument("bad launch args");
+    py_launch_scrypt_yield(p, base, count, xbuf, scratch, progress, it_end, stages, abort, yield, epoch, out, cap,
+                           grid, launch_grid, stream);
+  }, py::arg("params"), py::arg("base"), py::arg("count"), py::arg("xbuf"), py::arg("scratch"), py::arg("progress"),
+     py::arg("it_end") = kRomixIters, py::arg("stages") = 7, py::arg("abort") = 0, py::arg("yield_word") = 0,
+     py::arg("epoch") = 0, py::arg("out") = 0, py::arg("cap") = 0, py::arg("grid") = 0, py::arg("launch_grid") = 0,
+     py::arg("stream") = 0);
+
   m.def("launch_x11_stage", [](const py::bytes& params, int stage, uint32_t base, uintptr_t H, uint32_t stride,
                                uint32_t n, uintptr_t out, uint32_t cap, uintptr_t stream) {
     std::string ps = need(params, sizeof(X11Params), "params");
@@ -503,7 +541,10 @@
   py::class_<GpuMiner, MinerBase, std::shared_ptr<GpuMiner>>(m, "GpuMiner")
       .def(py::init<int, std::string, uint64_t, int, size_t, int>(), py::arg("device"), py::arg("device_id"),
            py::arg("batch_nonces") = (1ull << 32), py::arg("grid") = 2048, py::arg("queue_cap") = 1024,
-           py::arg("sha_variants") = 128);
+           py::arg("sha_variants") = 128)
+      .def("request_yield", &GpuMiner::request_yield, py::arg("timeout_s") = 0.05,
+           "ask the scrypt batches in flight to give their wave slots back (held until release_yield or the timeout)")
+      .def("release_yield", &GpuMiner::release_yield);
   py::class_<CpuMiner, MinerBase, std::shared_ptr<CpuMiner>>(m, "CpuMiner")
       .def(py::init<int, std::string, size_t>(), py::arg("threads"), py::arg("device_id") = "cpu-0",
            py::arg("queue_cap") = 1024);
@@ -511,4 +552,9 @@
   m.attr("SHA256D_PARAMS_SIZE") = sizeof(Sha256dParams);
   m.attr("SHA256D_V_PARAMS_SIZE") = sizeof(Sha256dParamsV);
   m.attr("SCRYPT_PARAMS_SIZE") = sizeof(ScryptParams);
+  m.attr("SCRYPT_STAGE_IN") = kScryptStageIn;
+  m.attr("SCRYPT_STAGE_ROMIX") = kScryptStageRomix;
+  m.attr("SCRYPT_STAGE_OUT") = kScryptStageOut;
+  m.attr("ROMIX_ITERS") = kRomixIters;
+  m.attr("ROMIX_POLL") = kRomixPoll;
 }
diff --git a/csrc/include/otedama/hitsink.h b/csrc/include/otedama/hitsink.h
--- a/csrc/include/otedama/hitsink.h
+++ b/csrc/include/otedama/hitsink.h
@@ -15,6 +15,7 @@
   uint32_t* out = nullptr;
   HitRecord* ring = nullptr;
   const uint32_t* abort = nullptr;
+  const uint32_t* yield = nullptr;
   uint32_t cap = 0;
   uint32_t tag = 0;
   uint32_t epoch = 0;
diff --git a/csrc/include/otedama/launch_plan.h b/csrc/include/otedama/launch_plan.h
--- a/csrc/include/otedama/launch_plan.h
+++ b/csrc/include/otedama/launch_plan.h
@@ -107,4 +107,74 @@
 }
 inline double update_scrypt_hash_s(double scrypt_hash_s, double ms) { return 0.7 * scrypt_hash_s + 0.3e-3 * ms; }
 
+constexpr uint32_t kRomixIters = 2048;
+constexpr uint32_t kRomixWrite = 1024;
+constexpr uint32_t kRomixPoll = 64;
+
+inline uint32_t romix_trips(uint32_t count64, uint32_t launch_grid, uint32_t slot_base) {
+  const uint64_t nslots = uint64_t(launch_grid) * 256u;
+  if (nslots == 0 || slot_base >= count64) return 0;
+  return uint32_t((uint64_t(count64) - slot_base + nslots - 1) / nslots);
 }
+inline uint32_t romix_waves(uint32_t launch_grid) { return launch_grid * 4u; }
+inline uint32_t romix_progress_words(uint32_t launch_grid) { return romix_waves(launch_grid) + 1u; }
+
+struct RomixResume {
+  uint32_t trip = 0, it = 0;
+  bool done = false;
+};
+inline RomixResume romix_resume(uint32_t progress, uint32_t trips) {
+  RomixResume r;
+  r.done = uint64_t(progress) >= uint64_t(trips) * kRomixIters;
+  r.trip = r.done ? trips : progress / kRomixIters;
+  r.it = r.done ? 0 : progress % kRomixIters;
+  return r;
+}
+
+inline uint32_t romix_next_poll(uint32_t it) {
+  const uint32_t phase_end = it < kRomixWrite ? kRomixWrite : kRomixIters;
+  return std::min(it + kRomixPoll, phase_end);
+}
+
+inline uint32_t romix_launch_stop(uint32_t progress, uint32_t trips, uint32_t limit, uint32_t raised_at) {
+  const uint64_t end = uint64_t(trips) * kRomixIters;
+  uint64_t g = progress;
+  while (g < end) {
+    const uint32_t trip = uint32_t(g / kRomixIters), it = uint32_t(g % kRomixIters);
+    if (it >= limit) return uint32_t(g);
+    const uint32_t poll = std::min(romix_next_poll(it), limit);
+    g = uint64_t(trip) * kRomixIters + poll;
+    if (g >= raised_at) return uint32_t(g);
+    if (poll == limit && limit < kRomixIters) return uint32_t(g);
+  }
+  return uint32_t(end);
+}
+
+inline uint32_t romix_active_waves(uint32_t count64, uint32_t launch_grid) {
+  uint32_t n = 0;
+  for (uint32_t w = 0; w < romix_waves(launch_grid); ++w) n += romix_trips(count64, launch_grid, w * 64u) > 0;
+  return n;
+}
+inline bool romix_batch_complete(uint32_t finished_waves, uint32_t count64, uint32_t launch_grid) {
+  return finished_waves >= romix_active_waves(count64, launch_grid);
+}
+
+enum class YieldStep { kRetireAborted, kRetireComplete, kResume, kWait };
+inline YieldStep yield_step(bool aborted, bool complete, bool yield_raised) {
+  if (aborted) return YieldStep::kRetireAborted;
+  if (complete) return YieldStep::kRetireComplete;
+  return yield_raised ? YieldStep::kWait : YieldStep::kResume;
+}
+inline uint64_t yielded_batch_hashes(YieldStep step, uint64_t full, double rate_hpms, double ms) {
+  switch (step) {
+    case YieldStep::kRetireAborted: return aborted_launch_hashes(full, rate_hpms, ms);
+    case YieldStep::kRetireComplete: return full;
+    case YieldStep::kResume:
+    case YieldStep::kWait: break;
+  }
+  return 0;
+}
+
+inline bool yield_wanted(double until, double now) { return until > 0 && now < until; }
+
+}
diff --git a/csrc/include/otedama/runtime.h b/csrc/include/otedama/runtime.h
--- a/csrc/include/otedama/runtime.h
+++ b/csrc/include/otedama/runtime.h
@@ -76,6 +76,9 @@
   uint64_t clock_samples = 0;
   bool host_abort = false;
   uint64_t reserved_cus = 0;
+  uint64_t yields = 0;
+  uint64_t yield_expired = 0;
+  uint64_t resumed_launches = 0;
   double hashes_done_at_s = 0;
   std::vector<std::pair<std::string, double>> startup_ms;
   std::vector<std::pair<std::string, double>> startup_rss_mb;
@@ -140,8 +143,11 @@
   ~GpuMiner() override;
   void start() override;
   void stop() override;
+  void request_yield(double timeout_s);
+  void release_yield();
  private:
   struct Run;
+  std::atomic<double> yield_until_{0.0};
   void loop();
   int device_;
   uint64_t batch_;
diff --git a/csrc/include/otedama/search_launch.h b/csrc/include/otedama/search_launch.h
--- a/csrc/include/otedama/search_launch.h
+++ b/csrc/include/otedama/search_launch.h
@@ -13,6 +13,8 @@
 std::string gpu_arch_name(int device);
 int gpu_cu_count(int device);
 
+constexpr int kScryptStageIn = 1, kScryptStageRomix = 2, kScryptStageOut = 4;
+
 void py_launch_sha256d(const Sha256dParams& p, uint32_t base, uint64_t count, uintptr_t out, uint32_t cap, int grid,
                        uintptr_t stream);
 void py_launch_sha256d_k(const Sha256dParamsK& p, uint32_t base, uint64_t count, uintptr_t out, uint32_t cap, int grid,
@@ -21,6 +23,9 @@
                          uint32_t cap, int grid, uintptr_t stream, int block, int chains);
 void py_launch_scrypt(const ScryptParams& p, uint32_t base, uint32_t count, uintptr_t xbuf, uintptr_t scratch, int gap,
                       uintptr_t out, uint32_t cap, int grid, uintptr_t stream);
+void py_launch_scrypt_yield(const ScryptParams& p, uint32_t base, uint32_t count, uintptr_t xbuf, uintptr_t scratch,
+                            uintptr_t progress, uint32_t it_end, int stages, uintptr_t abort, uintptr_t yield,
+                            uint32_t epoch, uintptr_t out, uint32_t cap, int grid, int launch_grid, uintptr_t stream);
 void py_launch_x11_stage(const X11Params& p, int stage, uint32_t base, uintptr_t H, uint32_t stride, uint32_t n,
                          uintptr_t out, uint32_t cap, uintptr_t stream);
 void py_launch_x11(const X11Params& p, uint32_t base, uintptr_t H, uint32_t stride, uint32_t n, uintptr_t out,
@@ -43,5 +48,9 @@
 hipError_t launch_scrypt_search(const ScryptParams& p, uint32_t base, uint32_t count, void* xbuf, void* scratch,
                                 int gap, const HitSink& sink, int grid, hipStream_t stream);
 
+hipError_t launch_scrypt_yield(const ScryptParams& p, uint32_t base, uint32_t count, void* xbuf, void* scratch,
+                               uint32_t* progress, uint32_t it_end, int stages, const HitSink& sink, int grid,
+                               int launch_grid, hipStream_t stream);
+
 }
 #endif
diff --git a/csrc/kernels/hitsink_dev.h b/csrc/kernels/hitsink_dev.h
--- a/csrc/kernels/hitsink_dev.h
+++ b/csrc/kernels/hitsink_dev.h
@@ -19,11 +19,18 @@
   return __hip_atomic_load(const_cast<uint32_t*>(s.abort), __ATOMIC_RELAXED, __HIP_MEMORY_SCOPE_SYSTEM);
 }
 
+__device__ __forceinline__ uint32_t word_peek_scalar(const uint32_t* word) {
+  uint32_t v;
+  asm volatile("s_load_dword %0, %1, 0x0 glc\n\ts_waitcnt lgkmcnt(0)" : "=s"(v) : "s"(word));
+  return v;
+}
 __device__ __forceinline__ uint32_t abort_peek_scalar(const otedama::HitSink& s) {
   if (s.abort == nullptr) return s.epoch;
-  uint32_t v;
-  asm volatile("s_load_dword %0, %1, 0x0 glc\n\ts_waitcnt lgkmcnt(0)" : "=s"(v) : "s"(s.abort));
-  return v;
+  return word_peek_scalar(s.abort);
+}
+__device__ __forceinline__ bool yield_peek_scalar(const otedama::HitSink& s) {
+  if (s.yield == nullptr) return false;
+  return word_peek_scalar(s.yield) != 0u;
 }
 
 __device__ __forceinline__ bool abort_newer(uint32_t word, uint32_t epoch) {
diff --git a/csrc/kernels/scrypt_search.hip b/csrc/kernels/scrypt_search.hip
--- a/csrc/kernels/scrypt_search.hip
+++ b/csrc/kernels/scrypt_search.hip
@@ -8,6 +8,7 @@
 #include <cstring>
 
 #include "otedama/job.h"
+#include "otedama/launch_plan.h"
 #include "otedama/search_launch.h"
 
 namespace {
@@ -207,7 +208,7 @@
   }
 }
 
-template <int LCPOL>
+template <int LCPOL, bool BPERM = false>
 __device__ __forceinline__ void coop_issue(const uint32_t X[32], __amdgpu_buffer_rsrc_t rs, uint4* __restrict__ tile,
                                            uint32_t lane, coop_v4u R[4]) {
   uint32_t ln = lane;
@@ -219,14 +220,17 @@
   for (int r = 0; r < 4; ++r) {
     const uint32_t chunk = slot ^ (((octet >> 1) & 3u) | (uint32_t(r & 1) << 2));
     const uint32_t o0 = uint32_t(8 * r) + octet, o1 = o0 + 32u;
-    const uint32_t j0 = uint32_t(__shfl(int(j), int(o0), 64));
-    const uint32_t j1 = uint32_t(__shfl(int(j), int(o1), 64));
+    const uint32_t j0 = BPERM ? uint32_t(__builtin_amdgcn_ds_bpermute(int(o0 << 2), int(j)))
+                              : uint32_t(__shfl(int(j), int(o0), 64));
+    const uint32_t j1 = BPERM ? uint32_t(__builtin_amdgcn_ds_bpermute(int(o1 << 2), int(j)))
+                              : uint32_t(__shfl(int(j), int(o1), 64));
     __builtin_amdgcn_raw_ptr_buffer_load_lds(rs, (glds_lptr_t*)(tile + 64 * r), 16, (j0 << 13) | (o0 << 7) | (chunk << 4),
                                              0, 0, LCPOL);
     R[r] = __builtin_amdgcn_raw_buffer_load_b128(rs, (j1 << 13) | (o1 << 7) | (chunk << 4), 0, LCPOL);
   }
 }
 
+template <bool REDO = false>
 __device__ __forceinline__ void coop_consume(uint32_t X[32], uint4* __restrict__ tile, uint32_t lane,
                                              const coop_v4u R[4]) {
   const char* tb = reinterpret_cast<const char*>(tile);
@@ -246,10 +250,12 @@
 #pragma unroll
   for (int r = 0; r < 4; ++r) tile[64 * r + ln] = make_uint4(R[r].x, R[r].y, R[r].z, R[r].w);
   __builtin_amdgcn_wave_barrier();
+  uint32_t rd2 = rd;
+  if constexpr (REDO) asm volatile("" : "+v"(rd2));
   if (ln >= 32u) {
 #pragma unroll
     for (int c = 0; c < 8; ++c) {
-      const uint4 t = *reinterpret_cast<const uint4*>(tb + (rd ^ (uint32_t(c) << 4)));
+      const uint4 t = *reinterpret_cast<const uint4*>(tb + (rd2 ^ (uint32_t(c) << 4)));
       X[4 * c] ^= t.x; X[4 * c + 1] ^= t.y; X[4 * c + 2] ^= t.z; X[4 * c + 3] ^= t.w;
     }
   }
@@ -411,6 +417,82 @@
       blockmix(X);
     }
     store_entry(xbuf + (h << 3), X);
+  }
+}
+
+__device__ __forceinline__ uint32_t lane_now() {
+  uint32_t l;
+  asm volatile("v_mbcnt_lo_u32_b32 %0, -1, 0\n\tv_mbcnt_hi_u32_b32 %0, -1, %0" : "=v"(l));
+  return l;
+}
+
+template <int LCPOL>
+__global__ __launch_bounds__(256) __attribute__((amdgpu_waves_per_eu(8, 8))) void otd_scrypt_romix_coop_yield(
+    uint32_t count, uint4* __restrict__ xbuf, uint4* __restrict__ V, uint32_t* __restrict__ progress, uint32_t it_end,
+    const otedama::HitSink sink) {
+  __shared__ uint4 tiles[4 * 256];
+  const uint32_t slot = blockIdx.x * blockDim.x + threadIdx.x;
+  const uint32_t nslots = gridDim.x * blockDim.x;
+  const uint32_t wave = __builtin_amdgcn_readfirstlane(slot >> 6);
+  uint4* tile = tiles + __builtin_amdgcn_readfirstlane(threadIdx.x >> 6) * 256;
+  const uint32_t base = wave << 6;
+  const uint32_t trips = base < count ? uint32_t((uint64_t(count) - base + nslots - 1u) / nslots) : 0u;
+  const uint32_t g_end = trips * otedama::kRomixIters;
+  const uint32_t g0 = __builtin_amdgcn_readfirstlane(progress[wave]);
+  if (g0 >= g_end) return;
+  if (abort_newer(abort_peek(sink), sink.epoch)) return;
+  uint32_t trip = g0 / otedama::kRomixIters, it0 = g0 % otedama::kRomixIters;
+  uint32_t reached = it0;
+  bool stop = false;
+  while (true) {
+    const uint64_t h = uint64_t(slot) + uint64_t(trip) * nslots;
+    const uint32_t hw = __builtin_amdgcn_readfirstlane(uint32_t(h >> 6));
+    const __amdgpu_buffer_rsrc_t rh =
+        __builtin_amdgcn_make_buffer_rsrc(V + uint64_t(hw) * (1024ull * 64u * 8u), (short)0, 1024 * 64 * 128, 0x00020000);
+    uint32_t X[32];
+    load_entry(xbuf + (h << 3), X);
+    uint32_t lim = it_end < otedama::kRomixIters ? it_end : otedama::kRomixIters;
+    uint32_t w1 = lim < otedama::kRomixWrite ? lim : otedama::kRomixWrite;
+    for (uint32_t c = it0; c < w1;) {
+      const uint32_t e = c + otedama::kRomixPoll < w1 ? c + otedama::kRomixPoll : w1;
+      for (uint32_t i = c; i < e; ++i) {
+        coop_store_entry(X, rh, tile, lane_now(), i);
+        blockmix(X);
+      }
+      c = e;
+      if (abort_newer(abort_peek_scalar(sink), sink.epoch) || yield_peek_scalar(sink)) {
+        stop = true;
+        w1 = e;
+        lim = e;
+      }
+    }
+    for (uint32_t c = it0 > otedama::kRomixWrite ? it0 : otedama::kRomixWrite; c < lim;) {
+      const uint32_t e = c + otedama::kRomixPoll < lim ? c + otedama::kRomixPoll : lim;
+      for (uint32_t i = c; i < e; ++i) {
+        coop_v4u R[4];
+        const uint32_t ln = lane_now();
+        coop_issue<LCPOL, true>(X, rh, tile, ln, R);
+        coop_consume<true>(X, tile, ln, R);
+        blockmix(X);
+      }
+      c = e;
+      if (abort_newer(abort_peek_scalar(sink), sink.epoch) || yield_peek_scalar(sink)) {
+        stop = true;
+        lim = e;
+      }
+    }
+    store_entry(xbuf + (h << 3), X);
+    reached = it0 > lim ? it0 : lim;
+    if (reached < otedama::kRomixIters) break;
+    ++trip;
+    it0 = 0;
+    reached = 0;
+    if (trip >= trips || stop) break;
+  }
+  if (lane_now() == 0) {
+    const uint32_t g = trip * otedama::kRomixIters + reached;
+    progress[wave] = g;
+    if (g >= g_end) atomicAdd(progress + (gridDim.x * 4u), 1u);
   }
 }
 
@@ -458,6 +540,20 @@
                                                                        const otedama::HitSink sink) {
   const uint32_t i = blockIdx.x * blockDim.x + threadIdx.x;
   if (i >= count) return;
+  if (abort_newer(abort_peek(sink), sink.epoch)) return;
+  uint32_t X[32];
+  load_entry(xbuf + (uint64_t(i) << 3), X);
+  const uint32_t h7 = scrypt_pbkdf_out(p, base + i, X);
+  if (bswap(h7) <= p.target_hi) hit_publish(sink, base + i, 0u);
+}
+
+extern "C" __global__ __launch_bounds__(256) void otd_scrypt_pbkdf_out_y(const otedama::ScryptParams p, uint32_t base,
+                                                                         uint32_t count, const uint4* __restrict__ xbuf,
+                                                                         const uint32_t* __restrict__ finished,
+                                                                         uint32_t need, const otedama::HitSink sink) {
+  const uint32_t i = blockIdx.x * blockDim.x + threadIdx.x;
+  if (i >= count) return;
+  if (*finished < need) return;
   if (abort_newer(abort_peek(sink), sink.epoch)) return;
   uint32_t X[32];
   load_entry(xbuf + (uint64_t(i) << 3), X);
@@ -548,4 +644,29 @@
   return hipGetLastError();
 }
 
-}
+hipError_t launch_scrypt_yield(const ScryptParams& p, uint32_t base, uint32_t count, void* xbuf, void* scratch,
+                               uint32_t* progress, uint32_t it_end, int stages, const HitSink& sink, int grid,
+                               int launch_grid, hipStream_t stream) {
+  uint4* X = static_cast<uint4*>(xbuf);
+  uint4* V = static_cast<uint4*>(scratch);
+  const int eg = int((count + 255) / 256);
+  const uint32_t count64 = (count + 63u) & ~63u;
+  if (count == 0 || grid <= 0 || launch_grid <= 0 || launch_grid > grid || progress == nullptr ||
+      uint64_t(count64) > uint64_t(grid) * 256u)
+    return hipErrorInvalidValue;
+  const uint32_t words = romix_progress_words(uint32_t(launch_grid));
+  if (stages & kScryptStageIn) {
+    const hipError_t e = hipMemsetAsync(progress, 0, words * sizeof(uint32_t), stream);
+    if (e != hipSuccess) return e;
+    hipLaunchKernelGGL(otd_scrypt_pbkdf_in, dim3(eg), dim3(256), 0, stream, p, base, count, X);
+  }
+  if (stages & kScryptStageRomix)
+    hipLaunchKernelGGL(otd_scrypt_romix_coop_yield<2>, dim3(launch_grid), dim3(256), 0, stream, count64, X, V, progress,
+                       it_end, sink);
+  if (stages & kScryptStageOut)
+    hipLaunchKernelGGL(otd_scrypt_pbkdf_out_y, dim3(eg), dim3(256), 0, stream, p, base, count, X,
+                       progress + (words - 1u), romix_active_waves(count64, uint32_t(launch_grid)), sink);
+  return hipGetLastError();
+}
+
+}
diff --git a/csrc/runtime/gpu_miner.hip b/csrc/runtime/gpu_miner.hip
--- a/csrc/runtime/gpu_miner.hip
+++ b/csrc/runtime/gpu_miner.hip
@@ -146,6 +146,15 @@
   uint64_t* h_clk = nullptr;
   uint64_t* d_clk = nullptr;
   bool clk_pending = false;
+  DeviceMem<uint32_t> d_progress;
+  bool resumable = false;
+  uint32_t resumes = 0;
+  ScryptParams sp{};
+  uint32_t sbase = 0;
+  void* sxb = nullptr;
+  void* spad = nullptr;
+  int sgrid = 0;
+  HitSink ssink;
   TraceId range = 0;
 };
 
@@ -157,6 +166,13 @@
       sha_variants_(sha_variants) {}
 
 GpuMiner::~GpuMiner() { stop(); }
+
+void GpuMiner::request_yield(double timeout_s) {
+  if (!(timeout_s > 0)) timeout_s = 0.05;
+  yield_until_.store(monotonic_seconds() + std::min(timeout_s, 1.0));
+}
+
+void GpuMiner::release_yield() { yield_until_.store(0.0); }
 
 void GpuMiner::start() {
   if (running_.exchange(true)) return;
@@ -201,6 +217,7 @@
   int scrypt_grid = 0;
   uint32_t scrypt_batch = 0;
   bool scrypt_halves = true, x11_overlap = true;
+  bool scrypt_yield = true;
   bool cap_launches = true;
   int grid_k = 0, grid_v = 0, grid_v2 = 0;
 
@@ -217,6 +234,7 @@
   double switch_t0 = 0;
   double rate_hpms = 0;
   double scrypt_hash_s = 0.064;
+  bool yield_up = false;
   std::deque<int> fifo;
   BoundedWorkQueue<Candidate> vq{kVerifyCap};
   std::thread verifier;
@@ -318,6 +336,12 @@
     scrypt_batch = uint32_t(scrypt_grid) * 256u;
     const char* halves_env = std::getenv("OTEDAMA_SCRYPT_HALVES");
     scrypt_halves = !(halves_env && halves_env[0] == '0');
+    const char* yield_env = std::getenv("OTEDAMA_SCRYPT_YIELD");
+    const char* seg_env = std::getenv("OTEDAMA_SCRYPT_SEGMENTS");
+    scrypt_yield = !(yield_env && yield_env[0] == '0') && !(seg_env && seg_env[0]);
+    if (scrypt_yield)
+      for (auto& s : slots)
+        OTD_HIP(hipMalloc(&s.d_progress.h, romix_progress_words(uint32_t(scrypt_grid)) * sizeof(uint32_t)));
     const char* x11ov_env = std::getenv("OTEDAMA_X11_OVERLAP");
     x11_overlap = !(x11ov_env && x11ov_env[0] == '0');
     const char* cap_env = std::getenv("OTEDAMA_LAUNCH_CAP");
@@ -360,6 +384,27 @@
     } else {
       OTD_HIP(hipStreamWriteValue32(ctl, d_abort, e, 0));
     }
+  }
+
+  uint32_t* yield_word() const { return d_abort.h + 16; }
+  void write_yield(uint32_t v) {
+    if (host_abort) {
+      __atomic_store_n(yield_word(), v, __ATOMIC_RELEASE);
+      _mm_sfence();
+    } else {
+      OTD_HIP(hipStreamWriteValue32(ctl, yield_word(), v, 0));
+    }
+  }
+
+  void check_yield() {
+    const double until = m.yield_until_.load();
+    const bool want = scrypt_yield && yield_wanted(until, monotonic_seconds());
+    if (want == yield_up) return;
+    write_yield(want ? 1u : 0u);
+    yield_up = want;
+    std::lock_guard<std::mutex> g(m.stats_mu_);
+    if (want) m.stats_.yields += 1;
+    else if (until > 0) m.stats_.yield_expired += 1;
   }
 
   JobPtr check_epoch(uint64_t* gen_out) {
@@ -478,8 +523,9 @@
     const uint64_t full = b.count * uint64_t(b.nvar);
     const bool aborted = int32_t(epoch - b.epoch) > 0;
     const uint64_t done_hashes = aborted ? aborted_launch_hashes(full, rate_hpms, ms) : full;
-    if (!aborted && ms > 0) rate_hpms = update_rate_hpms(rate_hpms, full, ms);
-    if (!aborted && ms > 0 && b.job && b.job->algo == Algo::kScrypt)
+    const bool timed = !aborted && ms > 0 && b.resumes == 0;
+    if (timed) rate_hpms = update_rate_hpms(rate_hpms, full, ms);
+    if (timed && b.job && b.job->algo == Algo::kScrypt)
       scrypt_hash_s = update_scrypt_hash_s(scrypt_hash_s, ms);
     std::lock_guard<std::mutex> g(m.stats_mu_);
     if (n > kHitCap) {
@@ -548,6 +594,18 @@
                 (scrypt_halves ? uint64_t(slot_i) * scrypt_scratch_bytes(grid, kScryptGap) : 0);
     char* xb = static_cast<char*>(xbuf.h) + (scrypt_halves ? uint64_t(slot_i) * lanes * 128ull : 0);
     const uint64_t count = launch_count(LaunchKind::kScrypt, m.batch_, launch_cap(job), 1, lanes, cursor.nonce_off);
+    if (scrypt_yield) {
+      s.resumable = true;
+      s.sp = p;
+      s.sbase = uint32_t(cursor.nonce_off);
+      s.sxb = xb;
+      s.spad = pad;
+      s.sgrid = grid;
+      s.ssink = sink;
+      OTD_HIP(launch_scrypt_yield(p, s.sbase, uint32_t(count), xb, pad, s.d_progress, kRomixIters,
+                                  kScryptStageIn | kScryptStageRomix | kScryptStageOut, sink, grid, grid, s.stream));
+      return count;
+    }
     OTD_HIP(launch_scrypt_search(p, uint32_t(cursor.nonce_off), uint32_t(count), xb, pad, kScryptGap, sink, grid,
                                  s.stream));
     return count;
@@ -608,6 +666,8 @@
     s.tag = ++tag == 0 ? ++tag : tag;
     s.consumed = 0;
     s.started = false;
+    s.resumable = false;
+    s.resumes = 0;
     s.range = trace_start(job->algo == Algo::kScrypt ? "otd.scrypt.batch"
                           : job->algo == Algo::kX11  ? "otd.x11.batch"
                                                      : "otd.sha256d.batch");
@@ -615,6 +675,7 @@
     sink.out = s.d_count;
     sink.ring = s.ring_dev;
     sink.abort = d_abort;
+    sink.yield = yield_word();
     sink.cap = kHitCap;
     sink.tag = s.tag;
     sink.epoch = s.epoch;
@@ -634,14 +695,44 @@
               : group->use_v             ? launch_sha_v(s, *job, sink)
               : group->nvar > 1          ? launch_sha_k(s, *job, sink)
                                          : launch_sha_single(s, *job, sink);
-    OTD_HIP(hipMemcpyAsync(s.h_count, s.d_count, sizeof(uint32_t), hipMemcpyDeviceToHost, stream));
-    OTD_HIP(hipEventRecord(s.done, stream));
+    queue_tail(s);
     s.busy = true;
     cursor.advance(s.count, group->nvar);
     std::lock_guard<std::mutex> g(m.stats_mu_);
     m.stats_.variant_epoch = job->epoch;
     m.stats_.launch_hashes = s.count * uint64_t(s.nvar);
     m.stats_.variant_next = cursor.variant_next(job->variant_start, job->variant_stride, group->nvar);
+  }
+
+  void queue_tail(Batch& s) {
+    OTD_HIP(hipMemcpyAsync(s.h_count, s.d_count, sizeof(uint32_t), hipMemcpyDeviceToHost, s.stream));
+    if (s.resumable)
+      OTD_HIP(hipMemcpyAsync(s.h_count.h + 1, s.d_progress.h + romix_waves(uint32_t(s.sgrid)), sizeof(uint32_t),
+                             hipMemcpyDeviceToHost, s.stream));
+    OTD_HIP(hipEventRecord(s.done, s.stream));
+  }
+
+  bool park_or_resume(Batch& b, bool* progressed) {
+    const uint32_t count64 = (uint32_t(b.count) + 63u) & ~63u;
+    const bool aborted = int32_t(epoch - b.epoch) > 0;
+    const bool complete = romix_batch_complete(b.h_count.h[1], count64, uint32_t(b.sgrid));
+    switch (yield_step(aborted, complete, yield_up)) {
+      case YieldStep::kRetireAborted:
+      case YieldStep::kRetireComplete:
+        return false;
+      case YieldStep::kWait:
+        return true;
+      case YieldStep::kResume:
+        break;
+    }
+    OTD_HIP(launch_scrypt_yield(b.sp, b.sbase, uint32_t(b.count), b.sxb, b.spad, b.d_progress, kRomixIters,
+                                kScryptStageRomix | kScryptStageOut, b.ssink, b.sgrid, b.sgrid, b.stream));
+    queue_tail(b);
+    ++b.resumes;
+    *progressed = true;
+    std::lock_guard<std::mutex> g(m.stats_mu_);
+    m.stats_.resumed_launches += 1;
+    return true;
   }
 
   bool retire_completed(const JobPtr& job, uint64_t gen) {
@@ -652,6 +743,7 @@
       if (q == hipErrorNotReady) { ++it; continue; }
       OTD_HIP(q);
       if (!b.started) b.started = true;
+      if (b.resumable && park_or_resume(b, &progressed)) { ++it; continue; }
       finish(b, job, gen);
       it = fifo.erase(it);
       progressed = true;
@@ -693,6 +785,7 @@
     while (job && (int)fifo.size() < kInflight) {
       const uint64_t v = job->variant_start + cursor.k * job->variant_stride;
       if (v >= job->variant_space()) break;
+      if (job->algo == Algo::kScrypt && yield_up) break;
       if (job->algo == Algo::kScrypt && scrypt_halves && fifo.size() == 1) {
         const Batch& only = slots[fifo.front()];
         if (only.epoch == epoch && monotonic_seconds() - only.enq_host < 0.5 * scrypt_hash_s) break;
@@ -746,6 +839,7 @@
       uint64_t gen = 0;
       auto job = check_epoch(&gen);
       if (job && gen != cur_gen) { cur_gen = gen; cursor.reset(); }
+      check_yield();
       bool progressed = false;
       for (int i : fifo)
         if (slots[i].clk_pending) clock_seen(slots[i]);
@@ -799,6 +893,18 @@
                                ops_sink(out, cap, 1), grid, reinterpret_cast<hipStream_t>(stream)));
 }
 
+void py_launch_scrypt_yield(const ScryptParams& p, uint32_t base, uint32_t count, uintptr_t xbuf, uintptr_t scratch,
+                            uintptr_t progress, uint32_t it_end, int stages, uintptr_t abort, uintptr_t yield,
+                            uint32_t epoch, uintptr_t out, uint32_t cap, int grid, int launch_grid, uintptr_t stream) {
+  HitSink s = ops_sink(out, cap, 1);
+  s.abort = reinterpret_cast<const uint32_t*>(abort);
+  s.yield = reinterpret_cast<const uint32_t*>(yield);
+  s.epoch = epoch;
+  OTD_HIP(launch_scrypt_yield(p, base, count, reinterpret_cast<void*>(xbuf), reinterpret_cast<void*>(scratch),
+                              reinterpret_cast<uint32_t*>(progress), it_end, stages, s, grid, launch_grid,
+                              reinterpret_cast<hipStream_t>(stream)));
+}
+
 void py_launch_x11_stage(const X11Params& p, int stage, uint32_t base, uintptr_t H, uint32_t stride, uint32_t n,
                          uintptr_t out, uint32_t cap, uintptr_t stream) {
   const HitSink s = ops_sink(out, cap, 1);
diff --git a/otedama_amd/engine/devproc.py b/otedama_amd/engine/devproc.py
--- a/otedama_amd/engine/devproc.py
+++ b/otedama_amd/engine/devproc.py
@@ -19,7 +19,8 @@
 MAX_FRAME = 64 << 20
 
 _CUMULATIVE = ("hashes", "candidates", "shares", "dropped", "launches", "rejected_candidates", "variant_launches",
-               "busy_seconds", "job_switches", "aborted_launches", "ring_hits", "ring_overflow", "verify_dropped")
+               "busy_seconds", "job_switches", "aborted_launches", "ring_hits", "ring_overflow", "verify_dropped",
+               "yields", "yield_expired", "resumed_launches")
 
 
 def _send(sock: socket.socket, obj, lock: threading.Lock | None = None) -> None:
@@ -163,6 +164,12 @@
     def set_job(self, template: dict | None) -> None:
         self._job = dict(template) if template is not None else None
         self._post({"op": "job", "t": self._job, "sent": time.monotonic()})
+
+    def request_yield(self, timeout_s: float = 0.05) -> None:
+        self._post({"op": "yield", "timeout": float(timeout_s)})
+
+    def release_yield(self) -> None:
+        self._post({"op": "unyield"})
 
     def poll(self, max_items: int = 256) -> list[dict]:
         out = []
@@ -318,6 +325,12 @@
                         if msg.get("sent"):
                             hops.append((time.monotonic() - float(msg["sent"])) * 1e3)
                         t_job = t_job or time.time()
+                    elif msg.get("op") == "yield":
+                        if hasattr(m, "request_yield"):
+                            m.request_yield(float(msg.get("timeout") or 0.05))
+                    elif msg.get("op") == "unyield":
+                        if hasattr(m, "release_yield"):
+                            m.release_yield()
                     elif msg.get("op") == "stop":
                         return 0
             if not first_hash and (m.stats()["job_switches"] > 0 or m.stats()["hashes"] > 0):
diff --git a/otedama_amd/parallel/comm_probe.py b/otedama_amd/parallel/comm_probe.py
--- a/otedama_amd/parallel/comm_probe.py
+++ b/otedama_amd/parallel/comm_probe.py
@@ -172,6 +172,8 @@
                 res["rate_alone"].append(_miner_rate(dp, a, _counter(dp)))
                 for c in configs:
                     def window(comm, c=c, w=w):
+                        if hasattr(comm, "yielder"):
+                            comm.yielder = dp
                         a = _counter(dp)
                         r = run_ops(comm, seconds, cadence_hz)
                         res["rate_with_ops"][c].append(_miner_rate(dp, a, _counter(dp)))
@@ -328,9 +330,17 @@
             time.sleep(rate_window_s)
             alone = _miner_rate(dp, a, _counter(dp)) or 0.0
             a = _counter(dp)
-            res = _lockstep_ops(comm, ops, cadence_hz, dev)
+            if hasattr(comm, "yielder"):
+                comm.yielder = dp
+            try:
+                res = _lockstep_ops(comm, ops, cadence_hz, dev)
+            finally:
+                if hasattr(comm, "yielder"):
+                    comm.yielder = None
             with_ops = _miner_rate(dp, a, _counter(dp)) or 0.0
             st = dp.stats()
+            res["yields"] = st.get("yields", 0)
+            res["resumed_launches"] = st.get("resumed_launches", 0)
             res["miner_rate_alone_hps"], res["miner_rate_with_ops_hps"] = alone, with_ops
             res["miner_faulted"] = bool(st.get("faulted"))
             out[ph] = res
diff --git a/otedama_amd/parallel/node.py b/otedama_amd/parallel/node.py
--- a/otedama_amd/parallel/node.py
+++ b/otedama_amd/parallel/node.py
@@ -238,6 +238,10 @@
         self.local = local
         self.comm = comm
         self.log = log
+        if hasattr(comm, "yielder") and comm.yielder is None:
+            from otedama_amd.parallel.rcclcomm import MinerYielder
+
+            comm.yielder = MinerYielder.of(local)
         self.store = comm.info.store
         self.rows: list[list[int]] = [[0, 0, 0, 0] for _ in range(comm.info.world_size)]
         self.error: BaseException | None = None
diff --git a/otedama_amd/parallel/rcclcomm.py b/otedama_amd/parallel/rcclcomm.py
--- a/otedama_amd/parallel/rcclcomm.py
+++ b/otedama_amd/parallel/rcclcomm.py
@@ -13,6 +13,31 @@
 COMM_KEY = "otd/comm"
 FAILED_ID = b"!"
 _HOSTED_SERVER = None
+
+
+YIELD_TIMEOUT_S = 0.05
+
+
+def yield_enabled() -> bool:
+    return os.environ.get("OTEDAMA_COMM_YIELD", "1") != "0"
+
+
+class MinerYielder:
+
+    def __init__(self, miners):
+        self.miners = [m for m in miners if hasattr(m, "request_yield") and hasattr(m, "release_yield")]
+
+    @classmethod
+    def of(cls, miner_set) -> "MinerYielder":
+        return cls([getattr(dm, "native", dm) for dm in getattr(miner_set, "miners", [])])
+
+    def request_yield(self, timeout_s: float = YIELD_TIMEOUT_S) -> None:
+        for m in self.miners:
+            m.request_yield(timeout_s)
+
+    def release_yield(self) -> None:
+        for m in self.miners:
+            m.release_yield()
 
 
 class NativeNodeComm:
@@ -36,6 +61,9 @@
             lo, hi = torch.cuda.Stream.priority_range()
             self.stream = torch.cuda.Stream(self.dev, priority=min(lo, hi))
         self._rc = None
+        self.yielder = None
+        self.yields = 0
+        self._release_q = None
         self._job_h = np.zeros(JOB_BLOB_BYTES, dtype=np.uint8)
 
     @property
@@ -46,6 +74,9 @@
         """Nothing to do: every native op selects the comm's device itself."""
 
     def close(self) -> None:
+        if self._release_q is not None:
+            self._release_q.put(None)
+            self._release_q = None
         self.abort()
 
     def abort(self) -> None:
@@ -84,14 +115,50 @@
     def _timeout(self) -> float:
         return self.deadline if self.bounded else PG_TIMEOUT_S
 
+    def _yield_on(self):
+        y = self.yielder
+        if y is None or not yield_enabled():
+            return None
+        y.request_yield(YIELD_TIMEOUT_S)
+        self.yields += 1
+        return y
+
+    def _release_after(self, y) -> None:
+        import queue
+        import threading
+
+        import torch
+
+        if self._release_q is None:
+            self._release_q = queue.SimpleQueue()
+
+            def drain(q=self._release_q):
+                while True:
+                    item = q.get()
+                    if item is None:
+                        return
+                    ev, who = item
+                    ev.synchronize()
+                    if q.empty():
+                        who.release_yield()
+
+            threading.Thread(target=drain, name="otedama-comm-yield", daemon=True).start()
+        ev = torch.cuda.Event()
+        ev.record(torch.cuda.current_stream(self.dev))
+        self._release_q.put((ev, y))
+
     def _call(self, fn, *args):
         if self._rc is None:
             raise RuntimeError("rccl: no communicator for this generation")
         self.collectives += 1
+        y = self._yield_on()
         try:
             return fn(*args, self._timeout())
         except TimeoutError as exc:
             raise CollectiveTimeout(str(exc)) from None
+        finally:
+            if y is not None:
+                y.release_yield()
 
     def broadcast_job(self, job: dict | None) -> dict | None:
         if self.info.is_primary:
@@ -155,8 +222,11 @@
         if self._rc is None:
             raise RuntimeError("rccl: no communicator for this generation")
         self.collectives += 1
+        y = self._yield_on() if getattr(self.dev, "type", "cpu") == "cuda" else None
         self._rc.all_gather_dev(inp.data_ptr(), out.data_ptr(), inp.numel() * inp.element_size(), self._cur_stream(),
                                 self._timeout())
+        if y is not None:
+            self._release_after(y)
 
     def broadcast_tensor(self, t, src: int = 0) -> None:
         if not self.multi:
@@ -164,7 +234,10 @@
         if self._rc is None:
             raise RuntimeError("rccl: no communicator for this generation")
         self.collectives += 1
+        y = self._yield_on() if getattr(self.dev, "type", "cpu") == "cuda" else None
         self._rc.broadcast_dev(t.data_ptr(), t.numel() * t.element_size(), src, self._cur_stream(), self._timeout())
+        if y is not None:
+            self._release_after(y)
 
     def run_async(self, fn):
         if self.stream is None:
```

Result: no change. 19.30 billion, median of 2 (+0.0%).
